# thanosDelatolas/eva-vos

Hardware: AMD Instinct MI355X
Metric: frames/sec STCN mask-propagate 480p 1-obj (higher is better)
Workload: dtype f32; 1 GPU; DAVIS-17-val-shaped 480x854 (padded 480x864) single-object STCN propagate: fresh engine, interact(mask,0), T=66 frames/video, mem_freq=5, top_k=50; one video per step per GPU; videos_per_gpu=38, streams_per_gpu=4, key_lookahead=0, clips=8 distinct synthetic clips (one per pooled engine), weights=synthetic recipe seed 0 (no checkpoints offline)

## Files before the change

### eva_vos_amd/csrc/engine.cpp

```cpp
#include "engine.h"
#include "src_hash.h"

#include <algorithm>
#include <atomic>
#include <cmath>
#include <cstdarg>
#include <cstdio>
#include <cstdlib>
#include <cstring>
#include <map>
#include <mutex>
#include <unordered_map>
#include <utility>

namespace stcn {

static thread_local char g_err[512] = "";
void set_error(const char *fmt, ...) {
    va_list ap;
    va_start(ap, fmt);
    vsnprintf(g_err, sizeof(g_err), fmt, ap);
    va_end(ap);
}
const char *get_error() { return g_err; }

Knobs Knobs::from_env() {
    Knobs k;
    k.wino_min_cin = env_int("STCN_WINO_MIN_CIN", k.wino_min_cin);
    k.wino_ppw = env_int("STCN_WINO_PPW", k.wino_ppw);
    k.wino4_chunk_mb = env_int("STCN_WINO4_CHUNK_MB", k.wino4_chunk_mb);
    k.fusion_conv12 = env_int("STCN_FUSION_CONV12", k.fusion_conv12) != 0;
    k.fusion_wino = env_int("STCN_FUSION_WINO", k.fusion_wino) != 0;
    k.pw_chain = env_int("STCN_PW_CHAIN", k.pw_chain);
    return k;
}

void Prof::reset() {
    for (int i = 0; i < STCN_K_COUNT; ++i) { flops[i] = 0; bytes[i] = 0; exec_flops[i] = 0; launches[i] = 0; }
    hbm_conv_flops = hbm_conv_bytes = hbm_conv_ms = 0; hbm_conv_launches = 0;
    wino2_flops = wino4_flops = 0;
    for (auto &e : events) { pool.push_back(e.a); pool.push_back(e.b); }
    events.clear();
}
Prof::Ev &Prof::push_pair(int cls, bool hbm) {
    Ev e; e.cls = cls; e.hbm = hbm;
    for (hipEvent_t *p : {&e.a, &e.b}) {
        if (!pool.empty()) { *p = pool.back(); pool.pop_back(); }
        else (void)hipEventCreate(p);
    }
    events.push_back(e);
    return events.back();
}
void Prof::begin(int cls, hipStream_t s) {
    launches[cls]++;
    if (!on) return;
    (void)hipEventRecord(push_pair(cls, false).a, s);
}
hipEvent_t *Prof::attach(int cls, bool hbm) {
    launches[cls]++;
    if (hbm) hbm_conv_launches++;
    if (!on) return nullptr;
    return &push_pair(cls, hbm).a;
}
void Prof::end(hipStream_t s) {
    if (!on) return;
    (void)hipEventRecord(events.back().b, s);
}
int Prof::collect(float *ms) {
    for (int i = 0; i < STCN_K_COUNT; ++i) ms[i] = 0.f;
    hbm_conv_ms = 0;
    for (auto &e : events) {
        if (hipEventSynchronize(e.b) != hipSuccess) return STCN_E_HIP;
        float t = 0.f;
        if (hipEventElapsedTime(&t, e.a, e.b) != hipSuccess) return STCN_E_HIP;
        ms[e.cls] += t;
        if (e.hbm) hbm_conv_ms += t;
    }
    return STCN_OK;
}
Prof::~Prof() {
    for (auto &e : events) { (void)hipEventDestroy(e.a); (void)hipEventDestroy(e.b); }
    for (auto &p : pool) (void)hipEventDestroy(p);
}
struct Scope {
    Prof *p; hipStream_t s;
    Scope(Prof *p_, int cls, hipStream_t s_, double fl = 0) : p(p_), s(s_) {
        if (p) { p->flops[cls] += fl; p->begin(cls, s); }
    }
    ~Scope() { if (p) p->end(s); }
};

const ConvW &Model::c(const std::string &name) const {
    auto it = conv.find(name);
    if (it == conv.end()) { static ConvW empty; set_error("missing conv '%s'", name.c_str()); return empty; }
    return it->second;
}

struct HostT { const float *p; int nd; int64_t sh[4]; };

static int upload(Model &m, const std::vector<float> &h, float **dev) {
    HIPCHK(hipMalloc((void **)dev, h.size() * sizeof(float)));
    m.allocs.push_back(*dev);
    HIPCHK(hipMemcpy(*dev, h.data(), h.size() * sizeof(float), hipMemcpyHostToDevice));
    return STCN_OK;
}

bool wants_wino(const ConvW &cw) {
    const bool fusion32 = cw.cin_p == 32 && cw.cout == 32;
    return !(!wino_enabled() || cw.kh != 3 || cw.kw != 3 || cw.cin_p % 32 || ((cw.cin_p < Knobs::from_env().wino_min_cin || cw.cout % 64) && !fusion32));
}
bool wants_wino_fusion12(const ConvW &cw) { return wino_enabled() && cw.kh == 3 && cw.kw == 3 && cw.cin_p == 12 && cw.cout == 32; }
bool wants_wino4(const ConvW &cw) {
    return !(!wino4_mode() || cw.kh != 3 || cw.kw != 3 || cw.cin_p % 32 || cw.cin_p < W4_MIN_CIN || cw.cout % 32);
}

int make_wino(Model &m, ConvW &cw, const std::vector<float> &w) {
    if (!wants_wino(cw)) return STCN_OK;
    std::vector<float> u((size_t)16 * cw.cin_p * cw.cout);
    wino_transform_weights(w.data(), cw.cout, cw.cin_p, cw.Kp, u.data());
    return upload(m, u, &cw.wino_u);
}

int make_wino_fusion12(Model &m, ConvW &cw, const std::vector<float> &w) {
    if (!wants_wino_fusion12(cw)) return STCN_OK;
    std::vector<float> w16((size_t)32 * 9 * 16, 0.f), u((size_t)16 * 16 * 32);
    for (int n = 0; n < 32; ++n)
        for (int tap = 0; tap < 9; ++tap)
            for (int c = 0; c < 12; ++c) w16[((size_t)n * 9 + tap) * 16 + c] = w[(size_t)n * cw.Kp + tap * 12 + c];
    wino_transform_weights(w16.data(), 32, 16, 9 * 16, u.data());
    return upload(m, u, &cw.wino_u);
}

int make_wino4(Model &m, ConvW &cw, const std::vector<float> &w) {
    if (!wants_wino4(cw)) return STCN_OK;
    std::vector<float> u((size_t)36 * cw.cin_p * cw.cout);
    wino4_transform_weights(w.data(), cw.cout, cw.cin_p, cw.Kp, u.data());
    return upload(m, u, &cw.wino4_u);
}

static bool wino4_layer(const std::string &name) {
    if (name == "value_encoder.layer2.0.conv1" || name == "value_encoder.layer3.0.conv1") return false;
    if (name == "key_encoder.layer2.0.conv2" || name == "key_encoder.layer3.0.conv2") return false;
    static const bool key_f4 = env_on("STCN_WINO4_KEY");
    if (key_f4 && name.compare(0, 12, "key_encoder.") == 0 && name.size() > 6 && name.compare(name.size() - 6, 6, ".conv2") == 0) return true;
    static const bool kproj_f4 = env_on("STCN_WINO4_KEYPROJ");
    if (kproj_f4 && name == "key_proj.key_proj") return true;
    return name.compare(0, 8, "decoder.") == 0 || name == "key_comp" || name.compare(0, 20, "value_encoder.fuser.") == 0 ||
           name.compare(0, 19, "value_encoder.layer") == 0;
}

static std::vector<float> repack(const HostT &wt, const std::vector<float> &scale, int lo, int hi, const ConvW &cw) {
    const int cout = (int)wt.sh[0], cin = (int)wt.sh[1], kh = (int)wt.sh[2], kw = (int)wt.sh[3];
    std::vector<float> w((size_t)cout * cw.Kp, 0.f);
    for (int n = 0; n < cout; ++n)
        for (int c = lo; c < hi; ++c)
            for (int y = 0; y < kh; ++y)
                for (int x = 0; x < kw; ++x)
                    w[(size_t)n * cw.Kp + (size_t)(y * kw + x) * cw.cin_p + (c - lo)] =
                        wt.p[(((size_t)n * cin + c) * kh + y) * kw + x] * scale[n];
    return w;
}

static int add_convs(Model &m, const std::map<std::string, HostT> &sd) {
    for (auto &kv : sd) {
        const std::string &name = kv.first;
        if (name.size() < 8 || name.compare(name.size() - 7, 7, ".weight") != 0 || kv.second.nd != 4) continue;
        const std::string pre = name.substr(0, name.size() - 7);
        const HostT &wt = kv.second;
        const int cout = (int)wt.sh[0], cin = (int)wt.sh[1], kh = (int)wt.sh[2], kw = (int)wt.sh[3];
        std::string bn;
        const size_t dot = pre.rfind('.');
        const std::string leaf = pre.substr(dot + 1), head = pre.substr(0, dot);
        if (leaf.compare(0, 4, "conv") == 0) bn = head + ".bn" + leaf.substr(4);
        else if (leaf == "0") bn = head + ".1";
        const bool has_bn = !bn.empty() && sd.count(bn + ".running_mean");
        std::vector<float> scale(cout, 1.f), bias(cout, 0.f);
        auto bit = sd.find(pre + ".bias");
        if (bit != sd.end()) for (int n = 0; n < cout; ++n) bias[n] = bit->second.p[n];
        if (has_bn) {
            const float *g = sd.at(bn + ".weight").p, *b = sd.at(bn + ".bias").p;
            const float *mu = sd.at(bn + ".running_mean").p, *var = sd.at(bn + ".running_var").p;
            for (int n = 0; n < cout; ++n) {
                const float sc = g[n] / std::sqrt(var[n] + 1e-5f);
                scale[n] = sc;
                bias[n] = (bias[n] - mu[n]) * sc + b[n];
            }
        }
        ConvW cw;
        cw.cout = cout; cw.cin = cin; cw.kh = kh; cw.kw = kw;
        cw.cin_p = (cin + 3) / 4 * 4;
        cw.K = kh * kw * cw.cin_p;
        cw.Kp = (cw.K + 31) / 32 * 32;
        const std::vector<float> w = repack(wt, scale, 0, cin, cw);
        int rc = upload(m, w, &cw.w);
        if (rc) return rc;
        rc = upload(m, bias, &cw.bias);
        if (rc) return rc;
        if ((rc = make_wino(m, cw, w)) || (rc = make_wino_fusion12(m, cw, w))) return rc;
        if (wino4_layer(pre) && (rc = make_wino4(m, cw, w))) return rc;
        cw.bias0 = bias[0];
        m.conv[pre] = cw;
        static const struct { const char *name; int c0; } splits[] = {
            {"decoder.compress.conv1", 512}, {"decoder.compress.downsample", 512},
            {"value_encoder.fuser.block1.conv1", 256}, {"value_encoder.fuser.block1.downsample", 256}};
        for (const auto &sp : splits) {
            if (pre != sp.name) continue;
            for (int part = 0; part < 2; ++part) {
                const int lo = part ? sp.c0 : 0, hi = part ? cin : sp.c0;
                ConvW pw;
                pw.cout = cout; pw.cin = hi - lo; pw.cin_p = hi - lo; pw.kh = kh; pw.kw = kw;
                pw.K = kh * kw * pw.cin_p; pw.Kp = (pw.K + 31) / 32 * 32;
                const std::vector<float> ww = repack(wt, scale, lo, hi, pw);
                std::vector<float> bb = part ? bias : std::vector<float>(cout, 0.f);
                if ((rc = upload(m, ww, &pw.w)) || (rc = upload(m, bb, &pw.bias))) return rc;
                if ((rc = make_wino(m, pw, ww))) return rc;
                if (wino4_layer(pre) && (rc = make_wino4(m, pw, ww))) return rc;
                pw.bias0 = bb[0];
                m.conv[pre + (part ? "#b" : "#a")] = pw;
            }
        }
    }
    return STCN_OK;
}

static int add_fusion(Model &m, const stcn_weight_desc *fuse, int n_fuse);
static int build_model(Model &m, const stcn_weight_desc *prop, int n_prop, const stcn_weight_desc *fuse, int n_fuse) {
    std::map<std::string, HostT> sd;
    for (int i = 0; i < n_prop; ++i) {
        if (!prop[i].name || !prop[i].data || prop[i].ndim < 0 || prop[i].ndim > 4) {
            set_error("bad weight descriptor %d", i);
            return STCN_E_INVALID;
        }
        HostT t{prop[i].data, prop[i].ndim, {1, 1, 1, 1}};
        for (int d = 0; d < prop[i].ndim; ++d) t.sh[d] = prop[i].shape[d];
        sd[prop[i].name] = t;
    }
    int rc = add_convs(m, sd);
    if (rc) return rc;
    static const char *required[] = {
        "key_encoder.conv1", "key_encoder.res2.0.downsample.0", "key_encoder.layer3.5.conv3", "key_proj.key_proj",
        "key_comp", "value_encoder.conv1", "value_encoder.layer3.1.conv2", "value_encoder.fuser.block1.downsample",
        "value_encoder.fuser.block2.conv2", "decoder.compress.downsample", "decoder.up_16_8.skip_conv",
        "decoder.up_16_8.out_conv.downsample", "decoder.up_8_4.out_conv.conv2", "decoder.pred"};
    for (const char *r : required)
        if (!m.conv.count(r)) { set_error("state_dict lacks '%s.weight'", r); return STCN_E_MISSING; }
    const char *cb = "value_encoder.fuser.attention.";
    auto need = [&](const std::string &n) -> const HostT * {
        auto it = sd.find(std::string(cb) + n);
        if (it == sd.end()) { set_error("state_dict lacks '%s%s'", cb, n.c_str()); return nullptr; }
        return &it->second;
    };
    const HostT *w1 = need("ChannelGate.mlp.1.weight"), *b1 = need("ChannelGate.mlp.1.bias");
    const HostT *w2 = need("ChannelGate.mlp.3.weight"), *b2 = need("ChannelGate.mlp.3.bias");
    const HostT *ws = need("SpatialGate.spatial.conv.weight"), *bs = need("SpatialGate.spatial.conv.bias");
    if (!w1 || !b1 || !w2 || !b2 || !ws || !bs) return STCN_E_MISSING;
    float *d;
    auto up = [&](const HostT *t, size_t n, const float **dst) -> int {
        std::vector<float> h(t->p, t->p + n);
        int r = upload(m, h, &d);
        *dst = d;
        return r;
    };
    if ((rc = up(w1, 32 * 512, &m.cbam.w1)) || (rc = up(b1, 32, &m.cbam.b1)) || (rc = up(w2, 512 * 32, &m.cbam.w2)) ||
        (rc = up(b2, 512, &m.cbam.b2)) || (rc = up(ws, 98, &m.cbam.wsp)))
        return rc;
    m.cbam.bsp = bs->p[0];
    m.has_prop = true;
    if (fuse && n_fuse > 0) return add_fusion(m, fuse, n_fuse);
    return STCN_OK;
}
static int add_fusion(Model &m, const stcn_weight_desc *fuse, int n_fuse) {
    std::map<std::string, HostT> fsd;
    for (int i = 0; i < n_fuse; ++i) {
        HostT t{fuse[i].data, fuse[i].ndim, {1, 1, 1, 1}};
        for (int dd = 0; dd < fuse[i].ndim; ++dd) t.sh[dd] = fuse[i].shape[dd];
        fsd[std::string("fuse.") + fuse[i].name] = t;
    }
    const int rc = add_convs(m, fsd);
    if (rc) return rc;
    for (const char *r : {"fuse.conv1.0", "fuse.conv2.0", "fuse.conv2.2", "fuse.conv3.0", "fuse.conv3.2", "fuse.final_conv"})
        if (!m.conv.count(r)) { set_error("fusion state_dict lacks '%s.weight'", r + 5); return STCN_E_MISSING; }
    m.has_fuse = true;
    return STCN_OK;
}

namespace {
struct DevPool {
    std::mutex mu;
    std::map<std::pair<int, size_t>, std::vector<void *>> free_;
    std::unordered_map<void *, std::pair<int, size_t>> live;
    size_t cached = 0;
    size_t cap() {
        static const size_t c = [] { const char *e = getenv("STCN_POOL_GB"); const double gb = e ? atof(e) : 64.0; return gb > 0 ? (size_t)(gb * (double)(1u << 30)) : (size_t)0; }();
        return c;
    }
    static size_t size_class(size_t bytes) {
        if (bytes <= (1u << 20)) return (bytes + 4095) / 4096 * 4096;
        size_t step = 1;
        while ((step << 4) <= bytes) step <<= 1;
        return (bytes + step - 1) / step * step;
    }
};
DevPool &pool() { static DevPool p; return p; }
}

hipError_t pool_malloc(void **p, size_t bytes) {
    DevPool &pl = pool();
    int dev = 0;
    (void)hipGetDevice(&dev);
    const size_t sc = DevPool::size_class(bytes);
    if (pl.cap() > 0) {
        bool hit = false;
        {
            std::lock_guard<std::mutex> g(pl.mu);
            auto it = pl.free_.find({dev, sc});
            if (it != pl.free_.end() && !it->second.empty()) {
                *p = it->second.back();
                it->second.pop_back();
                pl.cached -= sc;
                pl.live[*p] = {dev, sc};
                hit = true;
            }
        }
        if (hit) {
            static const bool poison = env_on("STCN_POOL_POISON", false);
            if (poison) { (void)hipMemset(*p, 0xFF, sc); (void)hipStreamSynchronize(nullptr); }
            return hipSuccess;
        }
    }
    hipError_t er = hipMalloc(p, sc);
    if (er != hipSuccess && pl.cap() > 0) {
        (void)hipGetLastError();
        pool_release();
        er = hipMalloc(p, sc);
    }
    if (er == hipSuccess && pl.cap() > 0) {
        std::lock_guard<std::mutex> g(pl.mu);
        pl.live[*p] = {dev, sc};
    }
    return er;
}

void pool_free(void *p) {
    if (!p) return;
    DevPool &pl = pool();
    {
        std::lock_guard<std::mutex> g(pl.mu);
        auto it = pl.live.find(p);
        if (it != pl.live.end()) {
            const auto key = it->second;
            pl.live.erase(it);
            if (pl.cached + key.second <= pl.cap()) {
                pl.free_[key].push_back(p);
                pl.cached += key.second;
                return;
            }
        }
    }
    (void)hipFree(p);
}

void pool_release() {
    DevPool &pl = pool();
    std::vector<void *> all;
    {
        std::lock_guard<std::mutex> g(pl.mu);
        for (auto &kv : pl.free_) { all.insert(all.end(), kv.second.begin(), kv.second.end()); kv.second.clear(); }
        pl.cached = 0;
    }
    for (void *q : all) (void)hipFree(q);
}

size_t wino_v_capacity(const Dims &d, int maxb) {
    const long mt = ((long)maxb * ((d.h4 + 1) / 2) * ((d.w4 + 1) / 2) + 63) / 64 * 64;
    size_t v = wino_enabled() ? (size_t)16 * 256 * mt : 0;
    if (v * 4 >= ((size_t)1 << 32)) v = ((size_t)1 << 30) - 64;
    return v;
}
int Work::init(int nh, int nw, int k_, int key_batch, int group) {
    d.set(nh, nw);
    k = k_;
    auto alloc = [&](void **p, size_t bytes) -> int {
        HIPCHK(pool_malloc(p, bytes));
        allocs.push_back(*p);
        return STCN_OK;
    };
    const size_t s1 = (size_t)k * d.hw2 * 64, s2 = (size_t)d.npix * 32, s3 = (size_t)k * d.hw4 * 256;
    const size_t s4 = (size_t)key_batch * d.hw2 * 64;
    const size_t s5 = (size_t)group * k * d.hw4 * 256;
    S = s1 > s2 ? s1 : s2;
    S = S > s3 ? S : s3;
    S = S > s4 ? S : s4;
    S = S > s5 ? S : s5;
    const int kg = k * group;
    int rc;
    for (float **b : {&A, &B, &C, &D})
        if ((rc = alloc((void **)b, S * sizeof(float)))) return rc;
    splitk_floats = (size_t)32 * 1024 * 1024;
    if ((rc = alloc((void **)&splitk, splitk_floats * sizeof(float)))) return rc;
    {
        wino_v_floats = wino_v_capacity(d, key_batch > k * group ? key_batch : k * group);
        if (wino_v_floats && (rc = alloc((void **)&wino_v, wino_v_floats * sizeof(float)))) return rc;
    }
    if ((rc = alloc((void **)&cbam, (size_t)k * (16 * 1024 + 512 + 3 * d.hw16) * sizeof(float)))) return rc;
    if ((rc = alloc((void **)&readout, (size_t)kg * d.hw16 * 512 * sizeof(float)))) return rc;
    if ((rc = alloc((void **)&logit4, (size_t)kg * d.hw4 * sizeof(float)))) return rc;
    if ((rc = alloc((void **)&flogit, (size_t)k * d.npix * sizeof(float)))) return rc;
    if ((rc = alloc((void **)&agg, (size_t)(k + 1) * group * d.npix * sizeof(float)))) return rc;
    if ((rc = alloc((void **)&agg_alt, (size_t)(k + 1) * group * d.npix * sizeof(float)))) return rc;
    if ((rc = alloc((void **)&pooled, (size_t)std::max(20, attention_nchp(2 * (k + 1))) * d.hw16 * sizeof(float)))) return rc;
    if ((rc = alloc((void **)&amap, (size_t)(k + 1) * 2 * d.hw16 * sizeof(float)))) return rc;
    if ((rc = alloc((void **)&attn, (size_t)(k + 1) * 2 * d.npix * sizeof(float)))) return rc;
    const MemReadScratchSizes ms = memread_scratch_floats(group * d.hw16);
    if ((rc = alloc((void **)&cand_v, std::max(ms.cand_v, attention_part_floats(k + 1, d.hw16)) * sizeof(float)))) return rc;
    if ((rc = alloc((void **)&cand_i, ms.cand_i * sizeof(int32_t)))) return rc;
    if ((rc = alloc((void **)&cand_n, ms.cand_n * sizeof(int32_t)))) return rc;
    if ((rc = alloc((void **)&qk, (size_t)group * d.hw16 * 64 * sizeof(float)))) return rc;
    if ((rc = alloc((void **)&vin, (size_t)k * d.npix * 8 * sizeof(float)))) return rc;
    if ((rc = alloc((void **)&gmax, ms.gmax * sizeof(float)))) return rc;
    if ((rc = alloc((void **)&tau, ms.tau * sizeof(float)))) return rc;
    return STCN_OK;
}
void Work::release() {
    for (void *p : allocs) pool_free(p);
    allocs.clear();
}

static thread_local int g_fail_countdown = 0;
static thread_local int g_fail_reserve = 0;
static std::atomic<int> g_side_delay_us{0};
void inject_failure_after(int n) { g_fail_countdown = n; }
int launch_status(const char *what) {
    if (g_fail_countdown > 0 && --g_fail_countdown == 0) {
        (void)hipGetLastError();
        set_error("launch of '%s' failed: injected fault (stcn_test_fail_at)", what);
        return STCN_E_HIP;
    }
    const hipError_t er = hipGetLastError();
    if (er == hipSuccess) return STCN_OK;
    set_error("launch of '%s' failed: %s", what, hipGetErrorString(er));
    return STCN_E_HIP;
}

namespace {
struct ConvPathRec {
    ConvPlan plan{};
    char lit[96] = "";
};
thread_local ConvPathRec g_path;
thread_local char g_path_str[96] = "";
thread_local bool g_trace_on = false;
thread_local std::string g_trace;
}
const char *format_conv_path(const ConvPlan &pl, char *out, size_t n) {
    switch (pl.family) {
    case CONV_FUSION: snprintf(out, n, "%s", pl.fusion_wino ? "fusion_wino" : "fusion_direct"); break;
    case CONV_WINO4: snprintf(out, n, "wino4 chunks=%d%s", pl.w4.chunks, pl.reduce ? " +tail" : ""); break;
    case CONV_WINO2: snprintf(out, n, "wino2 ppw=%d splitk=%d", pl.ppw, pl.splitk); break;
    case CONV_DIRECT: snprintf(out, n, "%s%s splitk=%d", pl.variant, pl.tail ? " +tail" : "", pl.splitk); break;
    default: snprintf(out, n, "%s", "");
    }
    return out;
}
const char *last_conv_path() { return g_path.plan.family == CONV_LITERAL ? g_path.lit : format_conv_path(g_path.plan, g_path_str, sizeof(g_path_str)); }
void set_conv_path(const char *s) { g_path.plan.family = CONV_LITERAL; snprintf(g_path.lit, sizeof(g_path.lit), "%s", s); }
void conv_trace(int on) { g_trace_on = on != 0; if (on) g_trace.clear(); }
const char *conv_trace_get() { return g_trace.c_str(); }

int plan_conv(const Model &m, const Work &w, const std::string &name, const ConvArgs &a, ConvP &p, ConvPlan &pl) {
    auto it = m.conv.find(name);
    if (it == m.conv.end()) { set_error("missing conv '%s'", name.c_str()); return STCN_E_MISSING; }
    const ConvW &cw = it->second;
    const int B = a.B, H = a.H, W = a.W, c0 = a.c0, c1 = a.c1;
    if (c0 + c1 != cw.cin_p) { set_error("conv '%s': %d+%d input channels, weights have %d", name.c_str(), c0, c1, cw.cin_p); return STCN_E_INVALID; }
    p = ConvP{};
    p.B = B; p.H = H; p.W = W;
    p.KH = cw.kh; p.KW = cw.kw; p.stride = a.stride; p.pad = cw.kh / 2;
    p.OH = (H + 2 * p.pad - cw.kh) / a.stride + 1;
    p.OW = (W + 2 * p.pad - cw.kw) / a.stride + 1;
    p.Cin = cw.cin_p;
    p.M = B * p.OH * p.OW; p.N = cw.cout; p.K = cw.K; p.Kp = cw.Kp;
    const long bs0 = a.bs0 == CONV_DENSE ? (long)H * W * c0 : a.bs0, bs1 = a.bs1 == CONV_DENSE ? (long)H * W * c1 : a.bs1;
    const long res_bs = a.res_bs == CONV_DENSE ? (long)p.OH * p.OW * p.N : a.res_bs;
    p.x0 = a.x0; p.x1 = a.x1; p.c0 = c0; p.c1 = c1; p.bs0 = bs0; p.bs1 = bs1;
    const long x0b = (bs0 ? (long)B * bs0 : (long)H * W * c0) * 4, x1b = a.x1 ? (bs1 ? (long)B * bs1 : (long)H * W * c1) * 4 : 0;
    if (x0b >= (1L << 31) || x1b >= (1L << 31) || (long)cw.cout * cw.Kp * 4 >= (1L << 31)) {
        set_error("conv '%s': operand of %ld bytes exceeds the 2 GiB the kernels can address (B=%d, %dx%d)", name.c_str(), x0b > x1b ? x0b : x1b, B, H, W);
        return STCN_E_INVALID;
    }
    p.x0_bytes = (unsigned)x0b;
    p.x1_bytes = (unsigned)x1b;
    p.w_bytes = (unsigned)((long)cw.cout * cw.Kp * 4);
    if (a.x1 && ((cw.cin_p % 32) || (c0 % 32) || cw.kh * cw.kw > 32)) { set_error("conv '%s': two-source input needs 32-aligned channel splits", name.c_str()); return STCN_E_INVALID; }
    p.w = cw.w; p.wino_u = cw.wino_u; p.wino4_u = cw.wino4_u;
    p.bias = cw.bias; p.res = a.res; p.res_bs = res_bs; p.res_bmod = a.res_bmod; p.y = a.y; p.y_bs = a.y_bs;
    p.relu_in = a.relu_in; p.relu_out = a.relu_out;
    p.fd_ohw = fastdiv_make((unsigned)(p.OH * p.OW));
    p.fd_ow = fastdiv_make((unsigned)p.OW);
    p.fd_cin = fastdiv_make((unsigned)p.Cin);
    p.fd_kw = fastdiv_make((unsigned)p.KW);
    p.pointwise = cw.kh == 1 && cw.kw == 1 && a.stride == 1 && !a.x1 && bs0 == (long)H * W * c0;
    p.affine_out = (a.y_bs == 0 || a.y_bs == (long)p.OH * p.OW * p.N) && (!a.res || (res_bs == (long)p.OH * p.OW * p.N && !a.res_bmod)) &&
                   ((long)p.M + 128) * p.N * 4 < (1L << 32);
    p.partial = w.splitk;
    p.kn = w.kn;
    pl = ConvPlan{};
    pl.fl = 2.0 * p.M * p.N * (double)(cw.kh * cw.kw * cw.cin);
    if (a.force_splitk <= 0 && (fusion_conv_plan(p, pl) || wino4_plan(p, m.wino4_min_wg, w.wino_v_floats, w.splitk_floats, pl) ||
                                wino_plan(p, w.wino_v_floats, w.splitk_floats, pl)))
        return STCN_OK;
    conv_plan(p, a.force_splitk, w.splitk_floats, pl);
    return STCN_OK;
}

int run_conv(const Model &m, Work &w, hipStream_t s, const std::string &name, const ConvArgs &a) {
    ConvP p;
    ConvPlan &pl = g_path.plan;
    const int rc = plan_conv(m, w, name, a, p, pl);
    if (rc) return rc;
    hipEvent_t *eg[W4_MAX_CHUNKS] = {}, *ei[W4_MAX_CHUNKS] = {}, *er = nullptr;
    if (w.prof) {
        const double in0 = (double)(p.bs0 ? p.B : 1) * p.H * p.W * p.c0, in1 = p.x1 ? (double)(p.bs1 ? p.B : 1) * p.H * p.W * p.c1 : 0.0;
        const double resb = p.res ? (p.res_bs ? (double)p.M * p.N : (double)p.OH * p.OW * p.N) : 0.0;
        const double bytes = 4.0 * (in0 + in1 + (double)p.N * p.K + (double)p.M * p.N + resb);
        const bool hbm_bound = pl.fl / bytes < 157.3e12 / 8.0e12;
        const int cls = w.conv_cls;
        const bool hbm_acc = hbm_bound && cls == STCN_K_CONV;
        w.prof->bytes[cls] += bytes;
        w.prof->flops[cls] += pl.fl;
        w.prof->exec_flops[cls] += pl.fl_exec;
        if (hbm_acc) { w.prof->hbm_conv_bytes += bytes; w.prof->hbm_conv_flops += pl.fl; }
        if (pl.family == CONV_WINO4) w.prof->wino4_flops += pl.fl; else if (pl.family == CONV_WINO2) w.prof->wino2_flops += pl.fl;
        for (int c = 0; c < pl.n_gemm; ++c) {
            eg[c] = w.prof->attach(cls, hbm_acc);
            if (c < pl.n_in) ei[c] = w.prof->attach(STCN_K_WINO_INPUT);
        }
        if (pl.reduce) er = w.prof->attach(STCN_K_CONV_REDUCE);
    }
    if (g_trace_on) { char b[96]; g_trace += name; g_trace += '='; g_trace += format_conv_path(pl, b, sizeof(b)); g_trace += '\n'; }
    switch (pl.family) {
    case CONV_FUSION: fusion_conv_launch(p, pl, s, eg[0]); break;
    case CONV_WINO4: wino4_launch(p, pl, w.wino_v, s, ei, eg, er); break;
    case CONV_WINO2: wino_launch(p, pl, w.wino_v, s, ei[0], eg[0], er); break;
    default: conv_launch(p, s, eg[0], er);
    }
    return launch_status(name.c_str());
}

#define RC(x) do { int rc_ = (x); if (rc_) return rc_; } while (0)

int encode_key(const Model &m, Work &w, hipStream_t s, const float *img4, const KeyOut &o, int B, long out_bs) {
    const Dims &d = w.d;
    const long obs = B > 1 ? out_bs : 0;
    const long ibs = obs ? obs : CONV_DENSE;
    RC(run_conv(m, w, s, "key_encoder.conv1", ConvArgs(img4, 4, B, d.nh, d.nw).strided(2).out(w.A).relu(0, 1)));
    { Scope sc(w.prof, STCN_K_ELEMWISE, s); maxpool3x3s2_launch(w.A, w.B, B, d.h2, d.w2, 64, s); }
    struct St { const char *name; int n, planes, stride; } stages[3] = {{"res2", 3, 64, 1}, {"layer2", 4, 128, 2}, {"layer3", 6, 256, 2}};
    int H = d.h4, W = d.w4, cin = 64;
    float *x = w.B;
    for (int si = 0; si < 3; ++si) {
        const St &st = stages[si];
        for (int i = 0; i < st.n; ++i) {
            const std::string p = std::string("key_encoder.") + st.name + "." + std::to_string(i);
            const int sd = i == 0 ? st.stride : 1;
            const int OH = H / sd, OW = W / sd;
            const float *idt = x;
            if (i == 0) { RC(run_conv(m, w, s, p + ".downsample.0", ConvArgs(x, cin, B, H, W).strided(sd).out(w.D))); idt = w.D; }
            RC(run_conv(m, w, s, p + ".conv1", ConvArgs(x, cin, B, H, W).out(w.C).relu(0, 1)));
            RC(run_conv(m, w, s, p + ".conv2", ConvArgs(w.C, st.planes, B, H, W).strided(sd).out(w.A).relu(0, 1)));
            float *dst = x;
            long dst_bs = 0;
            if (si == 2 && i == st.n - 1) { dst = o.f16; dst_bs = obs; }
            RC(run_conv(m, w, s, p + ".conv3", ConvArgs(w.A, st.planes, B, OH, OW).out(dst, dst_bs).residual(idt).relu(0, 1)));
            x = dst; H = OH; W = OW; cin = st.planes * 4;
        }
        if (si == 0) {
            if (o.f4_copy) HIPCHK(hipMemcpyAsync(o.f4_copy, x, (size_t)d.hw4 * 256 * 4, hipMemcpyDeviceToDevice, s));
            if (o.s4) RC(run_conv(m, w, s, "decoder.up_8_4.skip_conv", ConvArgs(x, 256, B, d.h4, d.w4).out(o.s4, obs)));
        } else if (si == 1) {
            if (o.f8_copy) HIPCHK(hipMemcpyAsync(o.f8_copy, x, (size_t)d.hw8 * 512 * 4, hipMemcpyDeviceToDevice, s));
            if (o.s8) RC(run_conv(m, w, s, "decoder.up_16_8.skip_conv", ConvArgs(x, 512, B, d.h8, d.w8).out(o.s8, obs)));
        }
    }
    if (o.k16) {
        RC(run_conv(m, w, s, "key_proj.key_proj", ConvArgs(o.f16, 1024, B, d.h16, d.w16, ibs).out(o.k16, obs)));
        if (o.msq) {
            Scope sc(w.prof, STCN_K_ELEMWISE, s);
            rowsumsq_launch(o.k16, d.hw16, 64, o.msq, s, B, out_bs, out_bs);
        }
    }
    if (o.f16_thin) RC(run_conv(m, w, s, "key_comp", ConvArgs(o.f16, 1024, B, d.h16, d.w16, ibs).out(o.f16_thin, obs)));
    if (o.f16_thin && o.dthin) {
        RC(run_conv(m, w, s, "decoder.compress.downsample#b", ConvArgs(o.f16_thin, 512, B, d.h16, d.w16, ibs).out(o.dthin, obs)));
        RC(run_conv(m, w, s, "decoder.compress.conv1#b", ConvArgs(o.f16_thin, 512, B, d.h16, d.w16, ibs).out(o.cthin, obs).relu(1, 0)));
    }
    return STCN_OK;
}

int value_frame_parts(const Model &m, Work &w, hipStream_t s, const float *f16, float *vd, float *vc) {
    const Dims &d = w.d;
    RC(run_conv(m, w, s, "value_encoder.fuser.block1.downsample#b", ConvArgs(f16, 1024, 1, d.h16, d.w16).out(vd)));
    RC(run_conv(m, w, s, "value_encoder.fuser.block1.conv1#b", ConvArgs(f16, 1024, 1, d.h16, d.w16).out(vc).relu(1, 0)));
    return STCN_OK;
}

static int resblock_split(const Model &m, Work &w, hipStream_t s, const std::string &p, const float *x, int c, int B,
                          int H, int W, const float *dpart, const float *cpart, long part_bs, int part_bmod, float *t1, float *t2,
                          float *out, long out_bs) {
    const ConvW &cw = m.c(p + ".conv1");
    RC(run_conv(m, w, s, p + ".downsample#a", ConvArgs(x, c, B, H, W).out(t2).residual(dpart, part_bs, part_bmod)));
    RC(run_conv(m, w, s, p + ".conv1#a", ConvArgs(x, c, B, H, W).out(t1).residual(cpart, part_bs, part_bmod).relu(1, 1)));
    RC(run_conv(m, w, s, p + ".conv2", ConvArgs(t1, cw.cout, B, H, W).out(out, out_bs).residual(t2)));
    return STCN_OK;
}

static int resblock(const Model &m, Work &w, hipStream_t s, const std::string &p, const float *x0, int c0, long bs0,
                    const float *x1, int c1, long bs1, int B, int H, int W, float *t1, float *t2, float *out,
                    long out_bs) {
    const ConvW &cw = m.c(p + ".conv1");
    const ConvArgs in = ConvArgs(x0, c0, B, H, W, bs0).concat(x1, c1, bs1);
    const float *skip; long skip_bs;
    if (m.conv.count(p + ".downsample")) {
        RC(run_conv(m, w, s, p + ".downsample", ConvArgs(in).out(t2)));
        skip = t2; skip_bs = CONV_DENSE;
    } else { skip = x0; skip_bs = bs0; }
    RC(run_conv(m, w, s, p + ".conv1", ConvArgs(in).out(t1).relu(1, 1)));
    RC(run_conv(m, w, s, p + ".conv2", ConvArgs(t1, cw.cout, B, H, W).out(out, out_bs).residual(skip, skip_bs)));
    return STCN_OK;
}

int encode_value(const Model &m, Work &w, hipStream_t s, const float *img4, const float *f16, const float *masks,
                 long mask_stride, float *out, long out_bs, const float *vd, const float *vc) {
    const Dims &d = w.d;
    const int k = w.k;
    { Scope sc(w.prof, STCN_K_ELEMWISE, s); pack_value_input_launch(img4, masks, mask_stride, k, (int)d.npix, w.vin, s); }
    RC(run_conv(m, w, s, "value_encoder.conv1", ConvArgs(w.vin, 8, k, d.nh, d.nw).strided(2).out(w.C).relu(0, 1)));
    { Scope sc(w.prof, STCN_K_ELEMWISE, s); maxpool3x3s2_launch(w.C, w.B, k, d.h2, d.w2, 64, s); }
    int H = d.h4, W = d.w4, cin = 64;
    const int planes[3] = {64, 128, 256}, strides[3] = {1, 2, 2};
    for (int li = 0; li < 3; ++li)
        for (int i = 0; i < 2; ++i) {
            const std::string p = "value_encoder.layer" + std::to_string(li + 1) + "." + std::to_string(i);
            const int sd = i == 0 ? strides[li] : 1;
            const int OH = H / sd, OW = W / sd;
            const float *idt = w.B;
            if (m.conv.count(p + ".downsample.0")) {
                RC(run_conv(m, w, s, p + ".downsample.0", ConvArgs(w.B, cin, k, H, W).strided(sd).out(w.D)));
                idt = w.D;
            }
            RC(run_conv(m, w, s, p + ".conv1", ConvArgs(w.B, cin, k, H, W).strided(sd).out(w.C).relu(0, 1)));
            RC(run_conv(m, w, s, p + ".conv2", ConvArgs(w.C, planes[li], k, OH, OW).out(w.B).residual(idt).relu(0, 1)));
            H = OH; W = OW; cin = planes[li];
        }
    const std::string f = "value_encoder.fuser.";
    if (vd && vc)
        RC(resblock_split(m, w, s, f + "block1", w.B, 256, k, d.h16, d.w16, vd, vc, 0, 0, w.C, w.D, w.A, 0));
    else
        RC(resblock(m, w, s, f + "block1", w.B, 256, (long)d.hw16 * 256, f16, 1024, 0, k, d.h16, d.w16, w.C, w.D, w.A, 0));
    { Scope sc(w.prof, STCN_K_OTHER, s); cbam_launch(w.A, w.C, k, d.h16, d.w16, m.cbam, w.cbam, s); }
    RC(resblock(m, w, s, f + "block2", w.C, 512, (long)d.hw16 * 512, nullptr, 0, 0, k, d.h16, d.w16, w.D, w.A, out, out_bs));
    return STCN_OK;
}

int decode_logit4(const Model &m, Work &w, hipStream_t s, const float *readout, const float *f16_thin, const float *s8,
                  const float *s4, const float *dthin, const float *cthin, int G, long slot_bs) {
    const Dims &d = w.d;
    const int k = w.k;
    if (G > 1 && (!dthin || !cthin)) { set_error("decode: frame batches need the cached frame parts"); return STCN_E_INVALID; }
    const int B = G > 1 ? G * k : k;
    const long fbs = G > 1 ? slot_bs : 0;
    const int bmod = G > 1 && k > 1 ? G : 0;
    if (dthin && cthin) {
        RC(resblock_split(m, w, s, "decoder.compress", readout, 512, B, d.h16, d.w16, dthin, cthin, fbs, bmod, w.C, w.D, w.A, 0));
    } else {
        RC(resblock(m, w, s, "decoder.compress", readout, 512, (long)d.hw16 * 512, f16_thin, 512, 0, k, d.h16, d.w16, w.C,
                    w.D, w.A, 0));
    }
    { Scope sc(w.prof, STCN_K_ELEMWISE, s); upsample2x_add_launch(w.A, s8, w.B, B, d.h16, d.w16, 512, s, fbs, bmod); }
    RC(resblock(m, w, s, "decoder.up_16_8.out_conv", w.B, 512, (long)d.hw8 * 512, nullptr, 0, 0, B, d.h8, d.w8, w.C, w.D,
                w.A, 0));
    { Scope sc(w.prof, STCN_K_ELEMWISE, s); upsample2x_add_launch(w.A, s4, w.B, B, d.h8, d.w8, 256, s, fbs, bmod); }
    RC(resblock(m, w, s, "decoder.up_8_4.out_conv", w.B, 256, (long)d.hw4 * 256, nullptr, 0, 0, B, d.h4, d.w4, w.C, w.D,
                w.A, 0));
    const ConvW &pw = m.c("decoder.pred");
    {
        Scope sc(w.prof, STCN_K_CONV_N1, s, 2.0 * B * d.hw4 * 9 * 256);
        conv_n1_launch(w.A, pw.w, pw.bias0, w.logit4, B, d.h4, d.w4, 256, 3, 1, s);
    }
    return STCN_OK;
}

int decode(const Model &m, Work &w, hipStream_t s, const float *readout, const float *f16_thin, const float *s8,
           const float *s4, float *agg, long agg_stride, const float *dthin, const float *cthin, int G, long slot_bs, long agg_gs) {
    const Dims &d = w.d;
    const int k = w.k;
    RC(decode_logit4(m, w, s, readout, f16_thin, s8, s4, dthin, cthin, G, slot_bs));
    {
        Scope sc(w.prof, STCN_K_ELEMWISE, s);
        if (G > 1)
            up4_sigmoid_aggregate_launch(w.logit4, k, d.h4, d.w4, agg, agg_stride, s, (long)G * d.hw4, G, (long)d.hw4, agg_gs ? agg_gs : (long)(k + 1) * agg_stride);
        else
            up4_sigmoid_aggregate_launch(w.logit4, k, d.h4, d.w4, agg, agg_stride, s);
    }
    return launch_status("decoder tail");
}

int fusion_logit(const Model &m, Work &w, hipStream_t s, const float *img4, const float *prev, const float *curr,
                 const float *attn2, float nc, float nr, float *logit) {
    if (!m.has_fuse) { set_error("model was built without a fusion network"); return STCN_E_STATE; }
    const Dims &d = w.d;
    { Scope sc(w.prof, STCN_K_ELEMWISE, s); pack_fusion_input_launch(img4, prev, curr, attn2, nc, nr, d.npix, w.A, s); }
    struct Cls { Work &w; Cls(Work &w_) : w(w_) { w.conv_cls = STCN_K_FUSION_CONV; } ~Cls() { w.conv_cls = STCN_K_CONV; } } cls_guard(w);
    RC(run_conv(m, w, s, "fuse.conv1.0", ConvArgs(w.A, 12, 1, d.nh, d.nw).out(w.B).relu(0, 1)));
    RC(run_conv(m, w, s, "fuse.conv2.0", ConvArgs(w.B, 32, 1, d.nh, d.nw).out(w.C).relu(0, 1)));
    RC(run_conv(m, w, s, "fuse.conv2.2", ConvArgs(w.C, 32, 1, d.nh, d.nw).out(w.D).residual(w.B).relu(0, 1)));
    RC(run_conv(m, w, s, "fuse.conv3.0", ConvArgs(w.D, 32, 1, d.nh, d.nw).out(w.C).relu(0, 1)));
    RC(run_conv(m, w, s, "fuse.conv3.2", ConvArgs(w.C, 32, 1, d.nh, d.nw).out(w.B).residual(w.D).relu(0, 1)));
    const ConvW &fw = m.c("fuse.final_conv");
    Scope sc(w.prof, STCN_K_CONV_N1, s, 2.0 * d.npix * 9 * 32);
    conv_n1_launch(w.B, fw.w, fw.bias0, logit, 1, d.nh, d.nw, 32, 3, 0, s);
    return STCN_OK;
}

std::vector<SweepGroup> plan_sweep(int idx, int closest, int mem_freq, int cap) {
    const int step = closest > idx ? 1 : -1, span = std::abs(closest - idx) - 1;
    std::vector<SweepGroup> groups;
    if (span > 0) groups.reserve(span / mem_freq + span / (cap > 1 ? cap : 1) + 1);
    int last = 0;
    auto inserts = [&](int dist) { return dist != span && dist - last >= mem_freq; };
    for (int dist = 1, G; dist <= span; dist += G) {
        G = 1;
        while (G < cap && !inserts(dist + G - 1) && dist + G <= span) ++G;
        const int first = idx + dist * step;
        const bool ins = inserts(dist + G - 1);
        groups.push_back(SweepGroup{first, step > 0 ? first : first - (G - 1), G, ins});
        if (ins) last = dist + G - 1;
    }
    return groups;
}

}

using namespace stcn;

extern "C" {

const char *stcn_last_error(void) { return stcn::get_error(); }
const char *stcn_version(void) { return "stcn_hip 0.4 (gfx950; exact-fp32 MFMA convs: direct implicit GEMM + Winograd; src " STCN_SRC_HASH ")"; }

int stcn_model_create(int device, const stcn_weight_desc *prop, int n_prop, const stcn_weight_desc *fuse, int n_fuse,
                      stcn_model **out) {
    return stcn_model_create_ex(device, prop, n_prop, fuse, n_fuse, nullptr, out);
}

static_assert(STCN_MAX_TOP_K == MEMREAD_MAX_TOPK, "the C ABI's limit is the read's");

int stcn_model_create_ex(int device, const stcn_weight_desc *prop, int n_prop, const stcn_weight_desc *fuse, int n_fuse,
                         const stcn_model_opts *opts, stcn_model **out) {
    if (!prop || n_prop <= 0 || !out) { set_error("stcn_model_create: null arguments"); return STCN_E_INVALID; }
    const int top_k = opts && opts->top_k > 0 ? opts->top_k : STCN_MAX_TOP_K;
    if (top_k > STCN_MAX_TOP_K) {
        set_error("stcn_model_create: top_k=%d is not supported: the memory read is built for 1 <= top_k <= %d", top_k, STCN_MAX_TOP_K);
        return STCN_E_INVALID;
    }
    if (opts && !std::isfinite(opts->km)) {
        set_error("stcn_model_create: km=%f is not supported: the kernelized memory read takes a finite km > 0 (0 or negative: not given)", (double)opts->km);
        return STCN_E_INVALID;
    }
    const float km = opts && opts->km > 0.f ? opts->km : 0.f;
    HIPCHK(hipSetDevice(device));
    stcn_model *mm = new stcn_model();
    mm->m.device = device;
    mm->m.top_k = top_k;
    mm->m.km = km;
    const int rc = build_model(mm->m, prop, n_prop, fuse, n_fuse);
    if (rc) { stcn_model_destroy(mm); return rc; }
    *out = mm;
    return STCN_OK;
}

int stcn_fusion_model_create(int device, const stcn_weight_desc *fuse, int n_fuse, stcn_model **out) {
    if (!fuse || n_fuse <= 0 || !out) { set_error("stcn_fusion_model_create: null arguments"); return STCN_E_INVALID; }
    for (int i = 0; i < n_fuse; ++i)
        if (!fuse[i].name || !fuse[i].data || fuse[i].ndim < 0 || fuse[i].ndim > 4) { set_error("bad weight descriptor %d", i); return STCN_E_INVALID; }
    HIPCHK(hipSetDevice(device));
    stcn_model *mm = new stcn_model();
    mm->m.device = device;
    const int rc = add_fusion(mm->m, fuse, n_fuse);
    if (rc) { stcn_model_destroy(mm); return rc; }
    *out = mm;
    return STCN_OK;
}

int stcn_model_get_top_k(const stcn_model *m, int32_t *top_k) {
    if (!m || !top_k) { set_error("stcn_model_get_top_k: null arguments"); return STCN_E_INVALID; }
    *top_k = m->m.top_k;
    return STCN_OK;
}

int stcn_model_get_km(const stcn_model *m, float *km) {
    if (!m || !km) { set_error("stcn_model_get_km: null arguments"); return STCN_E_INVALID; }
    *km = m->m.km;
    return STCN_OK;
}

int stcn_model_destroy(stcn_model *m) {
    if (!m) return STCN_OK;
    for (void *p : m->m.allocs) (void)hipFree(p);
    delete m;
    return STCN_OK;
}

static int eng_alloc(stcn_engine *e, void **p, size_t bytes) {
    HIPCHK(pool_malloc(p, bytes));
    e->allocs.push_back(*p);
    return STCN_OK;
}

struct SlotPtrs { float *k16, *msq, *f16_thin, *f16, *s8, *s4, *dthin, *cthin, *vd, *vc; };
struct PassCtx { hipStream_t s; Work *w; bool may_offload; int dir; };
static PassCtx main_ctx(stcn_engine *e) { return PassCtx{e->stream, &e->work, true, +1}; }
struct SweepBank {
    int lo, n_certain, dir, n_temp;
    int slots() const { return n_certain + n_temp; }
    int first() const { return dir > 0 ? lo : lo - n_temp; }
    int next_slot() const { return dir > 0 ? lo + n_certain + n_temp : lo - 1 - n_temp; }
};
struct Neighbours { int lo, hi; };
static Neighbours interacted_neighbours(const stcn_engine *e, int idx) {
    Neighbours n{-1, e->T};
    for (int t : e->interacted) { if (t < idx && t > n.lo) n.lo = t; if (t > idx && t < n.hi) n.hi = t; }
    return n;
}
static int sweep_slots(int span, int mem_freq) { return span / mem_freq + 1; }
static SlotPtrs slot_ptrs(const stcn_engine *e, int slot) {
    const Dims &d = e->d;
    float *b = e->cache + (size_t)slot * e->slot_floats;
    SlotPtrs p;
    p.k16 = b; b += (size_t)d.hw16 * 64;
    p.msq = b; b += (size_t)(d.hw16 + 3) / 4 * 4;
    p.f16_thin = b; b += (size_t)d.hw16 * 512;
    p.f16 = b; b += (size_t)d.hw16 * 1024;
    p.s8 = b; b += (size_t)d.hw8 * 512;
    p.s4 = b; b += (size_t)d.hw4 * 256;
    p.dthin = b; b += (size_t)d.hw16 * 512;
    p.cthin = b; b += (size_t)d.hw16 * 512;
    p.vd = b; b += (size_t)d.hw16 * 512;
    p.vc = b;
    return p;
}

static void bank_collect_retired(stcn_engine *e, bool wait) {
    if (e->retired.empty()) return;
    if (wait) (void)hipEventSynchronize(e->retire_ev);
    else if (hipEventQuery(e->retire_ev) != hipSuccess) return;
    for (void *p : e->retired) pool_free(p);
    e->retired.clear();
}

static int bank_reserve(stcn_engine *e, int slots) {
    if (slots <= e->bank_cap) return STCN_OK;
    const Dims &d = e->d;
    int cap = e->bank_cap ? e->bank_cap : 8;
    while (cap < slots) cap *= 2;
    float *nk = nullptr, *nq = nullptr, *nv = nullptr;
    int32_t *nc = nullptr;
    const size_t rows = (size_t)cap * d.hw16;
    const size_t cblock = e->model->km > 0.f ? (size_t)e->group * memread_centre_stride((int)rows) : 0;
    hipError_t er = pool_malloc((void **)&nk, rows * 64 * 4);
    if (er == hipSuccess) er = pool_malloc((void **)&nq, (rows + MEMREAD_MSQ_PAD) * 4);
    if (er == hipSuccess) er = pool_malloc((void **)&nv, (size_t)e->k * rows * 512 * 4);
    if (er == hipSuccess && cblock) er = pool_malloc((void **)&nc, 2 * cblock * 4);
    if (er != hipSuccess) {
        if (nk) pool_free(nk);
        if (nq) pool_free(nq);
        if (nv) pool_free(nv);
        if (nc) pool_free(nc);
        set_error("bank_reserve: %d slots (%zu MB) -> %s", cap, ((size_t)e->k * rows * 512 * 4 + rows * 65 * 4) >> 20, hipGetErrorString(er));
        return STCN_E_HIP;
    }
    auto fail = [&](hipError_t err, const char *what) {
        (void)hipStreamSynchronize(e->stream);
        pool_free(nk); pool_free(nq); pool_free(nv);
        if (nc) pool_free(nc);
        set_error("bank_reserve: %s -> %s", what, hipGetErrorString(err));
        return STCN_E_HIP;
    };
    if (e->n_certain > 0) {
        const size_t crow = (size_t)e->n_certain * d.hw16, orow = (size_t)e->bank_cap * d.hw16, lo = (size_t)e->bank_lo * d.hw16;
        if ((er = hipMemcpyAsync(nk + lo * 64, e->bank_k + lo * 64, crow * 64 * 4, hipMemcpyDeviceToDevice, e->stream)) != hipSuccess) return fail(er, "copy of the certain keys");
        if ((er = hipMemcpyAsync(nq + lo, e->bank_msq + lo, crow * 4, hipMemcpyDeviceToDevice, e->stream)) != hipSuccess) return fail(er, "copy of |mk|^2");
        for (int o = 0; o < e->k; ++o)
            if ((er = hipMemcpyAsync(nv + (o * rows + lo) * 512, e->bank_v + (o * orow + lo) * 512, crow * 512 * 4, hipMemcpyDeviceToDevice, e->stream)) != hipSuccess)
                return fail(er, "copy of the certain values");
    }
    if (e->bank_k) {
        bank_collect_retired(e, true);
        if (!e->retire_ev && (er = hipEventCreateWithFlags(&e->retire_ev, hipEventDisableTiming)) != hipSuccess) return fail(er, "event create");
        if ((er = hipEventRecord(e->retire_ev, e->stream)) != hipSuccess) return fail(er, "event record");
        e->retired = {e->bank_k, e->bank_msq, e->bank_v};
        if (e->bank_centre) e->retired.push_back(e->bank_centre);
    }
    e->bank_k = nk; e->bank_msq = nq; e->bank_v = nv; e->bank_cap = cap;
    e->bank_centre = nc; e->work.centre = nc; e->work2.centre = nc ? nc + cblock : nullptr;
    return STCN_OK;
}

static int engine_alloc_common(stcn_engine *e) {
    const Dims &d = e->d;
    if (!e->images4) {
        HIPCHK(pool_malloc((void **)&e->images4, (size_t)e->T * d.npix * 4 * 4));
        e->images_owner = std::shared_ptr<void>(e->images4, [](void *p) { pool_free(p); });
    }
    e->n_slots = e->T < 106 ? e->T : 106;
    e->slot_floats = (size_t)d.hw16 * (64 + 512 + 1024) + (size_t)(d.hw16 + 3) / 4 * 4 + (size_t)d.hw8 * 512 + (size_t)d.hw4 * 256 +
                     (size_t)4 * d.hw16 * 512;
    RC(eng_alloc(e, (void **)&e->cache, (size_t)e->n_slots * e->slot_floats * 4));
    e->slot_of.assign(e->T, -1);
    e->vparts_ready.assign(e->T, 0);
    RC(eng_alloc(e, (void **)&e->mask_pad, (size_t)(e->k + 1) * d.npix * 4));
    RC(eng_alloc(e, (void **)&e->pos, (size_t)(e->k + 1) * d.npix * 4));
    RC(eng_alloc(e, (void **)&e->neg, (size_t)(e->k + 1) * d.npix * 4));
    auto opt = [](int32_t &field, const char *env, int dflt) { if (field < 0) field = env_int(env, dflt); return (int)field; };
    const int la_env = opt(e->opts.lookahead, "STCN_LOOKAHEAD", 2);
    e->lookahead = la_env;
    if (e->T > e->n_slots) e->lookahead = 0;
    e->group = opt(e->opts.decode_batch, "STCN_DECODE_BATCH", 8);
    if (e->group > e->mem_freq) e->group = e->mem_freq;
    if (e->group < 1) e->group = 1;
    if (e->group > MAX_DECODE_GROUP) e->group = MAX_DECODE_GROUP;
    while (e->group > 1 && e->group * e->k > 16) --e->group;
    e->key_batch = opt(e->opts.key_batch, "STCN_KEY_BATCH", 0);
    if (e->key_batch <= 0) e->key_batch = e->group > 4 ? e->group : 4;
    if (e->key_batch < 1) e->key_batch = 1;
    if (e->key_batch > 8) e->key_batch = 8;
    RC(e->work.init(d.nh, d.nw, e->k, e->lookahead > 0 ? 1 : e->key_batch, e->group));
    e->work.prof = &e->prof;
    e->fuse_side = la_env > 0 && e->model->has_fuse && opt(e->opts.fuse_side, "STCN_FUSE_SIDE", 1) != 0;
    if (e->lookahead > 0 || e->fuse_side) {
        HIPCHK(hipStreamCreateWithFlags(&e->side, hipStreamNonBlocking));
        RC(e->work_side.init(d.nh, d.nw, e->k, e->lookahead > 0 ? e->key_batch : 1));
        e->work_side.prof = &e->prof;
        for (int b = 0; b < 2 && e->fuse_side; ++b) {
            HIPCHK(hipEventCreateWithFlags(&e->ev_dec[b], hipEventDisableTiming));
            HIPCHK(hipEventCreateWithFlags(&e->ev_fuse[b], hipEventDisableTiming));
        }
    }
    if (e->lookahead > 0) {
        e->key_ready.assign(e->T, nullptr);
        for (int t = 0; t < e->T; ++t) HIPCHK(hipEventCreateWithFlags(&e->key_ready[t], hipEventDisableTiming));
    }
    e->key_pending.assign(e->T, 0);
    e->bank_lo = 0;
    {
        const char *dv = getenv("STCN_DUAL_SWEEP");
        if (la_env > 0 && e->T <= e->n_slots && e->T >= 3 && (!dv || atoi(dv) != 0)) {
            HIPCHK(hipStreamCreateWithFlags(&e->stream2, hipStreamNonBlocking));
            RC(e->work2.init(d.nh, d.nw, e->k, e->lookahead > 0 ? 1 : e->key_batch, e->group));
            e->work2.prof = &e->prof;
            HIPCHK(hipEventCreateWithFlags(&e->ev_fork, hipEventDisableTiming));
            HIPCHK(hipEventCreateWithFlags(&e->ev_join, hipEventDisableTiming));
            e->bank_lo = sweep_slots(e->T - 1, e->mem_freq) + 1;
        }
    }
    return STCN_OK;
}

static int engine_init_outputs(stcn_engine *e) {
    const Dims &d = e->d;
    fill_launch(e->prob, 1e-7f, (long)e->T * d.npix, e->stream);
    fill_launch(e->prob + (size_t)e->T * d.npix, 0.f, (long)e->k * e->T * d.npix, e->stream);
    HIPCHK(hipMemsetAsync(e->masks, 0, (size_t)e->T * d.npix, e->stream));
    return STCN_OK;
}

int stcn_engine_create(const stcn_model *m, int T, int H, int W, int k, int mem_freq, void *stream,
                       const float *images_dev, float *prob_dev, uint8_t *masks_dev, stcn_engine **out) {
    return stcn_engine_create_ex(m, T, H, W, k, mem_freq, stream, images_dev, prob_dev, masks_dev, nullptr, out);
}

int stcn_engine_create_ex(const stcn_model *m, int T, int H, int W, int k, int mem_freq, void *stream,
                          const float *images_dev, float *prob_dev, uint8_t *masks_dev, const stcn_engine_opts *opts, stcn_engine **out) {
    if (!m || !images_dev || !prob_dev || !masks_dev || !out) { set_error("stcn_engine_create: null arguments"); return STCN_E_INVALID; }
    if (T < 1 || H < 16 || W < 16 || k < 1 || k > STCN_MAX_OBJECTS || mem_freq < 1) {
        set_error("stcn_engine_create: bad shape T=%d H=%d W=%d k=%d mem_freq=%d (1<=k<=%d)", T, H, W, k, mem_freq, STCN_MAX_OBJECTS);
        return STCN_E_INVALID;
    }
    if (!m->m.has_prop) { set_error("stcn_engine_create: a model of stcn_fusion_model_create serves stcn_stage_fusion only"); return STCN_E_STATE; }
    HIPCHK(hipSetDevice(m->m.device));
    stcn_engine *e = new stcn_engine();
    e->model = &m->m; e->stream = (hipStream_t)stream;
    if (opts) e->opts = *opts;
    e->T = T; e->H = H; e->W = W; e->k = k; e->mem_freq = mem_freq;
    const int nh = (H + 15) / 16 * 16, nw = (W + 15) / 16 * 16;
    e->lh = (nh - H) / 2; e->uh = nh - H - e->lh; e->lw = (nw - W) / 2; e->uw = nw - W - e->lw;
    e->d.set(nh, nw);
    if ((long)e->d.hw16 < m->m.top_k) {
        set_error("frame too small: (H/16)*(W/16) = %d must be >= top_k = %d for the top-k read", e->d.hw16, m->m.top_k);
        delete e;
        return STCN_E_INVALID;
    }
    e->prob = prob_dev; e->masks = masks_dev;
    int rc = engine_alloc_common(e);
    if (!rc) rc = bank_reserve(e, e->bank_lo + sweep_slots(T - 1, mem_freq) + 8);
    if (rc) { stcn_engine_destroy(e); return rc; }
    const Dims &d = e->d;
    for (int t = 0; t < T; ++t)
        pack_image_launch(images_dev + (size_t)t * 3 * H * W, e->images4 + (size_t)t * d.npix * 4, H, W, nh, nw, e->lw, e->lh, e->stream);
    if ((rc = engine_init_outputs(e))) { stcn_engine_destroy(e); return rc; }
    HIPCHK(hipStreamSynchronize(e->stream));
    *out = e;
    return STCN_OK;
}

int stcn_engine_reset(stcn_engine *e) {
    if (!e) { set_error("stcn_engine_reset: null engine"); return STCN_E_INVALID; }
    HIPCHK(hipSetDevice(e->model->device));
    if (e->side) HIPCHK(hipStreamSynchronize(e->side));
    if (e->stream2) HIPCHK(hipStreamSynchronize(e->stream2));
    e->failed.clear();
    e->interacted.clear();
    e->n_certain = 0;
    e->n_cached = 0;
    std::fill(e->slot_of.begin(), e->slot_of.end(), -1);
    std::fill(e->vparts_ready.begin(), e->vparts_ready.end(), 0);
    std::fill(e->key_pending.begin(), e->key_pending.end(), 0);
    e->fuse_pending[0] = e->fuse_pending[1] = 0;
    e->stats = stcn_stats{};
    return engine_init_outputs(e);
}

int stcn_engine_destroy(stcn_engine *e) {
    if (!e) return STCN_OK;
    if (e->stream) (void)hipStreamSynchronize(e->stream); else (void)hipDeviceSynchronize();
    if (e->side) { (void)hipStreamSynchronize(e->side); (void)hipStreamDestroy(e->side); }
    if (e->stream2) { (void)hipStreamSynchronize(e->stream2); (void)hipStreamDestroy(e->stream2); }
    if (e->ev_fork) (void)hipEventDestroy(e->ev_fork);
    if (e->ev_join) (void)hipEventDestroy(e->ev_join);
    e->work2.release();
    for (hipEvent_t ev : e->key_ready) if (ev) (void)hipEventDestroy(ev);
    for (int b = 0; b < 2; ++b) { if (e->ev_dec[b]) (void)hipEventDestroy(e->ev_dec[b]); if (e->ev_fuse[b]) (void)hipEventDestroy(e->ev_fuse[b]); }
    e->work_side.release();
    for (void *p : e->allocs) pool_free(p);
    if (e->bank_k) { pool_free(e->bank_k); pool_free(e->bank_msq); pool_free(e->bank_v); }
    if (e->bank_centre) pool_free(e->bank_centre);
    bank_collect_retired(e, true);
    if (e->retire_ev) (void)hipEventDestroy(e->retire_ev);
    e->work.release();
    delete e;
    return STCN_OK;
}

static int clone_state(stcn_engine *e, const stcn_engine *src) {
    const Dims &d = e->d;
    HIPCHK(hipStreamSynchronize(src->stream));
    if (src->side) HIPCHK(hipStreamSynchronize(src->side));
    if (src->stream2) HIPCHK(hipStreamSynchronize(src->stream2));
    HIPCHK(hipMemcpyAsync(e->cache, src->cache, (size_t)src->n_cached * e->slot_floats * 4, hipMemcpyDeviceToDevice, e->stream));
    e->slot_of = src->slot_of; e->n_cached = src->n_cached; e->vparts_ready = src->vparts_ready;
    e->n_certain = src->n_certain; e->interacted = src->interacted; e->failed = src->failed;
    const size_t crow = (size_t)e->n_certain * d.hw16;
    if (crow) {
        const size_t lo = (size_t)e->bank_lo * d.hw16, slo = (size_t)src->bank_lo * d.hw16;
        HIPCHK(hipMemcpyAsync(e->bank_k + lo * 64, src->bank_k + slo * 64, crow * 64 * 4, hipMemcpyDeviceToDevice, e->stream));
        HIPCHK(hipMemcpyAsync(e->bank_msq + lo, src->bank_msq + slo, crow * 4, hipMemcpyDeviceToDevice, e->stream));
        for (int o = 0; o < e->k; ++o)
            HIPCHK(hipMemcpyAsync(e->bank_v + ((size_t)o * e->bank_cap * d.hw16 + lo) * 512,
                                  src->bank_v + ((size_t)o * src->bank_cap * d.hw16 + slo) * 512, crow * 512 * 4,
                                  hipMemcpyDeviceToDevice, e->stream));
    }
    HIPCHK(hipMemcpyAsync(e->pos, src->pos, (size_t)(e->k + 1) * d.npix * 4, hipMemcpyDeviceToDevice, e->stream));
    HIPCHK(hipMemcpyAsync(e->neg, src->neg, (size_t)(e->k + 1) * d.npix * 4, hipMemcpyDeviceToDevice, e->stream));
    HIPCHK(hipStreamSynchronize(e->stream));
    return STCN_OK;
}

int stcn_engine_clone(const stcn_engine *src, float *prob_dev, uint8_t *masks_dev, void *stream, stcn_engine **out) {
    if (!src || !prob_dev || !masks_dev || !out) { set_error("stcn_engine_clone: null arguments"); return STCN_E_INVALID; }
    HIPCHK(hipSetDevice(src->model->device));
    stcn_engine *e = new stcn_engine();
    e->model = src->model; e->stream = (hipStream_t)stream;
    e->T = src->T; e->H = src->H; e->W = src->W; e->k = src->k; e->mem_freq = src->mem_freq;
    e->lw = src->lw; e->uw = src->uw; e->lh = src->lh; e->uh = src->uh; e->d = src->d;
    e->prob = prob_dev; e->masks = masks_dev;
    e->images4 = src->images4; e->images_owner = src->images_owner;
    e->opts = src->opts;
    e->work.kn = src->work.kn; e->work_side.kn = src->work_side.kn; e->work2.kn = src->work.kn;
    int rc = engine_alloc_common(e);
    if (!rc) rc = bank_reserve(e, src->bank_cap + e->bank_lo);
    if (!rc) rc = clone_state(e, src);
    if (rc) { stcn_engine_destroy(e); return rc; }
    *out = e;
    return STCN_OK;
}

static void flush_key_cache(stcn_engine *e) {
    for (int b = 0; b < 2; ++b)
        if (e->fuse_pending[b]) { (void)hipStreamWaitEvent(e->stream, e->ev_fuse[b], 0); e->fuse_pending[b] = 0; }
    std::fill(e->slot_of.begin(), e->slot_of.end(), -1);
    std::fill(e->vparts_ready.begin(), e->vparts_ready.end(), 0);
    e->n_cached = 0;
}

static int enqueue_key_batch(stcn_engine *e, int t_lo, int B, const PassCtx &cx) {
    const int slot = e->n_cached;
    e->n_cached += B;
    for (int b = 0; b < B; ++b) { e->slot_of[t_lo + b] = slot + b; e->vparts_ready[t_lo + b] = 0; }
    const SlotPtrs p = slot_ptrs(e, slot);
    KeyOut ko{p.k16, p.msq, p.f16_thin, p.f16, p.s8, p.s4, nullptr, nullptr, p.dthin, p.cthin};
    const float *img = e->images4 + (size_t)t_lo * e->d.npix * 4;
    if (e->lookahead > 0) {
        hipStream_t ks = e->side;
        if (const int us = g_side_delay_us.load(std::memory_order_relaxed)) spin_launch(us, ks);
        RC(encode_key(*e->model, e->work_side, ks, img, ko, B, (long)e->slot_floats));
        for (int b = 0; b < B; ++b) {
            HIPCHK(hipEventRecord(e->key_ready[t_lo + b], ks));
            e->key_pending[t_lo + b] = 1;
        }
    } else {
        RC(encode_key(*e->model, *cx.w, cx.s, img, ko, B, (long)e->slot_floats));
    }
    e->stats.key_miss += B;
    return STCN_OK;
}

static int enqueue_key(stcn_engine *e, int ti, const PassCtx &cx, int step = 0, int stop = 0) {
    if (e->slot_of[ti] >= 0) return STCN_OK;
    if (e->n_cached >= e->n_slots) flush_key_cache(e);
    int B = 1;
    if (step != 0)
        while (B < e->key_batch && e->n_cached + B < e->n_slots) {
            const int tn = ti + B * step;
            if (tn == stop || tn < 0 || tn >= e->T || e->slot_of[tn] >= 0) break;
            ++B;
        }
    return enqueue_key_batch(e, step < 0 ? ti - (B - 1) : ti, B, cx);
}

static int enqueue_group(stcn_engine *e, int t_lo, int G, const PassCtx &cx) {
    int missing = 0;
    for (int b = 0; b < G; ++b) missing += e->slot_of[t_lo + b] < 0;
    if (!missing) return STCN_OK;
    if (e->n_cached + missing > e->n_slots) { flush_key_cache(e); }
    for (int b = 0; b < G;) {
        if (e->slot_of[t_lo + b] >= 0) { ++b; continue; }
        int n = 1;
        while (b + n < G && n < e->key_batch && e->slot_of[t_lo + b + n] < 0) ++n;
        RC(enqueue_key_batch(e, t_lo + b, n, cx));
        b += n;
    }
    return STCN_OK;
}

static int ensure_key(stcn_engine *e, int ti, SlotPtrs *out, const PassCtx &cx) {
    RC(enqueue_key(e, ti, cx));
    if (e->key_pending[ti]) {
        HIPCHK(hipStreamWaitEvent(cx.s, e->key_ready[ti], 0));
        e->key_pending[ti] = 0;
    }
    *out = slot_ptrs(e, e->slot_of[ti]);
    return STCN_OK;
}

static void dbg_sum(stcn_engine *e, const char *tag, int ti, const float *p, size_t n) {
    static const bool on = getenv("STCN_DEBUG_CHECKSUM") != nullptr;
    if (!on) return;
    (void)hipDeviceSynchronize();
    std::vector<float> h(n);
    (void)hipMemcpy(h.data(), p, n * 4, hipMemcpyDeviceToHost);
    double s1 = 0, s2 = 0;
    unsigned long long hsh = 1469598103934665603ull, bag = 0;
    for (size_t i = 0; i < n; ++i) {
        unsigned u; memcpy(&u, &h[i], 4);
        hsh = (hsh ^ u) * 1099511628211ull;
        bag += (unsigned long long)u * 2654435761ull;
        if (std::isfinite(h[i])) { s1 += h[i]; s2 += (double)h[i] * h[i] * (1 + (i % 7)); }
    }
    fprintf(stderr, "CHK %-10s t=%d %.10e %.10e hash %016llx bag %016llx\n", tag, ti, s1, s2, hsh, bag);
    (void)e;
}

static float *bank_v_slot(stcn_engine *e, int slot) { return e->bank_v + (size_t)slot * e->d.hw16 * 512; }

static int bank_insert(stcn_engine *e, int slot, int ti, const SlotPtrs &kf, const float *masks, long mask_stride, const PassCtx &cx) {
    const Dims &d = e->d;
    {
        Scope sc(&e->prof, STCN_K_ELEMWISE, cx.s);
        copy2_launch(kf.k16, e->bank_k + (size_t)slot * d.hw16 * 64, (long)d.hw16 * 64, kf.msq, e->bank_msq + (size_t)slot * d.hw16, d.hw16, cx.s);
    }
    if (!e->vparts_ready[ti]) {
        RC(value_frame_parts(*e->model, *cx.w, cx.s, kf.f16, kf.vd, kf.vc));
        e->vparts_ready[ti] = 1;
    }
    RC(encode_value(*e->model, *cx.w, cx.s, e->images4 + (size_t)ti * d.npix * 4, kf.f16, masks, mask_stride,
                    bank_v_slot(e, slot), (long)e->bank_cap * d.hw16 * 512, kf.vd, kf.vc));
    dbg_sum(e, "value", ti, bank_v_slot(e, slot), (size_t)d.hw16 * 512);
    e->stats.value_enc++;
    return STCN_OK;
}

struct Sweep {
    const PassCtx &cx;
    int idx, closest, step;
    bool fuse;
    bool offload;
    SweepBank bank;
};

static int stage_keys_grouped(stcn_engine *e, const PassCtx &cx, const SweepGroup &g, const SweepGroup *next) {
    RC(enqueue_group(e, g.t_lo, g.G, cx));
    if (e->lookahead > 0 && next) RC(enqueue_group(e, next->t_lo, next->G, cx));
    return STCN_OK;
}
static int stage_keys_framewise(stcn_engine *e, const Sweep &sw, int ti) {
    RC(enqueue_key(e, ti, sw.cx, sw.step, sw.closest));
    for (int a = 1, tj = ti + sw.step; a <= e->lookahead && tj != sw.closest; ++a, tj += sw.step) RC(enqueue_key(e, tj, sw.cx, sw.step, sw.closest));
    return STCN_OK;
}

static int acquire_agg(stcn_engine *e, const PassCtx &cx, bool off, float **buf) {
    const int bi = off ? e->agg_buf : 0;
    if (cx.may_offload && e->fuse_pending[bi]) {
        HIPCHK(hipStreamWaitEvent(cx.s, e->ev_fuse[bi], 0));
        e->fuse_pending[bi] = 0;
    }
    *buf = bi ? cx.w->agg_alt : cx.w->agg;
    return STCN_OK;
}

static int read_decode(stcn_engine *e, const Sweep &sw, const SlotPtrs &f, int t_lo, int n, float *agg, long agg_rs) {
    const Dims &d = e->d;
    const int k = e->k, Q = n * d.hw16, N = sw.bank.slots() * d.hw16;
    const size_t row0 = (size_t)sw.bank.first() * d.hw16;
    Work &w = *sw.cx.w;
    hipStream_t const S = sw.cx.s;
    const float *qk = f.k16;
    if (n > 1) {
        Scope sc(&e->prof, STCN_K_ELEMWISE, S);
        copy_rows_launch(f.k16, (long)e->slot_floats, w.qk, (long)d.hw16 * 64, n, (long)d.hw16 * 64, S);
        qk = w.qk;
    }
    {
        const bool km = e->model->km > 0.f;
        const MemReadKm kmo{e->model->km, d.h16, d.w16, f.msq, (long)e->slot_floats, w.centre, nullptr};
        MemRead r{};
        r.mk = e->bank_k + row0 * 64; r.msq = e->bank_msq + row0; r.mv = e->bank_v + row0 * 512; r.mv_os = (long)e->bank_cap * d.hw16 * 512; r.N = N;
        r.qk = qk; r.Q = Q; r.k = k; r.top_k = e->model->top_k; r.readout = w.readout; r.ro_os = (long)Q * 512; r.km = km ? &kmo : nullptr;
        const MemReadCost cost = memread_cost(N, Q, k, r.top_k, km);
        Scope sc(&e->prof, STCN_K_MEMREAD, S, cost.flop);
        e->prof.bytes[STCN_K_MEMREAD] += cost.bytes;
        memory_read_launch(r, MemReadScratch{w.cand_v, w.cand_i, w.cand_n, w.gmax, w.tau}, S);
    }
    RC(launch_status(n > 1 ? "memory read (decode group)" : "memory read"));
    dbg_sum(e, "k16", t_lo, qk, (size_t)Q * 64);
    dbg_sum(e, "readout", t_lo, w.readout, (size_t)k * Q * 512);
    const long agg_gs = sw.fuse ? 0 : (long)d.npix;
    return decode(*e->model, w, S, w.readout, f.f16_thin, f.s8, f.s4, agg, agg_rs, f.dthin, f.cthin, n, (long)e->slot_floats, agg_gs);
}

static int fuse_frame(stcn_engine *e, const Sweep &sw, int t, const SlotPtrs &f, const float *agg, bool off, bool first_of_group) {
    const Dims &d = e->d;
    const int k = e->k;
    const long prs = (long)e->T * d.npix;
    float *dst = e->prob + (size_t)t * d.npix;
    const float nc = (float)std::abs(sw.closest - t) / (float)std::abs(sw.closest - sw.idx);
    const float nr = (float)std::abs(sw.idx - t) / (float)std::abs(sw.closest - sw.idx);
    const int cs = e->bank_lo + e->n_certain - 1;
    Work &fw = off ? e->work_side : *sw.cx.w;
    hipStream_t fs = off ? e->side : sw.cx.s;
    if (off && first_of_group) {
        HIPCHK(hipEventRecord(e->ev_dec[e->agg_buf], sw.cx.s));
        HIPCHK(hipStreamWaitEvent(e->side, e->ev_dec[e->agg_buf], 0));
        if (const int us = g_side_delay_us.load(std::memory_order_relaxed)) spin_launch(us, e->side);
    }
    {
        Scope sc(&e->prof, STCN_K_ATTENTION, fs, 2.0 * d.hw16 * d.hw16 * 64);
        attention_read_launch(e->bank_k + (size_t)cs * d.hw16 * 64, e->bank_msq + (size_t)cs * d.hw16, f.k16, nullptr,
                              nullptr, k + 1, d.h16, d.w16, e->work.pooled, fw.amap, fw.attn, AttnScratch{fw.gmax, fw.cand_v}, fs);
    }
    RC(launch_status("attention read"));
    for (int o = 1; o <= k; ++o)
        RC(fusion_logit(*e->model, fw, fs, e->images4 + (size_t)t * d.npix * 4, dst + (size_t)o * prs,
                        agg + (size_t)o * d.npix, fw.attn + (size_t)o * 2 * d.npix, nc, nr,
                        fw.flogit + (size_t)(o - 1) * d.npix));
    Scope sc(&e->prof, STCN_K_ELEMWISE, fs);
    sigmoid_aggregate_launch(fw.flogit, k, d.npix, dst, prs, fs);
    e->stats.fused++;
    return STCN_OK;
}

static int finish_frame(stcn_engine *e, Sweep &sw, int t, const SlotPtrs &f, float *agg, long agg_rs, bool inserts, bool off, bool first_of_group) {
    if (sw.fuse) dbg_sum(e, "agg", t, agg, (size_t)(e->k + 1) * e->d.npix);
    if (inserts) {
        RC(bank_insert(e, sw.bank.next_slot(), t, f, agg + agg_rs, agg_rs, sw.cx));
        ++sw.bank.n_temp;
    }
    if (sw.fuse) RC(fuse_frame(e, sw, t, f, agg, off, first_of_group));
    e->stats.frames++;
    return STCN_OK;
}

static int do_pass(stcn_engine *e, int idx, int closest, const PassCtx &cx) {
    const Dims &d = e->d;
    const bool forward = closest > idx, fuse = closest != e->T && closest != -1;
    RC(bank_reserve(e, e->bank_lo + sweep_slots(std::abs(closest - idx) - 1, e->mem_freq) + e->n_certain));
    Sweep sw{cx, idx, closest, forward ? 1 : -1, fuse, fuse && e->fuse_side && e->side && cx.may_offload, SweepBank{e->bank_lo, e->n_certain, cx.dir, 0}};
    const long agg_fs = (long)(e->k + 1) * d.npix;
    const long agg_rs = fuse ? (long)d.npix : (long)e->T * d.npix;
    const std::vector<SweepGroup> groups = plan_sweep(idx, closest, e->mem_freq, e->group);
    for (size_t i = 0; i < groups.size(); ++i) {
        const SweepGroup &g = groups[i];
        SlotPtrs kf[MAX_DECODE_GROUP];
        if (e->group > 1) RC(stage_keys_grouped(e, cx, g, i + 1 < groups.size() ? &groups[i + 1] : nullptr));
        else RC(stage_keys_framewise(e, sw, g.first));
        for (int j = 0; j < g.G; ++j) RC(ensure_key(e, g.first + j * sw.step, &kf[j], cx));
        bool batched = g.G > 1;
        for (int b = 1; b < g.G && batched; ++b) batched = e->slot_of[g.t_lo + b] == e->slot_of[g.t_lo] + b;
        const bool off = sw.offload && (batched || g.G == 1);
        float *aggbuf;
        RC(acquire_agg(e, cx, off, &aggbuf));
        auto agg_of = [&](int t) { return fuse ? aggbuf + (size_t)(batched ? t - g.t_lo : 0) * agg_fs : e->prob + (size_t)t * d.npix; };
        if (batched) RC(read_decode(e, sw, kf[forward ? 0 : g.G - 1], g.t_lo, g.G, agg_of(g.t_lo), agg_rs));
        for (int j = 0; j < g.G; ++j) {
            const int t = g.first + j * sw.step;
            if (!batched) RC(read_decode(e, sw, kf[j], t, 1, agg_of(t), agg_rs));
            RC(finish_frame(e, sw, t, kf[j], agg_of(t), agg_rs, g.inserts && j == g.G - 1, off, j == 0));
        }
        if (off) {
            HIPCHK(hipEventRecord(e->ev_fuse[e->agg_buf], e->side));
            e->fuse_pending[e->agg_buf] = 1;
            e->agg_buf ^= 1;
        }
    }
    (forward ? e->stats.bank_fwd : e->stats.bank_bwd) = sw.bank.slots();
    return STCN_OK;
}

static int interact_run(stcn_engine *e, const float *mask_dev, int mask_channels, int idx, int scribble) {
    const int kk = e->k + 1;
    const Dims &d = e->d;
    e->interacted.insert(idx);
    {
        Scope sc(&e->prof, STCN_K_ELEMWISE, e->stream);
        interact_mask_launch(mask_dev, mask_channels, e->H, e->W, d.nh, d.nw, e->lw, e->lh, e->prob + (size_t)idx * d.npix,
                             (long)e->T * d.npix, kk, e->mask_pad, e->pos, e->neg, e->stream);
    }
    attention_pool_launch(e->pos, e->neg, kk, d.h16, d.w16, e->work.pooled, e->stream);
    RC(launch_status("interaction mask"));
    SlotPtrs kf;
    const PassCtx c0 = main_ctx(e);
    RC(ensure_key(e, idx, &kf, c0));
    RC(bank_insert(e, e->bank_lo + e->n_certain, idx, kf, e->mask_pad + (scribble ? d.npix : 0), d.npix, c0));
    e->n_certain++;
    const Neighbours nb = interacted_neighbours(e, idx);
    if (e->stream2 && nb.hi - idx > 1 && idx - nb.lo > 1) {
        HIPCHK(hipEventRecord(e->ev_fork, e->stream));
        HIPCHK(hipStreamWaitEvent(e->stream2, e->ev_fork, 0));
        if (const int us = g_side_delay_us.load(std::memory_order_relaxed)) spin_launch(us, e->stream2);
        RC(do_pass(e, idx, nb.hi, c0));
        RC(do_pass(e, idx, nb.lo, PassCtx{e->stream2, &e->work2, false, -1}));
        HIPCHK(hipEventRecord(e->ev_join, e->stream2));
        HIPCHK(hipStreamWaitEvent(e->stream, e->ev_join, 0));
    } else {
        RC(do_pass(e, idx, nb.hi, c0));
        RC(do_pass(e, idx, nb.lo, c0));
    }
    for (int b = 0; b < 2; ++b)
        if (e->fuse_pending[b]) { HIPCHK(hipStreamWaitEvent(e->stream, e->ev_fuse[b], 0)); e->fuse_pending[b] = 0; }
    {
        Scope sc(&e->prof, STCN_K_ELEMWISE, e->stream);
        argmax_launch(e->prob, kk, e->T, d.npix, e->masks, e->stream);
    }
    return launch_status("argmax");
}

int stcn_interact(stcn_engine *e, const float *mask_dev, int mask_channels, int idx, int scribble) {
    if (!e || !mask_dev) { set_error("stcn_interact: null arguments"); return STCN_E_INVALID; }
    if (!e->failed.empty()) {
        set_error("stcn_interact: the engine is in a failed state after '%s': call stcn_engine_reset() (or destroy it)", e->failed.c_str());
        return STCN_E_STATE;
    }
    if (idx < 0 || idx >= e->T) { set_error("stcn_interact: idx %d outside [0,%d)", idx, e->T); return STCN_E_INVALID; }
    const int k = e->k, kk = k + 1;
    const int vplanes = scribble ? mask_channels - 1 : mask_channels;
    if ((mask_channels != 1 && mask_channels != kk) || vplanes != k) {
        set_error("stcn_interact: mask with %d channels is not valid for k=%d, scribble=%d (reference raises too)", mask_channels, k, scribble);
        return STCN_E_INVALID;
    }
    HIPCHK(hipSetDevice(e->model->device));
    bank_collect_retired(e, false);
    {
        const Neighbours nb = interacted_neighbours(e, idx);
        const int span = std::max(nb.hi - idx - 1, idx - nb.lo - 1);
        const int rc0 = g_fail_reserve ? (g_fail_reserve = 0, set_error("bank_reserve: injected fault (stcn_test_fail_at(-1))"), STCN_E_HIP)
                                       : bank_reserve(e, e->bank_lo + sweep_slots(span, e->mem_freq) + e->n_certain + 1);
        if (rc0) return rc0;
    }
    e->stats = stcn_stats{};
    e->prof.reset();
    const bool was_interacted = e->interacted.count(idx) != 0;
    const int n_certain0 = e->n_certain;
    const int rc = interact_run(e, mask_dev, mask_channels, idx, scribble);
    if (rc) {
        const std::string why = get_error();
        (void)hipStreamSynchronize(e->stream);
        if (e->side) (void)hipStreamSynchronize(e->side);
        if (e->stream2) (void)hipStreamSynchronize(e->stream2);
        (void)hipGetLastError();
        if (!was_interacted) e->interacted.erase(idx);
        e->n_certain = n_certain0;
        std::fill(e->key_pending.begin(), e->key_pending.end(), 0);
        e->fuse_pending[0] = e->fuse_pending[1] = 0;
        e->failed = why;
        set_error("%s", why.c_str());
    }
    return rc;
}

int stcn_pool_release(void) { pool_release(); return STCN_OK; }

const char *stcn_last_conv_path(void) { return stcn::last_conv_path(); }

int stcn_test_conv_trace(int on) { stcn::conv_trace(on); return STCN_OK; }
const char *stcn_test_conv_trace_get(void) { return stcn::conv_trace_get(); }

int stcn_test_side_delay_us(int us) { g_side_delay_us.store(us < 0 ? 0 : us, std::memory_order_relaxed); return STCN_OK; }

int stcn_test_fail_at(int n) {
    if (n < 0) { g_fail_reserve = 1; return STCN_OK; }
    inject_failure_after(n);
    return STCN_OK;
}

int stcn_engine_get_opts(const stcn_engine *e, stcn_engine_opts *out) {
    if (!e || !out) return STCN_E_INVALID;
    out->lookahead = e->lookahead;
    out->decode_batch = e->group;
    out->key_batch = e->key_batch;
    out->fuse_side = e->fuse_side ? 1 : 0;
    return STCN_OK;
}

int stcn_get_stats(const stcn_engine *e, stcn_stats *out) {
    if (!e || !out) return STCN_E_INVALID;
    *out = e->stats;
    return STCN_OK;
}
int stcn_get_flops(const stcn_engine *e, double *flops) {
    if (!e || !flops) return STCN_E_INVALID;
    double t = 0;
    for (int i = 0; i < STCN_K_COUNT; ++i) t += e->prof.flops[i];
    *flops = t;
    return STCN_OK;
}
int stcn_engine_set_profiling(stcn_engine *e, int on) {
    if (!e) return STCN_E_INVALID;
    e->prof.on = on != 0;
    return STCN_OK;
}
int stcn_get_kernel_ms(const stcn_engine *e, float *ms, int32_t *launches) {
    if (!e || !ms) return STCN_E_INVALID;
    stcn_engine *me = const_cast<stcn_engine *>(e);
    const int rc = me->prof.collect(ms);
    if (launches) for (int i = 0; i < STCN_K_COUNT; ++i) launches[i] = e->prof.launches[i];
    return rc;
}
int stcn_get_kernel_flops(const stcn_engine *e, double *flops) {
    if (!e || !flops) return STCN_E_INVALID;
    for (int i = 0; i < STCN_K_COUNT; ++i) flops[i] = e->prof.flops[i];
    return STCN_OK;
}
int stcn_get_kernel_exec_flops(const stcn_engine *e, double *flops) {
    if (!e || !flops) return STCN_E_INVALID;
    for (int i = 0; i < STCN_K_COUNT; ++i) flops[i] = e->prof.exec_flops[i];
    return STCN_OK;
}
int stcn_get_kernel_bytes(const stcn_engine *e, double *bytes) {
    if (!e || !bytes) return STCN_E_INVALID;
    for (int i = 0; i < STCN_K_COUNT; ++i) bytes[i] = e->prof.bytes[i];
    return STCN_OK;
}
int stcn_get_conv_regimes(stcn_engine *e, double *out) {
    if (!e || !out) return STCN_E_INVALID;
    float ms[STCN_K_COUNT];
    if (e->prof.on) { int rc = e->prof.collect(ms); if (rc) return rc; }
    out[0] = e->prof.hbm_conv_flops; out[1] = e->prof.hbm_conv_bytes; out[2] = e->prof.hbm_conv_ms; out[3] = e->prof.hbm_conv_launches;
    out[4] = e->prof.wino2_flops; out[5] = e->prof.wino4_flops;
    return STCN_OK;
}

}
```

### eva_vos_amd/csrc/engine.h

```cpp
#pragma once
#include <hip/hip_runtime.h>

#include <deque>
#include <map>
#include <memory>
#include <set>
#include <string>
#include <vector>

#include "../../include/stcn_hip.h"
#include "kernels.h"

namespace stcn {

void set_error(const char *fmt, ...);
struct Model;
struct ConvW;
hipError_t pool_malloc(void **p, size_t bytes);
void pool_free(void *p);
void pool_release();
bool wants_wino(const ConvW &cw);
bool wants_wino4(const ConvW &cw);
bool wants_wino_fusion12(const ConvW &cw);
int make_wino(Model &m, ConvW &cw, const std::vector<float> &w_host);
int make_wino4(Model &m, ConvW &cw, const std::vector<float> &w_host);
int make_wino_fusion12(Model &m, ConvW &cw, const std::vector<float> &w_host);
#define HIPCHK(x)                                                                          \
    do {                                                                                   \
        hipError_t e_ = (x);                                                               \
        if (e_ != hipSuccess) {                                                            \
            set_error("%s:%d %s -> %s", __FILE__, __LINE__, #x, hipGetErrorString(e_));    \
            return STCN_E_HIP;                                                             \
        }                                                                                  \
    } while (0)

struct ConvW {
    float *w = nullptr, *bias = nullptr;
    float *wino_u = nullptr;
    float *wino4_u = nullptr;
    float bias0 = 0.f;
    int cout = 0, cin = 0, cin_p = 0, kh = 0, kw = 0, K = 0, Kp = 0;
};

struct Model {
    int device = 0;
    std::map<std::string, ConvW> conv;
    CbamW cbam{};
    bool has_prop = false;
    bool has_fuse = false;
    int top_k = MEMREAD_MAX_TOPK;
    float km = 0.f;
    int wino4_min_wg = 100;
    std::vector<void *> allocs;
    const ConvW &c(const std::string &name) const;
};

struct Dims {
    int nh, nw, h2, w2, h4, w4, h8, w8, h16, w16;
    long npix;
    int hw2, hw4, hw8, hw16;
    void set(int nh_, int nw_) {
        nh = nh_; nw = nw_;
        h2 = nh / 2; w2 = nw / 2; h4 = nh / 4; w4 = nw / 4; h8 = nh / 8; w8 = nw / 8; h16 = nh / 16; w16 = nw / 16;
        npix = (long)nh * nw; hw2 = h2 * w2; hw4 = h4 * w4; hw8 = h8 * w8; hw16 = h16 * w16;
    }
};

struct Prof {
    bool on = false;
    double flops[STCN_K_COUNT] = {0};
    double bytes[STCN_K_COUNT] = {0};
    double exec_flops[STCN_K_COUNT] = {0};
    int launches[STCN_K_COUNT] = {0};
    struct Ev { int cls; bool hbm; hipEvent_t a, b; };
    std::deque<Ev> events;
    std::vector<hipEvent_t> pool;
    void reset();
    void begin(int cls, hipStream_t s);
    hipEvent_t *attach(int cls, bool hbm_bound_conv = false);
    double hbm_conv_flops = 0, hbm_conv_bytes = 0, hbm_conv_ms = 0; int hbm_conv_launches = 0;
    double wino2_flops = 0, wino4_flops = 0;
    void end(hipStream_t s);
    int collect(float *ms);
    ~Prof();
private:
    Ev &push_pair(int cls, bool hbm);
};

size_t wino_v_capacity(const Dims &d, int maxb);
struct Work {
    Dims d{};
    int k = 0;
    size_t S = 0;
    float *A = nullptr, *B = nullptr, *C = nullptr, *D = nullptr;
    float *splitk = nullptr; size_t splitk_floats = 0;
    float *wino_v = nullptr; size_t wino_v_floats = 0;
    float *cbam = nullptr;
    float *readout = nullptr;
    float *logit4 = nullptr;
    float *flogit = nullptr;
    float *agg = nullptr;
    float *agg_alt = nullptr;
    float *pooled = nullptr, *amap = nullptr, *attn = nullptr;
    float *cand_v = nullptr; int32_t *cand_i = nullptr, *cand_n = nullptr;
    float *gmax = nullptr, *tau = nullptr;
    int32_t *centre = nullptr;
    float *qk = nullptr;
    float *vin = nullptr;
    Prof *prof = nullptr;
    Knobs kn = Knobs::from_env();
    int conv_cls = STCN_K_CONV;
    std::vector<void *> allocs;
    int init(int nh, int nw, int k, int key_batch = 1, int group = 1);
    void release();
};

struct KeyOut { float *k16, *msq, *f16_thin, *f16, *s8, *s4, *f8_copy, *f4_copy, *dthin = nullptr, *cthin = nullptr; };
void inject_failure_after(int n);
int launch_status(const char *what);
const char *last_conv_path();
void set_conv_path(const char *s);
void conv_trace(int on);
const char *conv_trace_get();
constexpr long CONV_DENSE = -1;
struct ConvArgs {
    const float *x0 = nullptr, *x1 = nullptr;
    int c0 = 0, c1 = 0;
    long bs0 = CONV_DENSE, bs1 = 0;
    int B = 1, H = 0, W = 0, stride = 1;
    float *y = nullptr; long y_bs = 0;
    const float *res = nullptr; long res_bs = CONV_DENSE; int res_bmod = 0;
    int relu_in = 0, relu_out = 0, force_splitk = 0;
    ConvArgs(const float *x, int c, int B_, int H_, int W_, long bs = CONV_DENSE) : x0(x), c0(c), bs0(bs), B(B_), H(H_), W(W_) {}
    ConvArgs &concat(const float *x, int c, long bs) { x1 = x; c1 = c; bs1 = bs; return *this; }
    ConvArgs &strided(int s) { stride = s; return *this; }
    ConvArgs &out(float *y_, long bs = 0) { y = y_; y_bs = bs; return *this; }
    ConvArgs &residual(const float *r, long bs = CONV_DENSE, int bmod = 0) { res = r; res_bs = bs; res_bmod = bmod; return *this; }
    ConvArgs &relu(int in, int out_) { relu_in = in; relu_out = out_; return *this; }
    ConvArgs &splitk(int k) { force_splitk = k; return *this; }
};
int plan_conv(const Model &m, const Work &w, const std::string &name, const ConvArgs &a, ConvP &p, ConvPlan &pl);
const char *format_conv_path(const ConvPlan &pl, char *out, size_t n);
int run_conv(const Model &m, Work &w, hipStream_t s, const std::string &name, const ConvArgs &a);
struct SweepGroup {
    int first;
    int t_lo;
    int G;
    bool inserts;
};
std::vector<SweepGroup> plan_sweep(int idx, int closest, int mem_freq, int cap);
constexpr int MAX_DECODE_GROUP = 8;
int encode_key(const Model &m, Work &w, hipStream_t s, const float *img4, const KeyOut &o, int B = 1, long out_bs = 0);
int encode_value(const Model &m, Work &w, hipStream_t s, const float *img4, const float *f16,
                 const float *masks, long mask_stride, float *out, long out_bs, const float *vd = nullptr,
                 const float *vc = nullptr);
int value_frame_parts(const Model &m, Work &w, hipStream_t s, const float *f16, float *vd, float *vc);
int decode(const Model &m, Work &w, hipStream_t s, const float *readout, const float *f16_thin,
           const float *s8, const float *s4, float *agg, long agg_stride, const float *dthin = nullptr,
           const float *cthin = nullptr, int G = 1, long slot_bs = 0, long agg_gs = 0);
int decode_logit4(const Model &m, Work &w, hipStream_t s, const float *readout, const float *f16_thin, const float *s8, const float *s4,
                  const float *dthin = nullptr, const float *cthin = nullptr, int G = 1, long slot_bs = 0);
int fusion_logit(const Model &m, Work &w, hipStream_t s, const float *img4, const float *prev,
                 const float *curr, const float *attn2, float nc, float nr, float *logit);

long stage_grow(long cap, long need);

}

struct stcn_model { stcn::Model m; };

struct stcn_engine {
    const stcn::Model *model = nullptr;
    hipStream_t stream = nullptr;
    int T = 0, H = 0, W = 0, k = 0, mem_freq = 5;
    stcn_engine_opts opts{-1, -1, -1, -1};
    int lw = 0, uw = 0, lh = 0, uh = 0;
    stcn::Dims d{};
    float *images4 = nullptr;
    std::shared_ptr<void> images_owner;
    float *prob = nullptr;
    uint8_t *masks = nullptr;
    int n_slots = 0;
    std::vector<int> slot_of;
    std::vector<char> vparts_ready;
    int n_cached = 0;
    float *cache = nullptr; size_t slot_floats = 0;
    int bank_cap = 0, n_certain = 0;
    float *bank_k = nullptr, *bank_msq = nullptr, *bank_v = nullptr;
    int32_t *bank_centre = nullptr;
    std::vector<void *> retired;
    hipEvent_t retire_ev = nullptr;
    std::set<int> interacted;
    float *mask_pad = nullptr, *pos = nullptr, *neg = nullptr;
    stcn::Work work;
    hipStream_t side = nullptr;
    stcn::Work work_side;
    hipStream_t stream2 = nullptr;
    stcn::Work work2;
    hipEvent_t ev_fork = nullptr, ev_join = nullptr;
    int bank_lo = 0;
    std::vector<hipEvent_t> key_ready;
    std::vector<char> key_pending;
    int lookahead = 0;
    bool fuse_side = false;
    hipEvent_t ev_dec[2] = {nullptr, nullptr}, ev_fuse[2] = {nullptr, nullptr};
    char fuse_pending[2] = {0, 0};
    int agg_buf = 0;
    int key_batch = 1;
    int group = 1;
    stcn::Prof prof;
    stcn_stats stats{};
    std::string failed;
    std::vector<void *> allocs;
};
```

### eva_vos_amd/csrc/hooks.cpp

```cpp
#include <algorithm>
#include <climits>
#include <cmath>
#include <cstdlib>
#include <cstring>
#include <string>
#include <vector>

#include "engine.h"

using namespace stcn;
#define RC(x) do { int rc_ = (x); if (rc_) return rc_; } while (0)

namespace {
struct TmpWork {
    Work w;
    int rc;
    TmpWork(int nh, int nw, int k) { rc = w.init(nh, nw, k); }
    ~TmpWork() { (void)hipDeviceSynchronize(); w.release(); }
};
struct DevBuf {
    float *p = nullptr;
    int alloc(size_t floats) { HIPCHK(hipMalloc((void **)&p, floats * 4)); return STCN_OK; }
    ~DevBuf() { if (p) { (void)hipDeviceSynchronize(); (void)hipFree(p); } }
};
ConvW test_convw(int Cin, int Cout, int KH, int KW) {
    ConvW cw;
    cw.cout = Cout; cw.cin = Cin; cw.cin_p = Cin; cw.kh = KH; cw.kw = KW;
    cw.K = KH * KW * Cin; cw.Kp = (cw.K + 31) / 32 * 32;
    return cw;
}
size_t test_wino_v_floats(int B, int OH, int OW, int Cin) {
    const size_t v2 = (size_t)16 * Cin * (((size_t)B * ((OH + 1) / 2) * ((OW + 1) / 2) + 63) / 64 * 64);
    const size_t v4 = (size_t)36 * Cin * (((size_t)B * ((OH + 3) / 4) * ((OW + 3) / 4) + 127) / 128 * 128);
    return v2 > v4 ? v2 : v4;
}
struct ConvRig {
    Model m;
    Work w;
    DevBuf wv, ws;
    ~ConvRig() { (void)hipDeviceSynchronize(); for (void *p : m.allocs) (void)hipFree(p); }
    int init(ConvW cw, const std::vector<float> *hw, bool f4, int B, int OH, int OW, size_t slab_floats) {
        if (hw) {
            RC(make_wino(m, cw, *hw));
            RC(make_wino_fusion12(m, cw, *hw));
            if (f4) RC(make_wino4(m, cw, *hw));
            w.wino_v_floats = test_wino_v_floats(B, OH, OW, cw.cin_p);
            RC(wv.alloc(w.wino_v_floats));
            w.wino_v = wv.p;
        }
        m.conv["t"] = cw;
        w.splitk_floats = slab_floats;
        RC(ws.alloc(w.splitk_floats));
        w.splitk = ws.p;
        return STCN_OK;
    }
};
int plan_test_conv(int B, int H, int W, int Cin, int Cout, int K, int stride, int flags, int splitk, ConvP &p, ConvPlan &pl) {
    static float buf[4];
    Model m;
    ConvW cw = test_convw(Cin, Cout, K, K);
    cw.w = cw.bias = buf;
    const int OH = (H + 2 * (K / 2) - K) / stride + 1, OW = (W + 2 * (K / 2) - K) / stride + 1;
    Work w;
    if (K == 3 && stride == 1) {
        if (wants_wino(cw) || wants_wino_fusion12(cw)) cw.wino_u = buf;
        if (flags & 4) { if (wants_wino4(cw)) cw.wino4_u = buf; m.wino4_min_wg = 0; }
        w.wino_v_floats = test_wino_v_floats(B, OH, OW, Cin);
        w.wino_v = buf;
    }
    m.conv["t"] = cw;
    w.splitk_floats = (size_t)16 * 1024 * 1024;
    w.splitk = buf;
    return plan_conv(m, w, "t", ConvArgs(buf, Cin, B, H, W).strided(stride).out(buf).relu(flags & 1, (flags >> 1) & 1).splitk(splitk), p, pl);
}
struct ReadRig {
    DevBuf msq, cv, ci, cn, gm, tau, qsq, cen;
    MemReadKm km{};
    MemRead r{};
    MemReadScratch scr{};
    int init(const char *who, hipStream_t s, const float *mk, const float *mv, const float *qk, int N, int Q, int k, int top_k, int h16, int w16,
             float sigma, int32_t *centres, int32_t *topk_idx, float *topk_w, float *readout) {
        const bool bad = !mk || !mv || !qk || !readout || top_k < 1 || top_k > STCN_MAX_TOP_K || N < top_k || Q < 1 || k < 1;
        if (bad) { set_error("%s: bad arguments (1 <= top_k <= %d, N >= top_k; top_k=%d N=%d)", who, STCN_MAX_TOP_K, top_k, N); return STCN_E_INVALID; }
        const bool with_km = h16 != 0 || w16 != 0 || sigma != 0.f || centres;
        const bool km_ok = std::isfinite(sigma) && sigma > 0.f && h16 >= 1 && w16 >= 1 && h16 < 32768 && w16 < 32768 && (long)h16 * w16 <= Q && Q % (h16 * w16) == 0;
        if (with_km && !km_ok) { set_error("%s_km: bad arguments (km > 0 finite, Q a multiple of h16 * w16; km=%f h16=%d w16=%d Q=%d)", who, (double)sigma, h16, w16, Q); return STCN_E_INVALID; }
        const MemReadScratchSizes sz = memread_scratch_floats(Q);
        RC(msq.alloc((size_t)N + MEMREAD_MSQ_PAD)); RC(cv.alloc(sz.cand_v)); RC(ci.alloc(sz.cand_i)); RC(cn.alloc(sz.cand_n)); RC(gm.alloc(sz.gmax)); RC(tau.alloc(sz.tau));
        scr = MemReadScratch{cv.p, reinterpret_cast<int32_t *>(ci.p), reinterpret_cast<int32_t *>(cn.p), gm.p, tau.p};
        if (with_km) {
            RC(qsq.alloc(Q)); RC(cen.alloc((size_t)(Q / (h16 * w16)) * memread_centre_stride(N)));
            rowsumsq_launch(qk, Q, 64, qsq.p, s);
            km = MemReadKm{sigma, h16, w16, qsq.p, (long)h16 * w16, reinterpret_cast<int32_t *>(cen.p), centres};
        }
        HIPCHK(hipMemsetAsync(msq.p, 0, ((size_t)N + MEMREAD_MSQ_PAD) * 4, s));
        rowsumsq_launch(mk, N, 64, msq.p, s);
        r.mk = mk; r.msq = msq.p; r.mv = mv; r.mv_os = (long)N * 512; r.N = N; r.qk = qk; r.Q = Q; r.k = k; r.top_k = top_k;
        r.readout = readout; r.ro_os = (long)Q * 512; r.topk_idx = topk_idx; r.topk_w = topk_w; r.km = with_km ? &km : nullptr;
        return STCN_OK;
    }
};
void export_memread_plan(int N, int Q, int32_t *plan7) {
    const MemReadPlan pl = memread_plan(N, Q);
    const int32_t v[7] = {pl.steps, pl.ss, pl.ns, pl.nc1, pl.spc1, pl.nc2, pl.spc2};
    for (int i = 0; i < 7; ++i) plan7[i] = v[i];
}
struct SmallKernel { const char *name; int nptr, ni, nf; unsigned wide; };
const SmallKernel SMALL_KERNELS[] = {
    {"maxpool3x3s2", 2, 4, 0, 0}, {"upsample2x_add", 3, 6, 0, 1u << 4}, {"up4_sigmoid_aggregate", 2, 8, 0, 1u << 3 | 1u << 4 | 1u << 6 | 1u << 7},
    {"up4_sigmoid", 2, 3, 0, 0}, {"sigmoid_aggregate", 2, 3, 0, 1u << 1 | 1u << 2}, {"argmax", 2, 3, 0, 1u << 2}, {"rowsumsq", 2, 5, 0, 1u << 3 | 1u << 4},
    {"pack_image", 2, 6, 0, 0}, {"pack_value_input", 3, 3, 0, 1u << 0}, {"pack_fusion_input", 5, 1, 2, 1u << 0}, {"interact_mask", 5, 9, 0, 1u << 7},
    {"cbam", 7, 3, 1, 0}, {"copy_rows", 2, 4, 0, 1u << 0 | 1u << 1 | 1u << 3}, {"copy2", 4, 2, 0, 1u << 0 | 1u << 1}, {"fill", 1, 1, 1, 1u << 0},
};
}

extern "C" {

int stcn_test_conv(void *stream, const float *x, const float *wgt, const float *bias, const float *res, float *y, int B,
                   int H, int W, int Cin, int Cout, int KH, int KW, int stride, int pad, int flags, int splitk) {
    return stcn_test_conv_ex(stream, x, wgt, bias, res, y, B, H, W, Cin, Cout, KH, KW, stride, pad, flags, splitk, nullptr, 0, CONV_DENSE, CONV_DENSE,
                             CONV_DENSE, 0, CONV_DENSE);
}

int stcn_test_conv_ex(void *stream, const float *x, const float *wgt, const float *bias, const float *res, float *y, int B,
                      int H, int W, int Cin, int Cout, int KH, int KW, int stride, int pad, int flags, int splitk,
                      const float *x1, int c1, long bs0, long bs1, long res_bs, int res_bmod, long y_bs) {
    if (!x || !wgt || !y || B < 1 || H < 1 || W < 1 || Cin < 4 || Cout < 1 || stride < 1 || Cin % 4 || pad != KH / 2 || KH != KW) {
        set_error("stcn_test_conv_ex: x, w and y, B, H, W, Cout, stride >= 1, Cin%%4==0, square kernel, pad=K/2 required"); return STCN_E_INVALID;
    }
    if ((x1 != nullptr) != (c1 > 0) || c1 % 4 || bs0 < CONV_DENSE || bs1 < CONV_DENSE || res_bs < CONV_DENSE || res_bmod < 0 || y_bs < CONV_DENSE) {
        set_error("stcn_test_conv_ex: a second source has c1 > 0 channels (c1%%4==0); strides are -1 (dense), 0 (broadcast) or elements; res_bmod >= 0");
        return STCN_E_INVALID;
    }
    hipStream_t s = (hipStream_t)stream;
    ConvW cw = test_convw(Cin + c1, Cout, KH, KW);
    DevBuf wpad;
    RC(wpad.alloc((size_t)Cout * cw.Kp));
    HIPCHK(hipMemsetAsync(wpad.p, 0, (size_t)Cout * cw.Kp * 4, s));
    HIPCHK(hipMemcpy2DAsync(wpad.p, (size_t)cw.Kp * 4, wgt, (size_t)cw.K * 4, (size_t)cw.K * 4, Cout, hipMemcpyDeviceToDevice, s));
    cw.w = wpad.p; cw.bias = const_cast<float *>(bias);
    const int OH = (H + 2 * pad - KH) / stride + 1, OW = (W + 2 * pad - KW) / stride + 1;
    const bool wino = KH == 3 && stride == 1 && !x1;
    std::vector<float> hw;
    if (wino) {
        HIPCHK(hipStreamSynchronize(s));
        hw.resize((size_t)Cout * cw.Kp);
        HIPCHK(hipMemcpy(hw.data(), wpad.p, hw.size() * 4, hipMemcpyDeviceToHost));
    }
    ConvRig r;
    RC(r.init(cw, wino ? &hw : nullptr, flags & 4, B, OH, OW, (size_t)16 * 1024 * 1024));
    if (wino && (flags & 4)) r.m.wino4_min_wg = 0;
    if (Cout == 1) {
        const bool dense = !x1 && bs0 == CONV_DENSE && y_bs == CONV_DENSE && !res;
        if (stride != 1 || !dense) { set_error("Cout==1 path is stride 1, one dense source, dense output, no residual"); return STCN_E_INVALID; }
        float b0 = 0.f;
        if (bias) HIPCHK(hipMemcpy(&b0, bias, 4, hipMemcpyDeviceToHost));
        conv_n1_launch(x, wpad.p, b0, y, B, H, W, Cin, KH, flags & 1, s);
        set_conv_path("n1");
    } else {
        RC(run_conv(r.m, r.w, s, "t", ConvArgs(x, Cin, B, H, W, bs0).concat(x1, c1, x1 ? bs1 : 0).strided(stride).out(y, y_bs == CONV_DENSE ? 0 : y_bs)
                                          .residual(res, res_bs, res_bmod).relu(flags & 1, (flags >> 1) & 1).splitk(splitk)));
    }
    HIPCHK(hipStreamSynchronize(s));
    HIPCHK(hipGetLastError());
    return STCN_OK;
}

int stcn_test_conv_path(int B, int H, int W, int Cin, int Cout, int K, int stride, int flags, int splitk, char *out, int n) {
    if (Cin % 4 || !out || n < 1) { set_error("stcn_test_conv_path: Cin%%4==0 and an output buffer required"); return STCN_E_INVALID; }
    ConvP p;
    ConvPlan pl;
    RC(plan_test_conv(B, H, W, Cin, Cout, K, stride, flags, splitk, p, pl));
    format_conv_path(pl, out, (size_t)n);
    return STCN_OK;
}

int stcn_test_conv_plan(int B, int H, int W, int Cin, int Cout, int K, int stride, int flags, int splitk, int32_t *iv, int n, double *dv) {
    if (Cin % 4 || !iv || n < STCN_CONV_PLAN_INTS || !dv) { set_error("stcn_test_conv_plan: Cin%%4==0, STCN_CONV_PLAN_INTS ints and 2 doubles required"); return STCN_E_INVALID; }
    ConvP p;
    ConvPlan pl;
    RC(plan_test_conv(B, H, W, Cin, Cout, K, stride, flags, splitk, p, pl));
    const bool w2 = pl.family == CONV_WINO2, w4 = pl.family == CONV_WINO4, direct = pl.family == CONV_DIRECT;
    const WinoGeom g = w2 || w4 ? pl.geo : WinoGeom{};
    const W4Plan q = w4 ? pl.w4 : W4Plan{};
    const int32_t v[STCN_CONV_PLAN_INTS] = {
        pl.family, pl.splitk, pl.ppw, pl.tail, pl.n_in, pl.n_gemm, pl.reduce,
        g.TH, g.TW, g.Mt, g.Mt_pad, g.KB, w2 ? pl.w2.kb_per_split : 0,
        q.mb, q.tiles_m, q.tiles_n, q.grid, q.full_wg, q.pieces, q.per, q.chunks, q.tm_per_chunk,
        direct ? p.tile_big : 0, direct ? p.rem_full : 0, direct ? p.rem_split : 0, direct ? p.rem_per : 0, direct ? p.chain : 0};
    for (int i = 0; i < STCN_CONV_PLAN_INTS; ++i) iv[i] = v[i];
    dv[0] = (double)pl.v_floats; dv[1] = pl.fl_exec;
    return STCN_OK;
}

int stcn_bench_conv(void *stream, int B, int H, int W, int Cin, int Cout, int KH, int KW, int stride, int pad, int splitk,
                    int iters, float *avg_ms, double *flops_per_launch) {
    hipStream_t s = (hipStream_t)stream;
    (void)pad;
    ConvW cw = test_convw(Cin, Cout, KH, KW);
    const int OH = (H + 2 * (KH / 2) - KH) / stride + 1, OW = (W + 2 * (KW / 2) - KW) / stride + 1;
    DevBuf x, wt, b, y;
    RC(x.alloc((size_t)B * H * W * Cin)); RC(wt.alloc((size_t)Cout * cw.Kp)); RC(b.alloc(Cout));
    RC(y.alloc((size_t)B * OH * OW * Cout));
    std::vector<float> h((size_t)B * H * W * Cin);
    unsigned st = 12345u;
    auto rnd = [&]() { st = st * 1664525u + 1013904223u; return ((st >> 8) & 0xffff) / 32768.f - 1.f; };
    for (auto &v : h) v = rnd();
    HIPCHK(hipMemcpy(x.p, h.data(), h.size() * 4, hipMemcpyHostToDevice));
    h.assign((size_t)Cout * cw.Kp, 0.f);
    for (auto &v : h) v = rnd() * 0.05f;
    HIPCHK(hipMemcpy(wt.p, h.data(), h.size() * 4, hipMemcpyHostToDevice));
    HIPCHK(hipMemsetAsync(b.p, 0, Cout * 4, s));
    cw.w = wt.p; cw.bias = b.p;
    ConvRig r;
    RC(r.init(cw, KH == 3 && stride == 1 ? &h : nullptr, getenv("STCN_BENCH_CONV_F4") != nullptr, B, OH, OW, (size_t)32 * 1024 * 1024));
    hipEvent_t e0, e1;
    HIPCHK(hipEventCreate(&e0)); HIPCHK(hipEventCreate(&e1));
    DevBuf resb;
    const long obs = (long)OH * OW * Cout;
    if (getenv("STCN_BENCH_CONV_RES")) { RC(resb.alloc((size_t)B * obs)); HIPCHK(hipMemsetAsync(resb.p, 0, (size_t)B * obs * 4, s)); }
    const ConvArgs args = ConvArgs(x.p, Cin, B, H, W).strided(stride).out(y.p).residual(resb.p).relu(0, 1).splitk(splitk);
    for (int i = 0; i < 3; ++i)
        RC(run_conv(r.m, r.w, s, "t", args));
    HIPCHK(hipEventRecord(e0, s));
    for (int i = 0; i < iters; ++i)
        RC(run_conv(r.m, r.w, s, "t", args));
    HIPCHK(hipEventRecord(e1, s));
    HIPCHK(hipEventSynchronize(e1));
    float ms = 0.f;
    HIPCHK(hipEventElapsedTime(&ms, e0, e1));
    (void)hipEventDestroy(e0); (void)hipEventDestroy(e1);
    if (avg_ms) *avg_ms = ms / iters;
    if (flops_per_launch) *flops_per_launch = 2.0 * B * OH * OW * (double)Cout * KH * KW * Cin;
    return STCN_OK;
}

static int pack_one(const float *img_chw, int nh, int nw, float *img4, hipStream_t s) {
    pack_image_launch(img_chw, img4, nh, nw, nh, nw, 0, 0, s);
    return STCN_OK;
}

int stcn_test_encode_key(const stcn_model *m, void *stream, const float *img, int nh, int nw, float *k16, float *f16_thin,
                         float *f16, float *f8, float *f4) {
    if (!m || !img || nh % 16 || nw % 16) { set_error("stcn_test_encode_key: bad arguments"); return STCN_E_INVALID; }
    hipStream_t s = (hipStream_t)stream;
    TmpWork t(nh, nw, 1);
    RC(t.rc);
    const Dims &d = t.w.d;
    DevBuf img4, tf16, tk16, tmsq;
    RC(img4.alloc((size_t)d.npix * 4)); RC(tf16.alloc((size_t)d.hw16 * 1024)); RC(tk16.alloc((size_t)d.hw16 * 64));
    RC(tmsq.alloc(d.hw16));
    RC(pack_one(img, nh, nw, img4.p, s));
    KeyOut ko{k16 ? k16 : tk16.p, tmsq.p, f16_thin, f16 ? f16 : tf16.p, nullptr, nullptr, f8, f4, nullptr, nullptr};
    RC(encode_key(m->m, t.w, s, img4.p, ko));
    HIPCHK(hipStreamSynchronize(s));
    HIPCHK(hipGetLastError());
    return STCN_OK;
}

int stcn_test_encode_value(const stcn_model *m, void *stream, const float *img, const float *f16, const float *masks, int k,
                           int nh, int nw, float *out) {
    if (!m || !img || !f16 || !masks || !out || k < 1 || k > STCN_MAX_OBJECTS) { set_error("stcn_test_encode_value: bad arguments"); return STCN_E_INVALID; }
    hipStream_t s = (hipStream_t)stream;
    TmpWork t(nh, nw, k);
    RC(t.rc);
    DevBuf img4;
    RC(img4.alloc((size_t)t.w.d.npix * 4));
    RC(pack_one(img, nh, nw, img4.p, s));
    RC(encode_value(m->m, t.w, s, img4.p, f16, masks, t.w.d.npix, out, 0));
    HIPCHK(hipStreamSynchronize(s));
    HIPCHK(hipGetLastError());
    return STCN_OK;
}

int stcn_test_memory_read(void *stream, const float *mk, const float *mv, const float *qk, int N, int Q, int k,
                          int32_t *topk_idx, float *topk_w, float *readout) {
    return stcn_test_memory_read_k(stream, mk, mv, qk, N, Q, k, STCN_MAX_TOP_K, topk_idx, topk_w, readout);
}

int stcn_test_memory_read_k(void *stream, const float *mk, const float *mv, const float *qk, int N, int Q, int k, int top_k,
                            int32_t *topk_idx, float *topk_w, float *readout) {
    return stcn_test_memory_read_km(stream, mk, mv, qk, N, Q, k, top_k, 0, 0, 0.f, nullptr, topk_idx, topk_w, readout);
}

int stcn_test_memory_read_km(void *stream, const float *mk, const float *mv, const float *qk, int N, int Q, int k, int top_k, int h16, int w16,
                             float km, int32_t *centres, int32_t *topk_idx, float *topk_w, float *readout) {
    hipStream_t s = (hipStream_t)stream;
    ReadRig rig;
    RC(rig.init("stcn_test_memory_read", s, mk, mv, qk, N, Q, k, top_k, h16, w16, km, centres, topk_idx, topk_w, readout));
    memory_read_launch(rig.r, rig.scr, s);
    HIPCHK(hipStreamSynchronize(s));
    HIPCHK(hipGetLastError());
    return STCN_OK;
}

int stcn_bench_memory_read(void *stream, const float *mk, const float *mv, const float *qk, int N, int Q, int k, int iters,
                           float *readout, float *ms, int32_t *plan7) {
    return stcn_bench_memory_read_k(stream, mk, mv, qk, N, Q, k, STCN_MAX_TOP_K, iters, readout, ms, plan7);
}

int stcn_bench_memory_read_k(void *stream, const float *mk, const float *mv, const float *qk, int N, int Q, int k, int top_k, int iters,
                             float *readout, float *ms, int32_t *plan7) {
    return stcn_bench_memory_read_km(stream, mk, mv, qk, N, Q, k, top_k, 0, 0, 0.f, iters, readout, ms, plan7);
}

int stcn_bench_memory_read_km(void *stream, const float *mk, const float *mv, const float *qk, int N, int Q, int k, int top_k, int h16, int w16,
                              float km, int iters, float *readout, float *ms, int32_t *plan7) {
    hipStream_t s = (hipStream_t)stream;
    if (!ms || iters < 1) { set_error("stcn_bench_memory_read: bad arguments (ms and iters >= 1 required; top_k=%d N=%d)", top_k, N); return STCN_E_INVALID; }
    ReadRig rig;
    RC(rig.init("stcn_bench_memory_read", s, mk, mv, qk, N, Q, k, top_k, h16, w16, km, nullptr, nullptr, nullptr, readout));
    hipEvent_t e0, e1;
    HIPCHK(hipEventCreate(&e0)); HIPCHK(hipEventCreate(&e1));
    for (int it = 0; it < 2; ++it) memory_read_launch(rig.r, rig.scr, s);
    HIPCHK(hipEventRecord(e0, s));
    for (int it = 0; it < iters; ++it) memory_read_launch(rig.r, rig.scr, s);
    HIPCHK(hipEventRecord(e1, s));
    HIPCHK(hipEventSynchronize(e1));
    HIPCHK(hipEventElapsedTime(ms, e0, e1));
    *ms /= (float)iters;
    (void)hipEventDestroy(e0); (void)hipEventDestroy(e1);
    if (plan7) export_memread_plan(N, Q, plan7);
    HIPCHK(hipGetLastError());
    return STCN_OK;
}

int stcn_test_sweep_plan(int idx, int closest, int mem_freq, int cap, int32_t *out, int n, int32_t *count) {
    if (mem_freq < 1 || cap < 1 || n < 0 || (n > 0 && !out) || !count) { set_error("stcn_test_sweep_plan: bad arguments"); return STCN_E_INVALID; }
    const std::vector<SweepGroup> groups = plan_sweep(idx, closest, mem_freq, cap);
    *count = (int32_t)groups.size();
    for (int i = 0; i < n && i < (int)groups.size(); ++i) {
        const SweepGroup &g = groups[i];
        const int32_t v[4] = {g.first, g.t_lo, g.G, g.inserts ? 1 : 0};
        for (int j = 0; j < 4; ++j) out[4 * i + j] = v[j];
    }
    return STCN_OK;
}

int stcn_memread_plan(int N, int Q, int32_t *plan7) {
    if (!plan7 || N < 1 || Q < 1) { set_error("stcn_memread_plan: bad arguments"); return STCN_E_INVALID; }
    export_memread_plan(N, Q, plan7);
    return STCN_OK;
}

int stcn_memread_scratch(int Q, int64_t *sizes5) {
    if (!sizes5 || Q < 1) { set_error("stcn_memread_scratch: bad arguments"); return STCN_E_INVALID; }
    const MemReadScratchSizes sz = memread_scratch_floats(Q);
    for (size_t i = 0, v[5] = {sz.cand_v, sz.cand_i, sz.cand_n, sz.gmax, sz.tau}; i < 5; ++i) sizes5[i] = (int64_t)v[i];
    return STCN_OK;
}

int stcn_test_decode(const stcn_model *m, void *stream, const float *readout, const float *f16_thin, const float *f8,
                     const float *f4, int k, int nh, int nw, float *logit4, float *agg) {
    if (!m || !readout || !f16_thin || !f8 || !f4 || !agg) { set_error("stcn_test_decode: bad arguments"); return STCN_E_INVALID; }
    hipStream_t s = (hipStream_t)stream;
    TmpWork t(nh, nw, k);
    RC(t.rc);
    const Dims &d = t.w.d;
    DevBuf s8, s4;
    RC(s8.alloc((size_t)d.hw8 * 512)); RC(s4.alloc((size_t)d.hw4 * 256));
    RC(run_conv(m->m, t.w, s, "decoder.up_16_8.skip_conv", ConvArgs(f8, 512, 1, d.h8, d.w8, 0).out(s8.p)));
    RC(run_conv(m->m, t.w, s, "decoder.up_8_4.skip_conv", ConvArgs(f4, 256, 1, d.h4, d.w4, 0).out(s4.p)));
    RC(decode(m->m, t.w, s, readout, f16_thin, s8.p, s4.p, agg, d.npix));
    if (logit4) HIPCHK(hipMemcpyAsync(logit4, t.w.logit4, (size_t)k * d.hw4 * 4, hipMemcpyDeviceToDevice, s));
    HIPCHK(hipStreamSynchronize(s));
    HIPCHK(hipGetLastError());
    return STCN_OK;
}

int stcn_test_attention(void *stream, const float *mk, const float *qk, const float *pos, const float *neg, int kk, int nh,
                        int nw, float *attn) {
    if (!mk || !qk || !pos || !neg || !attn || kk < 1 || kk > STCN_MAX_OBJECTS + 1) { set_error("stcn_test_attention: bad arguments"); return STCN_E_INVALID; }
    hipStream_t s = (hipStream_t)stream;
    const int h = nh / 16, w = nw / 16;
    DevBuf msq, pooled, amap, gm, part;
    RC(gm.alloc((size_t)256 * h * w)); RC(part.alloc(attention_part_floats(kk, h * w)));
    RC(msq.alloc(h * w + MEMREAD_MSQ_PAD)); RC(pooled.alloc((size_t)std::max(20, attention_nchp(2 * kk)) * h * w)); RC(amap.alloc((size_t)kk * 2 * h * w));
    HIPCHK(hipMemsetAsync(msq.p, 0, (size_t)(h * w + MEMREAD_MSQ_PAD) * 4, s));
    rowsumsq_launch(mk, h * w, 64, msq.p, s);
    attention_read_launch(mk, msq.p, qk, pos, neg, kk, h, w, pooled.p, amap.p, attn, AttnScratch{gm.p, part.p}, s);
    HIPCHK(hipStreamSynchronize(s));
    HIPCHK(hipGetLastError());
    return STCN_OK;
}

int stcn_test_fusion(const stcn_model *m, void *stream, const float *img, const float *prev, const float *curr,
                     const float *attn, float nc, float nr, int nh, int nw, float *logit) {
    if (!m || !img || !prev || !curr || !attn || !logit) { set_error("stcn_test_fusion: bad arguments"); return STCN_E_INVALID; }
    hipStream_t s = (hipStream_t)stream;
    TmpWork t(nh, nw, 1);
    RC(t.rc);
    DevBuf img4;
    RC(img4.alloc((size_t)t.w.d.npix * 4));
    RC(pack_one(img, nh, nw, img4.p, s));
    RC(fusion_logit(m->m, t.w, s, img4.p, prev, curr, attn, nc, nr, logit));
    HIPCHK(hipStreamSynchronize(s));
    HIPCHK(hipGetLastError());
    return STCN_OK;
}

static int bound_radius(int H, int W) { return (int)std::ceil(0.008 * std::sqrt((double)H * H + (double)W * W)); }

static bool metric_args_ok(const char *who, bool has_k, int k, int T, int H, int W, int min_hw, std::initializer_list<const void *> ptrs) {
    if (has_k && (k < 1 || k > STCN_MAX_OBJECTS)) { set_error("%s: k = %d outside 1..%d (STCN_MAX_OBJECTS)", who, k, STCN_MAX_OBJECTS); return false; }
    if (T < 1 || H < min_hw || W < min_hw) { set_error("%s: bad shape (T >= 1, H, W >= %d required; T=%d H=%d W=%d)", who, min_hw, T, H, W); return false; }
    for (const void *p : ptrs)
        if (!p) { set_error("%s: null pointer", who); return false; }
    return true;
}

int stcn_metrics_jf_counts(void *stream, const uint8_t *gt_dev, const uint8_t *pred_dev, int T, int H, int W,
                           int32_t *counts_dev, uint8_t *scratch_dev) {
    if (!metric_args_ok("stcn_metrics_jf_counts", false, 0, T, H, W, 2, {gt_dev, pred_dev, counts_dev, scratch_dev})) return STCN_E_INVALID;
    jf_counts_launch(gt_dev, pred_dev, T, H, W, bound_radius(H, W), scratch_dev, counts_dev, (hipStream_t)stream);
    HIPCHK(hipGetLastError());
    return STCN_OK;
}

int stcn_metrics_j_counts(void *stream, const uint8_t *gt_dev, const uint8_t *pred_dev, int T, int H, int W, int32_t *counts_dev) {
    if (!metric_args_ok("stcn_metrics_j_counts", false, 0, T, H, W, 1, {gt_dev, pred_dev, counts_dev})) return STCN_E_INVALID;
    jf_counts_launch(gt_dev, pred_dev, T, H, W, -1, nullptr, counts_dev, (hipStream_t)stream);
    HIPCHK(hipGetLastError());
    return STCN_OK;
}

int stcn_metrics_objects_scratch(int k, int T, int H, int W, int64_t *bytes) {
    if (!metric_args_ok("stcn_metrics_objects_scratch", true, k, T, H, W, 2, {bytes})) return STCN_E_INVALID;
    *bytes = (int64_t)label_scratch_bytes(k, T, H, W);
    return STCN_OK;
}

int stcn_metrics_objects_jf_counts(void *stream, const uint8_t *gt_dev, const uint8_t *pred_dev, int k, int T, int H, int W, int32_t *counts_dev,
                                   void *scratch_dev) {
    if (!metric_args_ok("stcn_metrics_objects_jf_counts", true, k, T, H, W, 2, {gt_dev, pred_dev, counts_dev, scratch_dev})) return STCN_E_INVALID;
    label_counts_launch(gt_dev, pred_dev, k, T, H, W, bound_radius(H, W), scratch_dev, counts_dev, T, (hipStream_t)stream);
    HIPCHK(hipGetLastError());
    return STCN_OK;
}

int stcn_metrics_objects_j_counts(void *stream, const uint8_t *gt_dev, const uint8_t *pred_dev, int k, int T, int H, int W, int32_t *counts_dev) {
    if (!metric_args_ok("stcn_metrics_objects_j_counts", true, k, T, H, W, 2, {gt_dev, pred_dev, counts_dev})) return STCN_E_INVALID;
    label_counts_launch(gt_dev, pred_dev, k, T, H, W, -1, nullptr, counts_dev, T, (hipStream_t)stream);
    HIPCHK(hipGetLastError());
    return STCN_OK;
}

static int metrics_round(const char *who, bool labels, void *stream, const uint8_t *masks_dev, int nh, int nw, int lh, int lw, const uint8_t *gt_dev,
                         const uint8_t *annotated_dev, const uint8_t *flags_dev, int k, int T, int H, int W, int t0, int t1, int j_only, double no_object,
                         uint8_t *gen_dev, void *scratch_dev, int32_t *counts_dev, double *object_quality_dev, double *quality_dev, int32_t *select_dev) {
    const void *unused = who;
    if (!metric_args_ok(who, labels, k, T, H, W, 2, {masks_dev, gt_dev, annotated_dev, flags_dev, gen_dev, counts_dev, labels ? object_quality_dev : unused,
                                                    quality_dev, select_dev, j_only ? unused : scratch_dev}))
        return STCN_E_INVALID;
    if (lh < 0 || lw < 0 || lh + H > nh || lw + W > nw) { set_error("%s: the %d x %d crop at (%d, %d) leaves the %d x %d tensor", who, H, W, lh, lw, nh, nw); return STCN_E_INVALID; }
    if (t0 < 0 || t1 > T || t0 >= t1) { set_error("%s: frames [%d, %d) are not a non-empty range inside [0, %d)", who, t0, t1, T); return STCN_E_INVALID; }
    const size_t hw = (size_t)H * W;
    void *scratch = j_only ? nullptr : (char *)scratch_dev + (labels ? label_scratch_bytes(k, t0, H, W) : t0 * hw);
    round_score_launch(masks_dev + (size_t)t0 * nh * nw, nh, nw, lh, lw, gt_dev + t0 * hw, annotated_dev + t0, flags_dev, labels ? k : 0, t1 - t0, H, W,
                       j_only ? -1 : bound_radius(H, W), no_object, gen_dev + t0 * hw, scratch, counts_dev + (size_t)t0 * 6, T, object_quality_dev,
                       quality_dev, select_dev, (hipStream_t)stream, t0);
    HIPCHK(hipGetLastError());
    return STCN_OK;
}

int stcn_metrics_round(void *stream, const uint8_t *masks_dev, int nh, int nw, int lh, int lw, const uint8_t *gt_dev, const uint8_t *annotated_dev,
                       const uint8_t *noobj_dev, int T, int H, int W, int t0, int t1, int j_only, double no_object, uint8_t *gen_dev, uint8_t *scratch_dev,
                       int32_t *counts_dev, double *quality_dev, int32_t *select_dev) {
    return metrics_round("stcn_metrics_round", false, stream, masks_dev, nh, nw, lh, lw, gt_dev, annotated_dev, noobj_dev, 0, T, H, W, t0, t1, j_only,
                         no_object, gen_dev, scratch_dev, counts_dev, nullptr, quality_dev, select_dev);
}

int stcn_metrics_objects_round(void *stream, const uint8_t *masks_dev, int nh, int nw, int lh, int lw, const uint8_t *gt_dev,
                               const uint8_t *annotated_dev, const uint8_t *present_dev, int k, int T, int H, int W, int t0, int t1, int j_only,
                               double no_object, uint8_t *gen_dev, void *scratch_dev, int32_t *counts_dev, double *object_quality_dev,
                               double *quality_dev, int32_t *select_dev) {
    return metrics_round("stcn_metrics_objects_round", true, stream, masks_dev, nh, nw, lh, lw, gt_dev, annotated_dev, present_dev, k, T, H, W, t0, t1,
                         j_only, no_object, gen_dev, scratch_dev, counts_dev, object_quality_dev, quality_dev, select_dev);
}

int stcn_bench_mfma_rate(void *stream, int ms_target, float *tflops, float *ms_out) {
    if (!tflops || ms_target < 1 || ms_target > 2000) { set_error("stcn_bench_mfma_rate: bad arguments"); return STCN_E_INVALID; }
    hipStream_t s = (hipStream_t)stream;
    const int cus = device_cus();
    DevBuf out;
    RC(out.alloc(64));
    hipEvent_t e0, e1;
    HIPCHK(hipEventCreate(&e0)); HIPCHK(hipEventCreate(&e1));
    const int iters = ((int)(ms_target * 1000.0 / 1.15) + 3) / 4 * 4;
    (void)mfma_probe_launch(out.p, 2 * cus, (iters / 8 + 3) / 4 * 4, s);
    HIPCHK(hipEventRecord(e0, s));
    const double fl = mfma_probe_launch(out.p, 2 * cus, iters, s);
    HIPCHK(hipEventRecord(e1, s));
    HIPCHK(hipEventSynchronize(e1));
    float ms = 0.f;
    HIPCHK(hipEventElapsedTime(&ms, e0, e1));
    (void)hipEventDestroy(e0); (void)hipEventDestroy(e1);
    HIPCHK(hipGetLastError());
    *tflops = (float)(fl / (ms * 1e-3) / 1e12);
    if (ms_out) *ms_out = ms;
    return STCN_OK;
}

int stcn_test_kernel(const char *name, void *stream, void *const *ptrs, int nptr, const int64_t *iv, int ni, const double *fv, int nf) {
    const SmallKernel *k = nullptr;
    for (const SmallKernel &c : SMALL_KERNELS)
        if (name && !strcmp(name, c.name)) k = &c;
    if (!k) { set_error("stcn_test_kernel: unknown kernel '%s'", name ? name : "(null)"); return STCN_E_INVALID; }
    bool ok = nptr == k->nptr && ni == k->ni && nf == k->nf && ptrs && iv && (nf == 0 || fv);
    for (int i = 0; ok && i < nptr; ++i) ok = ptrs[i] != nullptr;
    for (int i = 0; ok && i < ni; ++i) ok = iv[i] >= 0 && iv[i] <= ((k->wide >> i) & 1 ? (1LL << 40) : (long long)INT_MAX);
    if (!ok) {
        set_error("stcn_test_kernel: '%s' takes %d non-null pointers, %d non-negative integers and %d doubles (got %d, %d, %d); sizes fit an int, strides 2^40",
                  k->name, k->nptr, k->ni, k->nf, nptr, ni, nf);
        return STCN_E_INVALID;
    }
    hipStream_t s = (hipStream_t)stream;
    const std::string n = k->name;
    auto F = [&](int i) { return static_cast<float *>(ptrs[i]); };
    auto I = [&](int i) { return (int)iv[i]; };
    auto objects = [&](int64_t v) { return v >= 1 && v <= STCN_MAX_OBJECTS; };
    auto bad = [&](const char *what) { set_error("stcn_test_kernel: '%s' needs %s", k->name, what); return STCN_E_INVALID; };
    DevBuf scratch;
    if (n == "maxpool3x3s2") {
        if (iv[3] % 4 || iv[3] < 4 || iv[1] < 2 || iv[2] < 2 || iv[0] < 1) return bad("B >= 1, H, W >= 2, C % 4 == 0");
        maxpool3x3s2_launch(F(0), F(1), I(0), I(1), I(2), I(3), s);
    } else if (n == "upsample2x_add") {
        if (iv[3] % 4 || iv[3] < 4 || iv[0] < 1 || iv[1] < 1 || iv[2] < 1) return bad("B, h, w >= 1, C % 4 == 0");
        upsample2x_add_launch(F(0), F(1), F(2), I(0), I(1), I(2), I(3), s, (long)iv[4], I(5));
    } else if (n == "up4_sigmoid_aggregate") {
        if (!objects(iv[0]) || iv[1] < 1 || iv[2] < 1 || iv[5] < 1) return bad("1 <= k <= STCN_MAX_OBJECTS, h4, w4, G >= 1");
        up4_sigmoid_aggregate_launch(F(0), I(0), I(1), I(2), F(1), (long)iv[3], s, (long)iv[4], I(5), (long)iv[6], (long)iv[7]);
    } else if (n == "up4_sigmoid") {
        if (!objects(iv[0]) || iv[1] < 1 || iv[2] < 1) return bad("1 <= k <= STCN_MAX_OBJECTS, h4, w4 >= 1");
        up4_sigmoid_launch(F(0), I(0), I(1), I(2), F(1), s);
    } else if (n == "sigmoid_aggregate") {
        if (!objects(iv[0]) || iv[1] < 1) return bad("1 <= k <= STCN_MAX_OBJECTS, npix >= 1");
        sigmoid_aggregate_launch(F(0), I(0), (long)iv[1], F(1), (long)iv[2], s);
    } else if (n == "argmax") {
        if (iv[0] < 1 || iv[0] > 256 || iv[1] < 1 || iv[2] < 1) return bad("1 <= kk <= 256 (uint8 masks), T, npix >= 1");
        argmax_launch(F(0), I(0), I(1), (long)iv[2], static_cast<uint8_t *>(ptrs[1]), s);
    } else if (n == "rowsumsq") {
        if (iv[0] < 1 || iv[1] % 4 || iv[1] < 4 || iv[2] < 1) return bad("n, B >= 1, C % 4 == 0");
        rowsumsq_launch(F(0), I(0), I(1), F(1), s, I(2), (long)iv[3], (long)iv[4]);
    } else if (n == "pack_image") {
        if (iv[0] < 1 || iv[1] < 1 || iv[4] + iv[1] > iv[3] || iv[5] + iv[0] > iv[2]) return bad("H, W >= 1, lh + H <= nh, lw + W <= nw");
        pack_image_launch(F(0), F(1), I(0), I(1), I(2), I(3), I(4), I(5), s);
    } else if (n == "pack_value_input") {
        if (!objects(iv[1]) || iv[2] < 1) return bad("1 <= k <= STCN_MAX_OBJECTS, npix >= 1");
        pack_value_input_launch(F(0), F(1), (long)iv[0], I(1), I(2), F(2), s);
    } else if (n == "pack_fusion_input") {
        if (iv[0] < 1) return bad("npix >= 1");
        pack_fusion_input_launch(F(0), F(1), F(2), F(3), (float)fv[0], (float)fv[1], (long)iv[0], F(4), s);
    } else if (n == "interact_mask") {
        if (iv[8] < 1 || (iv[0] != 1 && iv[0] != iv[8]) || iv[1] < 1 || iv[2] < 1 || iv[6] + iv[1] > iv[3] || iv[5] + iv[2] > iv[4])
            return bad("kk >= 1, mc 1 or kk, H, W >= 1, lh + H <= nh, lw + W <= nw");
        interact_mask_launch(F(0), I(0), I(1), I(2), I(3), I(4), I(5), I(6), F(1), (long)iv[7], I(8), F(2), F(3), F(4), s);
    } else if (n == "cbam") {
        if (iv[0] < 1 || iv[1] < 1 || iv[2] < 1) return bad("B, h, w >= 1");
        RC(scratch.alloc((size_t)iv[0] * (16 * 1024 + 512 + 2 * (size_t)(iv[1] * iv[2]))));
        cbam_launch(F(0), F(1), I(0), I(1), I(2), CbamW{F(2), F(3), F(4), F(5), F(6), (float)fv[0]}, scratch.p, s);
    } else if (n == "copy_rows") {
        if (iv[2] < 1 || iv[3] < 1) return bad("rows, n >= 1");
        copy_rows_launch(F(0), (long)iv[0], F(1), (long)iv[1], I(2), (long)iv[3], s);
    } else if (n == "copy2") {
        if (iv[0] % 4) return bad("na % 4 == 0");
        copy2_launch(F(0), F(1), (long)iv[0], F(2), F(3), (long)iv[1], s);
    } else {
        fill_launch(F(0), (float)fv[0], (long)iv[0], s);
    }
    HIPCHK(hipStreamSynchronize(s));
    HIPCHK(hipGetLastError());
    return STCN_OK;
}

}
```

### eva_vos_amd/csrc/kernels.h

```cpp
#pragma once
#include <hip/hip_runtime.h>
#include <stdint.h>

#include <cstdlib>

#include "../../include/stcn_hip.h"

namespace stcn {

struct FastDiv {
    unsigned magic, shift, d;
};
static inline FastDiv fastdiv_make(unsigned d) {
    FastDiv f{0, 0, d};
    if (d <= 1) return f;
    unsigned s = 0;
    while ((1ull << s) < d) ++s;
    f.magic = (unsigned)(((1ull << (31 + s)) / d) + 1);
    f.shift = s - 1;
    return f;
}
#if defined(__HIPCC__)
__device__ __forceinline__ int fastdiv(int x, const FastDiv f) {
    return f.d <= 1 ? x : (int)(__umulhi((unsigned)x, f.magic) >> f.shift);
}
__device__ __forceinline__ int xcd_contiguous_block(int bid, int nblk) {
    const int q8 = nblk >> 3, r8 = nblk & 7, xcd = bid & 7;
    return (xcd < r8 ? xcd * (q8 + 1) : r8 * (q8 + 1) + (xcd - r8) * q8) + (bid >> 3);
}
#endif

static inline int env_int(const char *name, int dflt) { const char *e = getenv(name); return e ? atoi(e) : dflt; }
static inline bool env_on(const char *name, bool dflt = true) { return env_int(name, dflt) != 0; }
int device_cus();

struct Knobs {
    int wino_min_cin = 128;
    int wino_ppw = 0;
    int wino4_chunk_mb = 160;
    int fusion_conv12 = 0;
    int fusion_wino = 1;
    int pw_chain = 2;
    static Knobs from_env();
};

struct ConvP {
    const float *x0, *x1;
    int c0, c1;
    long bs0, bs1;
    unsigned x0_bytes, x1_bytes, w_bytes;
    int B, H, W;
    int OH, OW;
    int KH, KW, stride, pad;
    int Cin;
    int M, N;
    int K, Kp;
    const float *w;
    const float *bias;
    const float *res;
    long res_bs;
    int res_bmod;
    float *y;
    long y_bs;
    int relu_in, relu_out;
    int splitk;
    float *partial;
    int rem_full, rem_split, rem_per;
    const float *wino_u;
    const float *wino4_u;
    FastDiv fd_ohw, fd_ow;
    FastDiv fd_cin, fd_kw;
    int pointwise;
    int affine_out;
    int tile_big;
    int panel;
    int chain;
    Knobs kn;
};
constexpr int W4_MAX_CHUNKS = 16;
struct WinoGeom { int TH, TW, Mt, Mt_pad, KB; };
struct W2Plan { int tiles_n, ntile, kb_per_split; };
struct W4Plan { int tiles_m, tiles_n, mb, grid, full_wg, pieces, per, chunks, tm_per_chunk, judge_wg; };
enum ConvFamily { CONV_LITERAL = 0, CONV_FUSION = 1, CONV_WINO4 = 2, CONV_WINO2 = 3, CONV_DIRECT = 4 };
struct ConvPlan {
    int family = CONV_LITERAL;
    bool fusion_wino = false;
    WinoGeom geo{};
    W4Plan w4{};
    W2Plan w2{};
    int splitk = 1;
    int ppw = 0;
    const char *variant = "";
    bool tail = false;
    size_t v_floats = 0;
    int n_in = 0, n_gemm = 1;
    bool reduce = false;
    double fl = 0;
    double fl_exec = 0;
};
void conv_plan(ConvP &p, int force_splitk, size_t workspace_floats, ConvPlan &pl);
void conv_launch(const ConvP &p, hipStream_t s, hipEvent_t *ev_gemm = nullptr, hipEvent_t *ev_red = nullptr);
void conv_reduce_launch(const ConvP &p, hipStream_t s, hipEvent_t *ev_red = nullptr);
bool wino_plan(const ConvP &p, size_t v_cap, size_t slab_floats, ConvPlan &pl);
void wino_launch(const ConvP &p, const ConvPlan &pl, float *V, hipStream_t s, hipEvent_t *ev_in = nullptr, hipEvent_t *ev_gemm = nullptr,
                 hipEvent_t *ev_red = nullptr);
void wino_transform_weights(const float *w, int N, int Cin, int Kp, float *U);
#ifndef W4_MIN_CIN
#define W4_MIN_CIN 64
#endif
bool wino4_plan(const ConvP &p, int min_wg, size_t v_cap, size_t slab_floats, ConvPlan &pl);
void wino4_launch(const ConvP &p, const ConvPlan &pl, float *V, hipStream_t s, hipEvent_t *const *ev_in = nullptr,
                  hipEvent_t *const *ev_gemm = nullptr, hipEvent_t *ev_red = nullptr);
void wino4_transform_weights(const float *w, int N, int Cin, int Kp, float *U);
bool wino_enabled();
int wino4_mode();

bool fusion_conv_plan(const ConvP &p, ConvPlan &pl);
void fusion_conv_launch(const ConvP &p, const ConvPlan &pl, hipStream_t s, hipEvent_t *ev_gemm = nullptr);

void conv_n1_launch(const float *x, const float *w, float bias, float *y, int B, int H, int W, int C,
                    int KH, int relu_in, hipStream_t s);

void maxpool3x3s2_launch(const float *x, float *y, int B, int H, int W, int C, hipStream_t s);
void pack_image_launch(const float *img_chw, float *out, int H, int W, int nh, int nw, int lw, int lh,
                       hipStream_t s);
void pack_value_input_launch(const float *img4, const float *masks, long mask_stride, int k, int npix,
                             float *out, hipStream_t s);
void upsample2x_add_launch(const float *x, const float *skip, float *u, int B, int h, int w, int C,
                           hipStream_t s, long skip_bs = 0, int skip_bmod = 0);
void up4_sigmoid_aggregate_launch(const float *logit4, int k, int h4, int w4, float *agg,
                                  long agg_stride, hipStream_t s, long obj_stride = 0, int G = 1, long logit_gs = 0, long agg_gs = 0);
void up4_sigmoid_launch(const float *logit4, int k, int h4, int w4, float *prob, hipStream_t s);
void aggregate_wbg_launch(const float *prob, int k, long npix, int keep_bg, int hard, float *out, hipStream_t s);
void sigmoid_aggregate_launch(const float *logit, int k, long npix, float *agg, long agg_stride,
                              hipStream_t s);
void argmax_launch(const float *prob, int kk, int T, long npix, uint8_t *masks, hipStream_t s);
void rowsumsq_launch(const float *x, int n, int C, float *out, hipStream_t s, int B = 1, long x_bs = 0, long out_bs = 0);
void fill_launch(float *p, float v, long n, hipStream_t s);
void spin_launch(int us, hipStream_t s);
void copy_rows_launch(const float *src, long src_stride, float *dst, long dst_stride, int rows, long n,
                      hipStream_t s);
void copy2_launch(const float *a, float *da, long na, const float *b, float *db, long nb, hipStream_t s);
void interact_mask_launch(const float *mask, int mc, int H, int W, int nh, int nw, int lw, int lh,
                          float *prob_idx, long prob_row_stride, int kk, float *padded, float *pos,
                          float *neg, hipStream_t s);

void planes_to_rows_launch(const float *planes, long ld, long planes_bs, float *rows, long rows_bs, int B, int R, int C, hipStream_t s);
void rows_to_planes_launch(const float *rows, long rows_bs, float *planes, long ld, long planes_bs, int B, int R, int C, hipStream_t s);

struct CbamW { const float *w1, *b1, *w2, *b2, *wsp; float bsp; };
void cbam_launch(const float *x, float *out, int B, int h, int w, const CbamW &cw, float *scratch,
                 hipStream_t s);

constexpr int MEMREAD_MAX_TOPK = 50;
struct MemReadPlan { int steps, ss, ns, nc1, spc1, nc2, spc2; };
MemReadPlan memread_plan(int N, int Q);
struct MemReadCost { double flop, bytes; };
MemReadCost memread_cost(int N, int Q, int k, int top_k, bool km);
struct MemReadScratch { float *cand_v; int32_t *cand_i; int32_t *cand_n; float *gmax; float *tau; };
struct MemReadScratchSizes { size_t cand_v, cand_i, cand_n, gmax, tau; };
MemReadScratchSizes memread_scratch_floats(int Q);
constexpr int MEMREAD_MSQ_PAD = 64;
void allow_big_lds(const void *kernel, size_t lds);
#if defined(__HIPCC__)
template <typename... KArgs, typename... Args>
static inline void launch(void (*kernel)(KArgs...), dim3 grid, dim3 block, size_t lds_bytes, hipStream_t s, hipEvent_t *ev, const Args &...args) {
    if (lds_bytes > 64 * 1024) allow_big_lds(reinterpret_cast<const void *>(kernel), lds_bytes);
    if (ev) hipExtLaunchKernelGGL(kernel, grid, block, lds_bytes, s, ev[0], ev[1], 0, args...);
    else hipLaunchKernelGGL(kernel, grid, block, lds_bytes, s, args...);
}
#endif
struct MemReadKm { float sigma; int h16, w16; const float *qsq; long qsq_fs; int32_t *centre; int32_t *centre_idx; };
long memread_centre_stride(int N);
struct MemRead {
    const float *mk, *msq, *mv; long mv_os; int N;
    const float *qk; int Q;
    int k, top_k;
    float *readout; long ro_os; int32_t *topk_idx; float *topk_w;
    const MemReadKm *km;
};
void memory_read_launch(const MemRead &r, const MemReadScratch &scr, hipStream_t s);
struct AttnScratch { float *gmax, *part; };
int attention_nchp(int nch);
size_t attention_part_floats(int kk, int hw);
void attention_pool_launch(const float *pos, const float *neg, int kk, int h, int w, float *pooled, hipStream_t s);
void attention_read_launch(const float *mk, const float *msq, const float *qk, const float *pos,
                           const float *neg, int kk, int h, int w, float *pooled, float *amap,
                           float *attn, AttnScratch scr, hipStream_t s);
void pack_fusion_input_launch(const float *img4, const float *prev, const float *curr,
                              const float *attn2, float nc, float nr, long npix, float *out,
                              hipStream_t s);

void jf_counts_launch(const uint8_t *gt, const uint8_t *pred, int T, int H, int W, int radius, uint8_t *bmap,
                      int *counts, hipStream_t s);

size_t label_scratch_bytes(int k, int T, int H, int W);
void label_counts_launch(const uint8_t *gt, const uint8_t *pred, int k, int Tn, int H, int W, int radius, void *bsets, int *counts, int T_all,
                         hipStream_t s);
void round_score_launch(const uint8_t *masks, int nh, int nw, int lh, int lw, const uint8_t *gt, const uint8_t *annotated, const uint8_t *flags, int k,
                        int Tn, int H, int W, int radius, double no_object, uint8_t *gen, void *scratch, int *counts, int T_all,
                        double *object_quality, double *quality, int *select, hipStream_t s, int t0);

double mfma_probe_launch(float *out, int grid, int iters, hipStream_t s);

}
```

### eva_vos_amd/csrc/winograd4.hip

```cpp
#include <hip/hip_ext.h>

#include <cstdio>
#include <cstdlib>
#include <type_traits>

#include "wino_common.h"

namespace stcn {

typedef float f32x4 __attribute__((ext_vector_type(4)));
typedef float f32x16 __attribute__((ext_vector_type(16)));

#ifdef STCN_W4_CLOCK
__device__ unsigned long long g_w4_clock[2 * 8192];
#if STCN_W4_CLOCK == 2
#define W4_MFMA(a_, b_, c_) w4_fake_mfma(a_, b_, c_)
#endif
#endif
#ifndef W4_MFMA
#define W4_MFMA(a_, b_, c_) __builtin_amdgcn_mfma_f32_32x32x2f32(a_, b_, c_, 0, 0, 0)
#endif

static constexpr int W4T = 32;
static constexpr int W4N = 32;
static constexpr int W4W = 12;

#if defined(STCN_W4_CLOCK) && STCN_W4_CLOCK == 2
__device__ __forceinline__ f32x16 w4_fake_mfma(float a, float b, f32x16 c) {
#pragma unroll
    for (int e = 0; e < 16; ++e) asm volatile("v_fma_f32 %0, %1, %2, %0" : "+v"(c[e]) : "v"(a), "v"(b));
    return c;
}
#endif

__device__ __forceinline__ void bt6(const f32x4 &d0, const f32x4 &d1, const f32x4 &d2, const f32x4 &d3, const f32x4 &d4, const f32x4 &d5,
                                    f32x4 &o0, f32x4 &o1, f32x4 &o2, f32x4 &o3, f32x4 &o4, f32x4 &o5) {
    o0 = d0 * 1.265625f - d2 * 2.8125f + d4;
    const f32x4 e1 = d4 - d2 * 2.25f, f1 = d3 * 0.75f - d1 * 1.6875f;
    o1 = e1 + f1;
    o2 = e1 - f1;
    const f32x4 e2 = d4 - d2 * 0.5625f, f2 = d3 * 1.5f - d1 * 0.84375f;
    o3 = e2 + f2;
    o4 = e2 - f2;
    o5 = d1 * 1.265625f - d3 * 2.8125f + d5;
}

__global__ __launch_bounds__(256) void wino4_input_kernel(const float *__restrict__ x, unsigned x_bytes, long x_bs, int H, int W, int C,
                                                          int relu_in, int TH, int TW, int Mt, int Mt_pad, int cb_per_chunk,
                                                          int tile_lo, int tile_hi, float *__restrict__ V) {
    const long i = xcd_contiguous_block((int)blockIdx.x, (int)gridDim.x) * 256L + threadIdx.x;
    const int c16 = (int)(i & 7);
    const long tile = tile_lo + (i >> 3);
    if (tile >= tile_hi) return;
    const int KB = C / 8, NCB = C / 32;
    const int cb0 = blockIdx.y * cb_per_chunk, cb1 = min(NCB, cb0 + cb_per_chunk);
    const bool live = tile < Mt;
    const int tpi = TH * TW;
    const int b = live ? (int)(tile / tpi) : 0;
    const int r = live ? (int)(tile - (long)b * tpi) : 0;
    const int ty = r / TW, tx = r - ty * TW;
    const int y0 = 4 * ty - 1, x0 = 4 * tx - 1;
    unsigned long long ok = 0;
#pragma unroll
    for (int yy = 0; yy < 6; ++yy)
#pragma unroll
        for (int xx = 0; xx < 6; ++xx)
            if (live && (unsigned)(y0 + yy) < (unsigned)H && (unsigned)(x0 + xx) < (unsigned)W) ok |= 1ull << (yy * 6 + xx);
    const __amdgpu_buffer_rsrc_t rx = __builtin_amdgcn_make_buffer_rsrc(const_cast<float *>(x), 0, x_bytes, 0x00020000);
    const int xoff = (int)((b * x_bs + ((long)y0 * W + x0) * C + 4 * c16) * 4);
    const long ps = ((long)KB * Mt_pad) << 3;
    const float lo = relu_in ? 0.f : -__builtin_inff();
    for (int cb = cb0; cb < cb1; ++cb) {
        f32x4 t[6][6];
#pragma unroll
        for (int xx = 0; xx < 6; ++xx) {
            f32x4 d[6];
#pragma unroll
            for (int yy = 0; yy < 6; ++yy) {
                const unsigned vo = ((ok >> (yy * 6 + xx)) & 1ull) ? (unsigned)(xoff + ((yy * W + xx) * C + 32 * cb) * 4) : 0x80000000u;
                f32x4 v = __builtin_bit_cast(f32x4, __builtin_amdgcn_raw_buffer_load_b128(rx, vo, 0, 0));
                v.x = fmaxf(v.x, lo); v.y = fmaxf(v.y, lo); v.z = fmaxf(v.z, lo); v.w = fmaxf(v.w, lo);
                d[yy] = v;
            }
            bt6(d[0], d[1], d[2], d[3], d[4], d[5], t[0][xx], t[1][xx], t[2][xx], t[3][xx], t[4][xx], t[5][xx]);
        }
        const int kb = cb * 4 + (c16 >> 1);
        float *base = V + (((long)kb * Mt_pad + tile) << 3) + 4 * (c16 & 1);
#pragma unroll
        for (int xi = 0; xi < 6; ++xi) {
            f32x4 v[6];
            bt6(t[xi][0], t[xi][1], t[xi][2], t[xi][3], t[xi][4], t[xi][5], v[0], v[1], v[2], v[3], v[4], v[5]);
            float *dst = base + (long)(xi * 6) * ps;
#pragma unroll
            for (int nu = 0; nu < 6; ++nu) *reinterpret_cast<f32x4 *>(dst + nu * ps) = v[nu];
        }
    }
}

struct Wino4G {
    const float *V, *U;
    unsigned v_bytes, u_bytes;
    int Mt, Mt_pad, KB, N;
    int TH, TW, OH, OW, B, M;
    const float *bias, *res;
    long res_bs; int res_bmod;
    float *y; long y_bs;
    int relu_out;
    FastDiv fd_tpi, fd_tw, fd_tiles_n;
    int full_wg, pieces, kb_per_piece;
    float *partial;
    int tm0;
    int xb_m, xb_n, xb_cols;
};

template <int MB>
__global__ __launch_bounds__(64 * W4W) void wino4_gemm_kernel(const Wino4G p, const int tiles_n) {
    constexpr int PPW = 3, WT = W4T * MB;
    extern __shared__ __attribute__((aligned(16))) float smem[];
    int swz, piece = -1, kb0 = 0, kb1 = p.KB;
    if (MB == 1 && p.pieces > 1 && (int)blockIdx.x >= p.full_wg) {
        const int j = xcd_contiguous_block((int)blockIdx.x - p.full_wg, (int)gridDim.x - p.full_wg);
        const int rt = j / p.pieces;
        piece = j - rt * p.pieces;
        swz = p.full_wg + rt;
        kb0 = piece * p.kb_per_piece;
        kb1 = min(p.KB, kb0 + p.kb_per_piece);
    } else {
        swz = xcd_contiguous_block((int)blockIdx.x, MB == 1 && p.pieces > 1 ? p.full_wg : (int)gridDim.x);
    }
    int tm_l = fastdiv(swz, p.fd_tiles_n), tn = swz - tm_l * tiles_n;
    if (p.xb_m > 0 && piece < 0) {
        const int per = p.xb_m * p.xb_n, blk = swz / per, in = swz - blk * per;
        const int bm_i = blk / p.xb_cols, bn_i = blk - bm_i * p.xb_cols, im = in / p.xb_n;
        tm_l = bm_i * p.xb_m + im;
        tn = bn_i * p.xb_n + (in - im * p.xb_n);
    }
    const int tm = tm_l + p.tm0;
    const int t = threadIdx.x, lane = t & 63, l31 = lane & 31, h = lane >> 5;
    const int wave = __builtin_amdgcn_readfirstlane(t >> 6);
    const int pos0 = PPW * wave;

    const __amdgpu_buffer_rsrc_t rv = __builtin_amdgcn_make_buffer_rsrc(const_cast<float *>(p.V), 0, p.v_bytes, 0x00020000);
    const __amdgpu_buffer_rsrc_t ru = __builtin_amdgcn_make_buffer_rsrc(const_cast<float *>(p.U), 0, p.u_bytes, 0x00020000);
    const unsigned vl = (unsigned)(l31 * 32 + h * 16);
    unsigned sa0[PPW], sb0[PPW];
#pragma unroll
    for (int pi = 0; pi < PPW; ++pi) {
        sa0[pi] = (unsigned)((((long)(pos0 + pi) * p.KB + kb0) * p.Mt_pad + tm * WT) * 32);
        sb0[pi] = (unsigned)((((long)(pos0 + pi) * p.KB + kb0) * p.N + tn * W4N) * 32);
    }
    const unsigned sa = (unsigned)p.Mt_pad * 32u, sb = (unsigned)p.N * 32u;

    f32x16 acc[PPW][MB];
#pragma unroll
    for (int pi = 0; pi < PPW; ++pi)
#pragma unroll
        for (int bi = 0; bi < MB; ++bi)
#pragma unroll
            for (int e = 0; e < 16; ++e) acc[pi][bi][e] = 0.f;

    const int nk = kb1 - kb0;
    auto load1 = [&](int k, int pi, f32x4 (&fa)[MB], f32x4 &fb) {
        const unsigned oa = sa0[pi] + (unsigned)k * sa, ob = sb0[pi] + (unsigned)k * sb;
#pragma unroll
        for (int bi = 0; bi < MB; ++bi) fa[bi] = __builtin_bit_cast(f32x4, __builtin_amdgcn_raw_buffer_load_b128(rv, vl, oa + bi * 1024u, 0));
        fb = __builtin_bit_cast(f32x4, __builtin_amdgcn_raw_buffer_load_b128(ru, vl, ob, 0));
    };
    auto compute1 = [&](int pi, const f32x4 (&fa)[MB], const f32x4 &fb) {
#pragma unroll
        for (int j = 0; j < 4; ++j)
#pragma unroll
            for (int bi = 0; bi < MB; ++bi) acc[pi][bi] = W4_MFMA(fa[bi][j], fb[j], acc[pi][bi]);
    };
#ifdef STCN_W4_CLOCK
    unsigned long long ck_t0 = 0, ck_r0 = 0;
    if (wave == 0) {
        __builtin_amdgcn_sched_barrier(0);
        ck_t0 = __builtin_amdgcn_s_memtime();
        ck_r0 = __builtin_amdgcn_s_memrealtime();
        __builtin_amdgcn_s_waitcnt(0xC07F);
        __builtin_amdgcn_sched_barrier(0);
    }
#endif
    if (MB == 1) {
        f32x4 fa[3][PPW][MB], fb[3][PPW];
        auto load = [&](int k, int set) {
#pragma unroll
            for (int pi = 0; pi < PPW; ++pi) load1(k, pi, fa[set][pi], fb[set][pi]);
        };
        auto compute = [&](int set) {
#pragma unroll
            for (int j = 0; j < 4; ++j)
#pragma unroll
                for (int pi = 0; pi < PPW; ++pi)
#pragma unroll
                    for (int bi = 0; bi < MB; ++bi)
                        acc[pi][bi] = W4_MFMA(fa[set][pi][bi][j], fb[set][pi][j], acc[pi][bi]);
        };
        load(0, 0);
        load(min(1, nk - 1), 1);
        int k = 0;
        for (; k + 2 < nk; k += 3) {
            load(k + 2, 2);
            __builtin_amdgcn_sched_barrier(0);
            compute(0);
            __builtin_amdgcn_sched_barrier(0);
            load(min(k + 3, nk - 1), 0);
            __builtin_amdgcn_sched_barrier(0);
            compute(1);
            __builtin_amdgcn_sched_barrier(0);
            load(min(k + 4, nk - 1), 1);
            __builtin_amdgcn_sched_barrier(0);
            compute(2);
            __builtin_amdgcn_sched_barrier(0);
        }
        if (k < nk) compute(0);
        if (k + 1 < nk) compute(1);
    } else {
        f32x4 fa[2][PPW], fb[2][PPW];
        auto loadA = [&](int k, int bi, f32x4 (&d)[PPW]) {
#pragma unroll
            for (int pi = 0; pi < PPW; ++pi)
                d[pi] = __builtin_bit_cast(f32x4, __builtin_amdgcn_raw_buffer_load_b128(rv, vl, sa0[pi] + (unsigned)k * sa + bi * 1024u, 0));
        };
        auto loadB = [&](int k, f32x4 (&d)[PPW]) {
#pragma unroll
            for (int pi = 0; pi < PPW; ++pi)
                d[pi] = __builtin_bit_cast(f32x4, __builtin_amdgcn_raw_buffer_load_b128(ru, vl, sb0[pi] + (unsigned)k * sb, 0));
        };
        auto comp = [&](int bi, const f32x4 (&a)[PPW], const f32x4 (&bb)[PPW]) {
#pragma unroll
            for (int j = 0; j < 4; ++j)
#pragma unroll
                for (int pi = 0; pi < PPW; ++pi) acc[pi][bi] = W4_MFMA(a[pi][j], bb[pi][j], acc[pi][bi]);
        };
        loadB(0, fb[0]);
        loadA(0, 0, fa[0]);
        for (int k = 0; k < nk; k += 2) {
            const int k2 = min(k + 2, nk - 2);
            loadA(k, 1, fa[1]);
            __builtin_amdgcn_sched_barrier(0);
            comp(0, fa[0], fb[0]);
            __builtin_amdgcn_sched_barrier(0);
            loadB(k + 1, fb[1]);
            loadA(k + 1, 0, fa[0]);
            __builtin_amdgcn_sched_barrier(0);
            comp(1, fa[1], fb[0]);
            __builtin_amdgcn_sched_barrier(0);
            loadA(k + 1, 1, fa[1]);
            __builtin_amdgcn_sched_barrier(0);
            comp(0, fa[0], fb[1]);
            __builtin_amdgcn_sched_barrier(0);
            loadB(k2, fb[0]);
            loadA(k2, 0, fa[0]);
            __builtin_amdgcn_sched_barrier(0);
            comp(1, fa[1], fb[1]);
            __builtin_amdgcn_sched_barrier(0);
        }
    }
#ifdef STCN_W4_CLOCK
    if (wave == 0) {
        __builtin_amdgcn_sched_barrier(0);
        const unsigned long long ck_t1 = __builtin_amdgcn_s_memtime(), ck_r1 = __builtin_amdgcn_s_memrealtime();
        __builtin_amdgcn_s_waitcnt(0xC07F);
        __builtin_amdgcn_sched_barrier(0);
        if (lane == 0 && blockIdx.x < 8192) { g_w4_clock[2 * blockIdx.x] = ck_t1 - ck_t0; g_w4_clock[2 * blockIdx.x + 1] = ck_r1 - ck_r0; }
    }
#endif
    const int chq = t & 7, tl = (t >> 3) & 31;
    const int jh = __builtin_amdgcn_readfirstlane(t >> 8);
    const int tpi = p.TH * p.TW, ohw = p.OH * p.OW;
    const int n = tn * W4N + 4 * chq;
    const bool kpiece = MB == 1 && piece >= 0;
    const float lo = p.relu_out ? 0.f : -__builtin_inff();
    const __amdgpu_buffer_rsrc_t rres = __builtin_amdgcn_make_buffer_rsrc(const_cast<float *>(p.res ? p.res : p.y), 0, -1, 0x00020000);
    const __amdgpu_buffer_rsrc_t ry = __builtin_amdgcn_make_buffer_rsrc(p.y, 0, -1, 0x00020000);
    const unsigned y_bs = (unsigned)(p.y_bs ? p.y_bs : (long)ohw * p.N);
#pragma unroll
    for (int half = 0; half < MB; ++half) {
        int toff = 32 * half + tl;
        asm volatile("" : "+v"(toff));
        const long gt = (long)tm * WT + toff;
        const bool work = jh < 2 && gt < p.Mt;
        const int gtc = (int)min(gt, (long)p.Mt - 1);
        const int b = fastdiv(gtc, p.fd_tpi);
        const int rr = gtc - b * tpi;
        const int ty = fastdiv(rr, p.fd_tw), tx = rr - ty * p.TW;
        unsigned prow[4], pcol[2];
#pragma unroll
        for (int i2 = 0; i2 < 4; ++i2) prow[i2] = (unsigned)(min(4 * ty + i2, p.OH - 1) * p.OW * p.N) * 4u;
#pragma unroll
        for (int j = 0; j < 2; ++j) pcol[j] = (unsigned)(min(4 * tx + 2 * jh + j, p.OW - 1) * p.N + n) * 4u;
        if (half) __syncthreads();
#pragma unroll
        for (int pi = 0; pi < PPW; ++pi)
#pragma unroll
            for (int r = 0; r < 16; ++r)
                smem[((pos0 + pi) * W4T + (r & 3) + 8 * (r >> 2) + 4 * h) * W4N + l31] = acc[pi][half][r];
        f32x4 yv[2][4], bv = {0.f, 0.f, 0.f, 0.f};
        if (p.bias && !kpiece) {
            int nb = n;
            asm volatile("" : "+v"(nb));
            bv = *reinterpret_cast<const f32x4 *>(p.bias + nb);
        }
        if (p.res && !kpiece && jh < 2) {
            const unsigned rb = (unsigned)(p.res_bmod ? b % p.res_bmod : b) * (unsigned)p.res_bs * 4u;
#pragma unroll
            for (int j = 0; j < 2; ++j)
#pragma unroll
                for (int i2 = 0; i2 < 4; ++i2)
                    yv[j][i2] = __builtin_bit_cast(f32x4, __builtin_amdgcn_raw_buffer_load_b128(rres, rb + prow[i2] + pcol[j], 0, 0));
        } else {
#pragma unroll
            for (int j = 0; j < 2; ++j)
#pragma unroll
                for (int i2 = 0; i2 < 4; ++i2) yv[j][i2] = f32x4{0.f, 0.f, 0.f, 0.f};
        }
        __syncthreads();
        if (!work) continue;
        auto zrow = [&](int xi, auto JH, f32x4 (&zr)[2]) {
            f32x4 m[6];
            int ro4 = (xi * 6 * W4T + tl) * (W4N / 4) + chq;
            asm volatile("" : "+v"(ro4));
#pragma unroll
            for (int nu = 0; nu < 6; ++nu) m[nu] = reinterpret_cast<const f32x4 *>(smem)[ro4 + nu * W4T * (W4N / 4)];
            if (decltype(JH)::value == 0) {
                zr[0] = m[0] + (m[1] + m[2]) + (m[3] + m[4]);
                zr[1] = (m[1] - m[2]) * 0.75f + (m[3] - m[4]) * 1.5f;
            } else {
                zr[0] = (m[1] + m[2]) * 0.5625f + (m[3] + m[4]) * 2.25f;
                zr[1] = (m[1] - m[2]) * 0.421875f + (m[3] - m[4]) * 3.375f + m[5];
            }
        };
        auto columns = [&](auto JH) {
            f32x4 za[2];
#pragma unroll
            for (int j = 0; j < 2; ++j)
#pragma unroll
                for (int i2 = 0; i2 < 4; ++i2) yv[j][i2] += bv;
            zrow(0, JH, za);
#pragma unroll
            for (int j = 0; j < 2; ++j) yv[j][0] += za[j];
            constexpr float c1[4] = {0.75f, -0.75f, 1.5f, -1.5f}, c2[4] = {0.5625f, 0.5625f, 2.25f, 2.25f},
                            c3[4] = {0.421875f, -0.421875f, 3.375f, -3.375f};
#pragma unroll
            for (int xi = 1; xi < 5; ++xi) {
                __builtin_amdgcn_sched_barrier(0);
                zrow(xi, JH, za);
#pragma unroll
                for (int j = 0; j < 2; ++j) {
                    yv[j][0] += za[j];
                    yv[j][1] += za[j] * c1[xi - 1];
                    yv[j][2] += za[j] * c2[xi - 1];
                    yv[j][3] += za[j] * c3[xi - 1];
                }
            }
            __builtin_amdgcn_sched_barrier(0);
            zrow(5, JH, za);
#pragma unroll
            for (int j = 0; j < 2; ++j) yv[j][3] += za[j];
        };
        if (jh == 0) columns(std::integral_constant<int, 0>{});
        else columns(std::integral_constant<int, 1>{});
        if (kpiece) {
            float *dst = p.partial + (((long)(swz - p.full_wg) * p.pieces + piece) * W4T + tl) * (16 * W4N) + 4 * chq;
#pragma unroll
            for (int j = 0; j < 2; ++j)
#pragma unroll
                for (int i2 = 0; i2 < 4; ++i2) *reinterpret_cast<f32x4 *>(dst + (i2 * 4 + 2 * jh + j) * W4N) = yv[j][i2];
            continue;
        }
        const unsigned yb = (unsigned)b * y_bs * 4u;
#pragma unroll
        for (int j = 0; j < 2; ++j)
#pragma unroll
            for (int i2 = 0; i2 < 4; ++i2) {
#pragma unroll
                for (int c = 0; c < 4; ++c) yv[j][i2][c] = fmaxf(yv[j][i2][c], lo);
                const bool ok = 4 * tx + 2 * jh + j < p.OW && 4 * ty + i2 < p.OH;
                __builtin_amdgcn_raw_buffer_store_b128(__builtin_bit_cast(__attribute__((__vector_size__(4 * sizeof(unsigned)))) unsigned, yv[j][i2]), ry,
                                                       ok ? yb + prow[i2] + pcol[j] : 0xFFFFFFFFu, 0, 0);
            }
    }
}

__global__ __launch_bounds__(256) void wino4_reduce_kernel(const Wino4G p, const int tiles_n) {
    const int rt = blockIdx.x >> 6, swz = p.full_wg + rt;
    const int tm = fastdiv(swz, p.fd_tiles_n), tn = swz - tm * tiles_n;
    const int n_l = threadIdx.x & 31;
    const int e = ((blockIdx.x & 63) << 3) + (threadIdx.x >> 5);
    const int tl = e >> 4, px = e & 15;
    const int n = tn * W4N + n_l;
    const long gt = (long)tm * W4T + tl;
    if (gt >= p.Mt) return;
    const int tpi = p.TH * p.TW, ohw = p.OH * p.OW;
    const int b = fastdiv((int)gt, p.fd_tpi);
    const int rr = (int)(gt - (long)b * tpi);
    const int ty = fastdiv(rr, p.fd_tw), tx = rr - ty * p.TW;
    const int oh = 4 * ty + (px >> 2), ow = 4 * tx + (px & 3);
    if (oh >= p.OH || ow >= p.OW) return;
    const float *src = p.partial + ((long)rt * p.pieces * W4T * 16 + e) * W4N + n_l;
    float pv[8];
#pragma unroll
    for (int s2 = 0; s2 < 8; ++s2) pv[s2] = src[(long)min(s2, p.pieces - 1) * (W4T * 16 * W4N)];
    const long po = ((long)oh * p.OW + ow) * p.N + n;
    const float rv = p.res ? p.res[(long)(p.res_bmod ? b % p.res_bmod : b) * p.res_bs + po] : 0.f;
    float v = 0.f;
#pragma unroll
    for (int s2 = 0; s2 < 8; ++s2) v += s2 < p.pieces ? pv[s2] : 0.f;
    v += (p.bias ? p.bias[n] : 0.f) + rv;
    p.y[(p.y_bs ? (long)b * p.y_bs : (long)b * ohw * p.N) + po] = fmaxf(v, p.relu_out ? 0.f : -__builtin_inff());
}

int wino4_mode() {
    static const int m = env_int("STCN_WINO4", 1);
    return m;
}

static KPieces wino4_small_pieces(int grid, int KB) {
    static const bool on = env_on("STCN_WINO4_SMALL");
    const int cus = device_cus();
    if (!on || grid * 2 > cus) return {1, KB};
    return k_pieces(cus / grid, KB, 8, 8);
}

static W4Plan wino4_gemm_plan(const ConvP &p, const WinoGeom &ge, size_t slab_floats) {
    static const int mb_env = env_int("STCN_WINO4_MB", 0);
    static const bool tail_on = env_on("STCN_WINO4_TAIL");
    const int cus = device_cus(), KB = ge.KB;
    W4Plan pl{};
    pl.tiles_n = p.N / W4N;
    pl.mb = mb_env == 1 || mb_env == 2 ? mb_env : ((ge.Mt_pad / (2 * W4T)) * pl.tiles_n >= 200 ? 2 : 1);
    pl.tiles_m = ge.Mt_pad / (W4T * pl.mb);
    pl.grid = pl.tiles_m * pl.tiles_n;
    pl.full_wg = pl.grid; pl.pieces = 1; pl.per = KB;
    const bool may_split = tail_on && pl.mb == 1 && p.partial;
    if (may_split) {
        const int full = pl.grid / cus * cus, rem = pl.grid - full;
        if (full >= cus && rem > 0 && rem <= cus / 2) {
            const KPieces kp = k_pieces(cus / rem, KB, 8, 8);
            if (kp.pieces > 1 && (size_t)rem * kp.pieces * W4T * 16 * W4N <= slab_floats) {
                pl.full_wg = full; pl.pieces = kp.pieces; pl.per = kp.per;
                pl.grid = full + rem * kp.pieces;
            }
        }
    }
    const int wg32 = (ge.Mt_pad / W4T) * pl.tiles_n;
    const KPieces small = wino4_small_pieces(wg32, KB);
    pl.judge_wg = wg32 * small.pieces;
    if (may_split && pl.pieces == 1 && small.pieces > 1 && (size_t)pl.grid * small.pieces * W4T * 16 * W4N <= slab_floats) {
        pl.full_wg = 0; pl.pieces = small.pieces; pl.per = small.per;
        pl.grid *= small.pieces;
    }
    pl.chunks = 1; pl.tm_per_chunk = pl.tiles_m;
    const long chunk_bytes = (long)p.kn.wino4_chunk_mb << 20;
    const long vbytes = 36L * p.Cin * ge.Mt_pad * 4;
    if (pl.mb == 2 && chunk_bytes > 0 && vbytes > chunk_bytes * 3 / 2) {
        const int rounds = (pl.grid + cus - 1) / cus;
        const int n = (int)((vbytes + chunk_bytes - 1) / chunk_bytes);
        const int rpc = (rounds + n - 1) / n;
        int tmpc = rpc * cus / pl.tiles_n;
        tmpc = tmpc < 1 ? 1 : tmpc;
        if (tmpc < pl.tiles_m && (pl.tiles_m + tmpc - 1) / tmpc <= W4_MAX_CHUNKS) { pl.tm_per_chunk = tmpc; pl.chunks = (pl.tiles_m + tmpc - 1) / tmpc; }
    }
    return pl;
}

bool wino4_plan(const ConvP &p, int min_wg, size_t v_cap, size_t slab_floats, ConvPlan &cp) {
    if (!wino4_mode() || !p.wino4_u || p.KH != 3 || p.KW != 3 || p.stride != 1 || p.x1) return false;
    if (p.Cin % 32 || p.Cin < W4_MIN_CIN || p.N % W4N || p.bs0 == 0) return false;
    const WinoGeom ge = wino_geom(p, 4, 2 * W4T);
    if (!wino_extents_ok(p, 36, ge.Mt_pad)) return false;
    const W4Plan w4 = wino4_gemm_plan(p, ge, slab_floats);
    if (wino4_mode() < 2 && w4.judge_wg < min_wg) return false;
    const size_t need = (size_t)36 * p.Cin * ge.Mt_pad;
    if (need > v_cap) return false;
    cp.family = CONV_WINO4;
    cp.geo = ge; cp.w4 = w4;
    cp.v_floats = need;
    cp.n_in = cp.n_gemm = w4.chunks; cp.reduce = w4.pieces > 1;
    cp.fl_exec = 2.0 * (double)need * p.N;
    return true;
}

void wino4_launch(const ConvP &p, const ConvPlan &cp, float *V, hipStream_t s, hipEvent_t *const *ev_in, hipEvent_t *const *ev_gemm,
                  hipEvent_t *ev_red) {
    const W4Plan &pl = cp.w4;
    const WinoGeom &ge = cp.geo;
    const int tiles_n = pl.tiles_n, mb = pl.mb, tiles_m = pl.tiles_m;
    Wino4G g{};
    wino_fill_desc(g, p, ge, 36, V, p.wino4_u, tiles_n);
    g.full_wg = pl.full_wg; g.pieces = pl.pieces; g.kb_per_piece = pl.per; g.partial = p.partial;
    g.xb_m = g.xb_n = g.xb_cols = 0;
    {
        const int rows = pl.full_wg / tiles_n;
        if (pl.chunks == 1 && pl.full_wg % 8 == 0 && rows * tiles_n == pl.full_wg && tiles_n >= 8) {
            const int per = pl.full_wg / 8;
            int best = 0, best_sum = per % tiles_n == 0 ? per / tiles_n + tiles_n : rows + tiles_n;
            for (int bn = 2; bn <= tiles_n; ++bn) {
                if (per % bn || tiles_n % bn) continue;
                const int bm = per / bn;
                if (bm < 1 || rows % bm || (rows / bm) * (tiles_n / bn) != 8) continue;
                if (bm + bn < best_sum) { best_sum = bm + bn; best = bn; }
            }
            if (best && best != tiles_n) { g.xb_n = best; g.xb_m = per / best; g.xb_cols = tiles_n / best; }
        }
    }
    const size_t lds = (size_t)36 * W4T * W4N * sizeof(float);
    for (int c = 0; c < pl.chunks; ++c) {
        const int tm_lo = c * pl.tm_per_chunk, tm_hi = tm_lo + pl.tm_per_chunk < tiles_m ? tm_lo + pl.tm_per_chunk : tiles_m;
        const int tile_lo = tm_lo * W4T * mb, tile_hi = pl.chunks == 1 ? ge.Mt_pad : tm_hi * W4T * mb;
        hipEvent_t *ei = ev_in ? ev_in[c] : nullptr, *eg = ev_gemm ? ev_gemm[c] : nullptr;
        const WinoInGrid ig = wino_input_grid(tile_hi - tile_lo, p.Cin);
        launch(wino4_input_kernel, dim3(ig.gx, ig.chunks), dim3(256), 0, s, ei, p.x0, p.x0_bytes, p.bs0, p.H, p.W, p.Cin, p.relu_in, ge.TH, ge.TW,
               ge.Mt, ge.Mt_pad, ig.per, tile_lo, tile_hi, V);
        g.tm0 = tm_lo;
        if (mb == 2) {
            const int grid = (tm_hi - tm_lo) * tiles_n;
            launch(wino4_gemm_kernel<2>, dim3(grid), dim3(64 * W4W), lds, s, eg, g, tiles_n);
        } else {
            launch(wino4_gemm_kernel<1>, dim3(pl.grid), dim3(64 * W4W), lds, s, eg, g, tiles_n);
            if (g.pieces > 1) launch(wino4_reduce_kernel, dim3((tiles_m * tiles_n - g.full_wg) * 64), dim3(256), 0, s, ev_red, g, tiles_n);
        }
    }
}

void wino4_transform_weights(const float *w, int N, int Cin, int Kp, float *U) {
    static const double G[6][3] = {{64.0 / 81, 0, 0},
                                   {-128.0 / 243, -32.0 / 81, -8.0 / 27},
                                   {-128.0 / 243, 32.0 / 81, -8.0 / 27},
                                   {32.0 / 243, 16.0 / 81, 8.0 / 27},
                                   {32.0 / 243, -16.0 / 81, 8.0 / 27},
                                   {0, 0, 1}};
    wino_transform_weights_with(G, w, N, Cin, Kp, U);
}

#ifdef STCN_W4_CLOCK
extern "C" int stcn_debug_w4_clock(unsigned long long *host_out, int n_pairs) {
    return hipMemcpyFromSymbol(host_out, HIP_SYMBOL(g_w4_clock), (size_t)2 * (n_pairs < 8192 ? n_pairs : 8192) * sizeof(unsigned long long)) == hipSuccess ? 0 : 1;
}
#endif

}
```

Before: 802.6 frames/s.

## Add fused Winograd F(4,3) input+GEMM kernel and reuse transformed input across convs

Adds a fused Winograd-4 kernel for 64->64 channel convs that transforms input tiles in LDS while running the MFMA GEMM, removing the separate input-transform launch and its V buffer round trip. The fused path is off by default (knob wino4_fused=0). Also adds a default-on reuse of the transformed V buffer: key_comp, when it shares input with the preceding conv, skips the input-transform kernel via a tag check. The epilogue is refactored into a shared helper. The tag-based reuse risks stale data if the buffer is overwritten between calls.

```diff
diff --git a/eva_vos_amd/csrc/engine.cpp b/eva_vos_amd/csrc/engine.cpp
--- a/eva_vos_amd/csrc/engine.cpp
+++ b/eva_vos_amd/csrc/engine.cpp
@@ -32,6 +32,8 @@
     k.fusion_conv12 = env_int("STCN_FUSION_CONV12", k.fusion_conv12) != 0;
     k.fusion_wino = env_int("STCN_FUSION_WINO", k.fusion_wino) != 0;
     k.pw_chain = env_int("STCN_PW_CHAIN", k.pw_chain);
+    k.wino4_fused = env_int("STCN_WINO4_FUSED", k.wino4_fused) != 0;
+    k.wino4_reuse_v = env_int("STCN_WINO4_REUSE_V", k.wino4_reuse_v) != 0;
     return k;
 }
 
@@ -456,6 +458,7 @@
     switch (pl.family) {
     case CONV_FUSION: snprintf(out, n, "%s", pl.fusion_wino ? "fusion_wino" : "fusion_direct"); break;
     case CONV_WINO4: snprintf(out, n, "wino4 chunks=%d%s", pl.w4.chunks, pl.reduce ? " +tail" : ""); break;
+    case CONV_WINO4F: snprintf(out, n, "%s", "wino4_fused"); break;
     case CONV_WINO2: snprintf(out, n, "wino2 ppw=%d splitk=%d", pl.ppw, pl.splitk); break;
     case CONV_DIRECT: snprintf(out, n, "%s%s splitk=%d", pl.variant, pl.tail ? " +tail" : "", pl.splitk); break;
     default: snprintf(out, n, "%s", "");
@@ -504,11 +507,14 @@
                    ((long)p.M + 128) * p.N * 4 < (1L << 32);
     p.partial = w.splitk;
     p.kn = w.kn;
+    p.wino4_fused = a.wino4_fused;
     pl = ConvPlan{};
     pl.fl = 2.0 * p.M * p.N * (double)(cw.kh * cw.kw * cw.cin);
     if (a.force_splitk <= 0 && (fusion_conv_plan(p, pl) || wino4_plan(p, m.wino4_min_wg, w.wino_v_floats, w.splitk_floats, pl) ||
-                                wino_plan(p, w.wino_v_floats, w.splitk_floats, pl)))
+                                wino_plan(p, w.wino_v_floats, w.splitk_floats, pl))) {
+        if (pl.family == CONV_WINO4) wino4_fused_plan(p, pl);
         return STCN_OK;
+    }
     conv_plan(p, a.force_splitk, w.splitk_floats, pl);
     return STCN_OK;
 }
@@ -519,6 +525,16 @@
     const int rc = plan_conv(m, w, name, a, p, pl);
     if (rc) return rc;
     hipEvent_t *eg[W4_MAX_CHUNKS] = {}, *ei[W4_MAX_CHUNKS] = {}, *er = nullptr;
+    bool v_held = false;
+    {
+        Work::VTag tag{};
+        if (pl.family == CONV_WINO4 && pl.w4.chunks == 1) tag = Work::VTag{p.x0, p.bs0, p.B, p.H, p.W, p.Cin, p.relu_in, pl.geo.Mt_pad};
+        const Work::VTag &h = w.v_tag;
+        v_held = p.kn.wino4_reuse_v && a.same_x && tag.x && h.x == tag.x && h.bs == tag.bs && h.B == tag.B && h.H == tag.H && h.W == tag.W && h.Cin == tag.Cin &&
+                 h.relu_in == tag.relu_in && h.Mt_pad == tag.Mt_pad;
+        w.v_tag = tag;
+    }
+    const int n_in = v_held ? 0 : pl.n_in;
     if (w.prof) {
         const double in0 = (double)(p.bs0 ? p.B : 1) * p.H * p.W * p.c0, in1 = p.x1 ? (double)(p.bs1 ? p.B : 1) * p.H * p.W * p.c1 : 0.0;
         const double resb = p.res ? (p.res_bs ? (double)p.M * p.N : (double)p.OH * p.OW * p.N) : 0.0;
@@ -530,17 +546,18 @@
         w.prof->flops[cls] += pl.fl;
         w.prof->exec_flops[cls] += pl.fl_exec;
         if (hbm_acc) { w.prof->hbm_conv_bytes += bytes; w.prof->hbm_conv_flops += pl.fl; }
-        if (pl.family == CONV_WINO4) w.prof->wino4_flops += pl.fl; else if (pl.family == CONV_WINO2) w.prof->wino2_flops += pl.fl;
+        if (pl.family == CONV_WINO4 || pl.family == CONV_WINO4F) w.prof->wino4_flops += pl.fl; else if (pl.family == CONV_WINO2) w.prof->wino2_flops += pl.fl;
         for (int c = 0; c < pl.n_gemm; ++c) {
             eg[c] = w.prof->attach(cls, hbm_acc);
-            if (c < pl.n_in) ei[c] = w.prof->attach(STCN_K_WINO_INPUT);
+            if (c < n_in) ei[c] = w.prof->attach(STCN_K_WINO_INPUT);
         }
         if (pl.reduce) er = w.prof->attach(STCN_K_CONV_REDUCE);
     }
     if (g_trace_on) { char b[96]; g_trace += name; g_trace += '='; g_trace += format_conv_path(pl, b, sizeof(b)); g_trace += '\n'; }
     switch (pl.family) {
     case CONV_FUSION: fusion_conv_launch(p, pl, s, eg[0]); break;
-    case CONV_WINO4: wino4_launch(p, pl, w.wino_v, s, ei, eg, er); break;
+    case CONV_WINO4: wino4_launch(p, pl, w.wino_v, s, ei, eg, er, v_held); break;
+    case CONV_WINO4F: wino4_fused_launch(p, pl, s, eg[0]); break;
     case CONV_WINO2: wino_launch(p, pl, w.wino_v, s, ei[0], eg[0], er); break;
     default: conv_launch(p, s, eg[0], er);
     }
@@ -567,7 +584,7 @@
             const float *idt = x;
             if (i == 0) { RC(run_conv(m, w, s, p + ".downsample.0", ConvArgs(x, cin, B, H, W).strided(sd).out(w.D))); idt = w.D; }
             RC(run_conv(m, w, s, p + ".conv1", ConvArgs(x, cin, B, H, W).out(w.C).relu(0, 1)));
-            RC(run_conv(m, w, s, p + ".conv2", ConvArgs(w.C, st.planes, B, H, W).strided(sd).out(w.A).relu(0, 1)));
+            RC(run_conv(m, w, s, p + ".conv2", ConvArgs(w.C, st.planes, B, H, W).strided(sd).out(w.A).relu(0, 1).fused_input(si == 0)));
             float *dst = x;
             long dst_bs = 0;
             if (si == 2 && i == st.n - 1) { dst = o.f16; dst_bs = obs; }
@@ -589,7 +606,11 @@
             rowsumsq_launch(o.k16, d.hw16, 64, o.msq, s, B, out_bs, out_bs);
         }
     }
-    if (o.f16_thin) RC(run_conv(m, w, s, "key_comp", ConvArgs(o.f16, 1024, B, d.h16, d.w16, ibs).out(o.f16_thin, obs)));
+    if (o.f16_thin) {
+        ConvArgs kc = ConvArgs(o.f16, 1024, B, d.h16, d.w16, ibs).out(o.f16_thin, obs);
+        if (o.k16) kc.same_input();
+        RC(run_conv(m, w, s, "key_comp", kc));
+    }
     if (o.f16_thin && o.dthin) {
         RC(run_conv(m, w, s, "decoder.compress.downsample#b", ConvArgs(o.f16_thin, 512, B, d.h16, d.w16, ibs).out(o.dthin, obs)));
         RC(run_conv(m, w, s, "decoder.compress.conv1#b", ConvArgs(o.f16_thin, 512, B, d.h16, d.w16, ibs).out(o.cthin, obs).relu(1, 0)));
diff --git a/eva_vos_amd/csrc/engine.h b/eva_vos_amd/csrc/engine.h
--- a/eva_vos_amd/csrc/engine.h
+++ b/eva_vos_amd/csrc/engine.h
@@ -95,6 +95,7 @@
     float *A = nullptr, *B = nullptr, *C = nullptr, *D = nullptr;
     float *splitk = nullptr; size_t splitk_floats = 0;
     float *wino_v = nullptr; size_t wino_v_floats = 0;
+    struct VTag { const float *x = nullptr; long bs = 0; int B = 0, H = 0, W = 0, Cin = 0, relu_in = 0, Mt_pad = 0; } v_tag;
     float *cbam = nullptr;
     float *readout = nullptr;
     float *logit4 = nullptr;
@@ -131,6 +132,8 @@
     float *y = nullptr; long y_bs = 0;
     const float *res = nullptr; long res_bs = CONV_DENSE; int res_bmod = 0;
     int relu_in = 0, relu_out = 0, force_splitk = 0;
+    int wino4_fused = 0;
+    int same_x = 0;
     ConvArgs(const float *x, int c, int B_, int H_, int W_, long bs = CONV_DENSE) : x0(x), c0(c), bs0(bs), B(B_), H(H_), W(W_) {}
     ConvArgs &concat(const float *x, int c, long bs) { x1 = x; c1 = c; bs1 = bs; return *this; }
     ConvArgs &strided(int s) { stride = s; return *this; }
@@ -138,6 +141,8 @@
     ConvArgs &residual(const float *r, long bs = CONV_DENSE, int bmod = 0) { res = r; res_bs = bs; res_bmod = bmod; return *this; }
     ConvArgs &relu(int in, int out_) { relu_in = in; relu_out = out_; return *this; }
     ConvArgs &splitk(int k) { force_splitk = k; return *this; }
+    ConvArgs &fused_input(int on = 1) { wino4_fused = on; return *this; }
+    ConvArgs &same_input() { same_x = 1; return *this; }
 };
 int plan_conv(const Model &m, const Work &w, const std::string &name, const ConvArgs &a, ConvP &p, ConvPlan &pl);
 const char *format_conv_path(const ConvPlan &pl, char *out, size_t n);
diff --git a/eva_vos_amd/csrc/hooks.cpp b/eva_vos_amd/csrc/hooks.cpp
--- a/eva_vos_amd/csrc/hooks.cpp
+++ b/eva_vos_amd/csrc/hooks.cpp
@@ -71,7 +71,8 @@
     m.conv["t"] = cw;
     w.splitk_floats = (size_t)16 * 1024 * 1024;
     w.splitk = buf;
-    return plan_conv(m, w, "t", ConvArgs(buf, Cin, B, H, W).strided(stride).out(buf).relu(flags & 1, (flags >> 1) & 1).splitk(splitk), p, pl);
+    return plan_conv(m, w, "t", ConvArgs(buf, Cin, B, H, W).strided(stride).out(buf).relu(flags & 1, (flags >> 1) & 1).splitk(splitk).fused_input((flags >> 3) & 1),
+                     p, pl);
 }
 struct ReadRig {
     DevBuf msq, cv, ci, cn, gm, tau, qsq, cen;
@@ -159,7 +160,8 @@
         set_conv_path("n1");
     } else {
         RC(run_conv(r.m, r.w, s, "t", ConvArgs(x, Cin, B, H, W, bs0).concat(x1, c1, x1 ? bs1 : 0).strided(stride).out(y, y_bs == CONV_DENSE ? 0 : y_bs)
-                                          .residual(res, res_bs, res_bmod).relu(flags & 1, (flags >> 1) & 1).splitk(splitk)));
+                                          .residual(res, res_bs, res_bmod).relu(flags & 1, (flags >> 1) & 1).splitk(splitk)
+                                          .fused_input((flags >> 3) & 1)));
     }
     HIPCHK(hipStreamSynchronize(s));
     HIPCHK(hipGetLastError());
@@ -180,7 +182,7 @@
     ConvP p;
     ConvPlan pl;
     RC(plan_test_conv(B, H, W, Cin, Cout, K, stride, flags, splitk, p, pl));
-    const bool w2 = pl.family == CONV_WINO2, w4 = pl.family == CONV_WINO4, direct = pl.family == CONV_DIRECT;
+    const bool w2 = pl.family == CONV_WINO2, w4 = pl.family == CONV_WINO4 || pl.family == CONV_WINO4F, direct = pl.family == CONV_DIRECT;
     const WinoGeom g = w2 || w4 ? pl.geo : WinoGeom{};
     const W4Plan q = w4 ? pl.w4 : W4Plan{};
     const int32_t v[STCN_CONV_PLAN_INTS] = {
@@ -219,7 +221,8 @@
     DevBuf resb;
     const long obs = (long)OH * OW * Cout;
     if (getenv("STCN_BENCH_CONV_RES")) { RC(resb.alloc((size_t)B * obs)); HIPCHK(hipMemsetAsync(resb.p, 0, (size_t)B * obs * 4, s)); }
-    const ConvArgs args = ConvArgs(x.p, Cin, B, H, W).strided(stride).out(y.p).residual(resb.p).relu(0, 1).splitk(splitk);
+    const ConvArgs args = ConvArgs(x.p, Cin, B, H, W).strided(stride).out(y.p).residual(resb.p).relu(0, 1).splitk(splitk)
+                              .fused_input(env_int("STCN_BENCH_CONV_FUSED", 0) != 0);
     for (int i = 0; i < 3; ++i)
         RC(run_conv(r.m, r.w, s, "t", args));
     HIPCHK(hipEventRecord(e0, s));
diff --git a/eva_vos_amd/csrc/kernels.h b/eva_vos_amd/csrc/kernels.h
--- a/eva_vos_amd/csrc/kernels.h
+++ b/eva_vos_amd/csrc/kernels.h
@@ -41,6 +41,8 @@
     int fusion_conv12 = 0;
     int fusion_wino = 1;
     int pw_chain = 2;
+    int wino4_fused = 0;
+    int wino4_reuse_v = 1;
     static Knobs from_env();
 };
 
@@ -75,13 +77,14 @@
     int tile_big;
     int panel;
     int chain;
+    int wino4_fused;
     Knobs kn;
 };
 constexpr int W4_MAX_CHUNKS = 16;
 struct WinoGeom { int TH, TW, Mt, Mt_pad, KB; };
 struct W2Plan { int tiles_n, ntile, kb_per_split; };
 struct W4Plan { int tiles_m, tiles_n, mb, grid, full_wg, pieces, per, chunks, tm_per_chunk, judge_wg; };
-enum ConvFamily { CONV_LITERAL = 0, CONV_FUSION = 1, CONV_WINO4 = 2, CONV_WINO2 = 3, CONV_DIRECT = 4 };
+enum ConvFamily { CONV_LITERAL = 0, CONV_FUSION = 1, CONV_WINO4 = 2, CONV_WINO2 = 3, CONV_DIRECT = 4, CONV_WINO4F = 5 };
 struct ConvPlan {
     int family = CONV_LITERAL;
     bool fusion_wino = false;
@@ -110,7 +113,9 @@
 #endif
 bool wino4_plan(const ConvP &p, int min_wg, size_t v_cap, size_t slab_floats, ConvPlan &pl);
 void wino4_launch(const ConvP &p, const ConvPlan &pl, float *V, hipStream_t s, hipEvent_t *const *ev_in = nullptr,
-                  hipEvent_t *const *ev_gemm = nullptr, hipEvent_t *ev_red = nullptr);
+                  hipEvent_t *const *ev_gemm = nullptr, hipEvent_t *ev_red = nullptr, bool skip_input = false);
+bool wino4_fused_plan(const ConvP &p, ConvPlan &pl);
+void wino4_fused_launch(const ConvP &p, const ConvPlan &pl, hipStream_t s, hipEvent_t *ev_gemm = nullptr);
 void wino4_transform_weights(const float *w, int N, int Cin, int Kp, float *U);
 bool wino_enabled();
 int wino4_mode();
diff --git a/eva_vos_amd/csrc/winograd4.hip b/eva_vos_amd/csrc/winograd4.hip
--- a/eva_vos_amd/csrc/winograd4.hip
+++ b/eva_vos_amd/csrc/winograd4.hip
@@ -8,6 +8,7 @@
 
 namespace stcn {
 
+typedef float f32x2 __attribute__((ext_vector_type(2)));
 typedef float f32x4 __attribute__((ext_vector_type(4)));
 typedef float f32x16 __attribute__((ext_vector_type(16)));
 
@@ -33,13 +34,14 @@
 }
 #endif
 
-__device__ __forceinline__ void bt6(const f32x4 &d0, const f32x4 &d1, const f32x4 &d2, const f32x4 &d3, const f32x4 &d4, const f32x4 &d5,
-                                    f32x4 &o0, f32x4 &o1, f32x4 &o2, f32x4 &o3, f32x4 &o4, f32x4 &o5) {
+template <typename T>
+__device__ __forceinline__ void bt6(const T &d0, const T &d1, const T &d2, const T &d3, const T &d4, const T &d5,
+                                    T &o0, T &o1, T &o2, T &o3, T &o4, T &o5) {
     o0 = d0 * 1.265625f - d2 * 2.8125f + d4;
-    const f32x4 e1 = d4 - d2 * 2.25f, f1 = d3 * 0.75f - d1 * 1.6875f;
+    const T e1 = d4 - d2 * 2.25f, f1 = d3 * 0.75f - d1 * 1.6875f;
     o1 = e1 + f1;
     o2 = e1 - f1;
-    const f32x4 e2 = d4 - d2 * 0.5625f, f2 = d3 * 1.5f - d1 * 0.84375f;
+    const T e2 = d4 - d2 * 0.5625f, f2 = d3 * 1.5f - d1 * 0.84375f;
     o3 = e2 + f2;
     o4 = e2 - f2;
     o5 = d1 * 1.265625f - d3 * 2.8125f + d5;
@@ -113,6 +115,141 @@
     int xb_m, xb_n, xb_cols;
 };
 
+struct W4Epi {
+    int chq, tl, jh, tpi, ohw;
+    float lo;
+    __amdgpu_buffer_rsrc_t rres, ry;
+    unsigned y_bs;
+};
+__device__ __forceinline__ W4Epi w4_epilogue_setup(const Wino4G &p) {
+    const int t = threadIdx.x;
+    W4Epi e;
+    e.chq = t & 7; e.tl = (t >> 3) & 31;
+    e.jh = __builtin_amdgcn_readfirstlane(t >> 8);
+    e.tpi = p.TH * p.TW; e.ohw = p.OH * p.OW;
+    e.lo = p.relu_out ? 0.f : -__builtin_inff();
+    e.rres = __builtin_amdgcn_make_buffer_rsrc(const_cast<float *>(p.res ? p.res : p.y), 0, -1, 0x00020000);
+    e.ry = __builtin_amdgcn_make_buffer_rsrc(p.y, 0, -1, 0x00020000);
+    e.y_bs = (unsigned)(p.y_bs ? p.y_bs : (long)e.ohw * p.N);
+    return e;
+}
+template <bool KP>
+__device__ __forceinline__ void w4_epilogue_block(const Wino4G &p, const W4Epi &e, float *smem, const f32x16 &a0, const f32x16 &a1, const f32x16 &a2,
+                                                  const int pos0, const long tile0, const int toff0, const int tn, const bool sync_first,
+                                                  const int swz, const int piece) {
+    constexpr int PPW = 3;
+    const int lane = threadIdx.x & 63, l31 = lane & 31, h = lane >> 5;
+    const int chq = e.chq, tl = e.tl, jh = e.jh, tpi = e.tpi;
+    const int n = tn * W4N + 4 * chq;
+    const bool kpiece = KP && piece >= 0;
+    const float lo = e.lo;
+    int toff = toff0 + tl;
+    asm volatile("" : "+v"(toff));
+    const long gt = tile0 + toff;
+    const bool work = jh < 2 && gt < p.Mt;
+    const int gtc = (int)min(gt, (long)p.Mt - 1);
+    const int b = fastdiv(gtc, p.fd_tpi);
+    const int rr = gtc - b * tpi;
+    const int ty = fastdiv(rr, p.fd_tw), tx = rr - ty * p.TW;
+    unsigned prow[4], pcol[2];
+#pragma unroll
+    for (int i2 = 0; i2 < 4; ++i2) prow[i2] = (unsigned)(min(4 * ty + i2, p.OH - 1) * p.OW * p.N) * 4u;
+#pragma unroll
+    for (int j = 0; j < 2; ++j) pcol[j] = (unsigned)(min(4 * tx + 2 * jh + j, p.OW - 1) * p.N + n) * 4u;
+    if (sync_first) __syncthreads();
+#pragma unroll
+    for (int pi = 0; pi < PPW; ++pi) {
+        const f32x16 &ac = pi == 0 ? a0 : pi == 1 ? a1 : a2;
+#pragma unroll
+        for (int r = 0; r < 16; ++r)
+            smem[((pos0 + pi) * W4T + (r & 3) + 8 * (r >> 2) + 4 * h) * W4N + l31] = ac[r];
+    }
+    f32x4 yv[2][4], bv = {0.f, 0.f, 0.f, 0.f};
+    if (p.bias && !kpiece) {
+        int nb = n;
+        asm volatile("" : "+v"(nb));
+        bv = *reinterpret_cast<const f32x4 *>(p.bias + nb);
+    }
+    if (p.res && !kpiece && jh < 2) {
+        const unsigned rb = (unsigned)(p.res_bmod ? b % p.res_bmod : b) * (unsigned)p.res_bs * 4u;
+#pragma unroll
+        for (int j = 0; j < 2; ++j)
+#pragma unroll
+            for (int i2 = 0; i2 < 4; ++i2)
+                yv[j][i2] = __builtin_bit_cast(f32x4, __builtin_amdgcn_raw_buffer_load_b128(e.rres, rb + prow[i2] + pcol[j], 0, 0));
+    } else {
+#pragma unroll
+        for (int j = 0; j < 2; ++j)
+#pragma unroll
+            for (int i2 = 0; i2 < 4; ++i2) yv[j][i2] = f32x4{0.f, 0.f, 0.f, 0.f};
+    }
+    __syncthreads();
+    if (!work) return;
+    auto zrow = [&](int xi, auto JH, f32x4 (&zr)[2]) {
+        f32x4 m[6];
+        int ro4 = (xi * 6 * W4T + tl) * (W4N / 4) + chq;
+        asm volatile("" : "+v"(ro4));
+#pragma unroll
+        for (int nu = 0; nu < 6; ++nu) m[nu] = reinterpret_cast<const f32x4 *>(smem)[ro4 + nu * W4T * (W4N / 4)];
+        if (decltype(JH)::value == 0) {
+            zr[0] = m[0] + (m[1] + m[2]) + (m[3] + m[4]);
+            zr[1] = (m[1] - m[2]) * 0.75f + (m[3] - m[4]) * 1.5f;
+        } else {
+            zr[0] = (m[1] + m[2]) * 0.5625f + (m[3] + m[4]) * 2.25f;
+            zr[1] = (m[1] - m[2]) * 0.421875f + (m[3] - m[4]) * 3.375f + m[5];
+        }
+    };
+    auto columns = [&](auto JH) {
+        f32x4 za[2];
+#pragma unroll
+        for (int j = 0; j < 2; ++j)
+#pragma unroll
+            for (int i2 = 0; i2 < 4; ++i2) yv[j][i2] += bv;
+        zrow(0, JH, za);
+#pragma unroll
+        for (int j = 0; j < 2; ++j) yv[j][0] += za[j];
+        constexpr float c1[4] = {0.75f, -0.75f, 1.5f, -1.5f}, c2[4] = {0.5625f, 0.5625f, 2.25f, 2.25f},
+                        c3[4] = {0.421875f, -0.421875f, 3.375f, -3.375f};
+#pragma unroll
+        for (int xi = 1; xi < 5; ++xi) {
+            __builtin_amdgcn_sched_barrier(0);
+            zrow(xi, JH, za);
+#pragma unroll
+            for (int j = 0; j < 2; ++j) {
+                yv[j][0] += za[j];
+                yv[j][1] += za[j] * c1[xi - 1];
+                yv[j][2] += za[j] * c2[xi - 1];
+                yv[j][3] += za[j] * c3[xi - 1];
+            }
+        }
+        __builtin_amdgcn_sched_barrier(0);
+        zrow(5, JH, za);
+#pragma unroll
+        for (int j = 0; j < 2; ++j) yv[j][3] += za[j];
+    };
+    if (jh == 0) columns(std::integral_constant<int, 0>{});
+    else columns(std::integral_constant<int, 1>{});
+    if (kpiece) {
+        float *dst = p.partial + (((long)(swz - p.full_wg) * p.pieces + piece) * W4T + tl) * (16 * W4N) + 4 * chq;
+#pragma unroll
+        for (int j = 0; j < 2; ++j)
+#pragma unroll
+            for (int i2 = 0; i2 < 4; ++i2) *reinterpret_cast<f32x4 *>(dst + (i2 * 4 + 2 * jh + j) * W4N) = yv[j][i2];
+        return;
+    }
+    const unsigned yb = (unsigned)b * e.y_bs * 4u;
+#pragma unroll
+    for (int j = 0; j < 2; ++j)
+#pragma unroll
+        for (int i2 = 0; i2 < 4; ++i2) {
+#pragma unroll
+            for (int c = 0; c < 4; ++c) yv[j][i2][c] = fmaxf(yv[j][i2][c], lo);
+            const bool ok = 4 * tx + 2 * jh + j < p.OW && 4 * ty + i2 < p.OH;
+            __builtin_amdgcn_raw_buffer_store_b128(__builtin_bit_cast(__attribute__((__vector_size__(4 * sizeof(unsigned)))) unsigned, yv[j][i2]), e.ry,
+                                                   ok ? yb + prow[i2] + pcol[j] : 0xFFFFFFFFu, 0, 0);
+        }
+}
+
 template <int MB>
 __global__ __launch_bounds__(64 * W4W) void wino4_gemm_kernel(const Wino4G p, const int tiles_n) {
     constexpr int PPW = 3, WT = W4T * MB;
@@ -267,121 +404,144 @@
         if (lane == 0 && blockIdx.x < 8192) { g_w4_clock[2 * blockIdx.x] = ck_t1 - ck_t0; g_w4_clock[2 * blockIdx.x + 1] = ck_r1 - ck_r0; }
     }
 #endif
-    const int chq = t & 7, tl = (t >> 3) & 31;
-    const int jh = __builtin_amdgcn_readfirstlane(t >> 8);
-    const int tpi = p.TH * p.TW, ohw = p.OH * p.OW;
-    const int n = tn * W4N + 4 * chq;
-    const bool kpiece = MB == 1 && piece >= 0;
-    const float lo = p.relu_out ? 0.f : -__builtin_inff();
-    const __amdgpu_buffer_rsrc_t rres = __builtin_amdgcn_make_buffer_rsrc(const_cast<float *>(p.res ? p.res : p.y), 0, -1, 0x00020000);
-    const __amdgpu_buffer_rsrc_t ry = __builtin_amdgcn_make_buffer_rsrc(p.y, 0, -1, 0x00020000);
-    const unsigned y_bs = (unsigned)(p.y_bs ? p.y_bs : (long)ohw * p.N);
-#pragma unroll
-    for (int half = 0; half < MB; ++half) {
-        int toff = 32 * half + tl;
-        asm volatile("" : "+v"(toff));
-        const long gt = (long)tm * WT + toff;
-        const bool work = jh < 2 && gt < p.Mt;
-        const int gtc = (int)min(gt, (long)p.Mt - 1);
-        const int b = fastdiv(gtc, p.fd_tpi);
-        const int rr = gtc - b * tpi;
-        const int ty = fastdiv(rr, p.fd_tw), tx = rr - ty * p.TW;
-        unsigned prow[4], pcol[2];
-#pragma unroll
-        for (int i2 = 0; i2 < 4; ++i2) prow[i2] = (unsigned)(min(4 * ty + i2, p.OH - 1) * p.OW * p.N) * 4u;
-#pragma unroll
-        for (int j = 0; j < 2; ++j) pcol[j] = (unsigned)(min(4 * tx + 2 * jh + j, p.OW - 1) * p.N + n) * 4u;
-        if (half) __syncthreads();
+    const W4Epi e = w4_epilogue_setup(p);
+#pragma unroll
+    for (int half = 0; half < MB; ++half)
+        w4_epilogue_block<MB == 1>(p, e, smem, acc[0][half], acc[1][half], acc[2][half], pos0, (long)tm * WT, 32 * half, tn, half != 0, swz, piece);
+}
+
+struct Wino4F {
+    Wino4G g;
+    const float *x; unsigned x_bytes; long x_bs;
+    int H, W, relu_in;
+};
+static constexpr int W4F_SLICE = 36 * W4T * 8;
+
+__global__ __launch_bounds__(64 * W4W) void wino4_fused_kernel(const Wino4F q) {
+    constexpr int PPW = 3, C = 64, KB = 8;
+    extern __shared__ __attribute__((aligned(16))) float smem[];
+    const Wino4G &p = q.g;
+    const int t = threadIdx.x, lane = t & 63, l31 = lane & 31, h = lane >> 5;
+    const int wave = __builtin_amdgcn_readfirstlane(t >> 6);
+    const int pos0 = PPW * wave;
+    const int wg = xcd_contiguous_block((int)blockIdx.x, (int)gridDim.x);
+    const int cp = t & 3, tl2 = (t >> 2) & 31;
+    const int w6 = __builtin_amdgcn_readfirstlane(t >> 7);
+    const long tile = (long)wg * W4T + tl2;
+    const bool live = tile < p.Mt;
+    const int tpi = p.TH * p.TW;
+    const int tcl = live ? (int)tile : 0;
+    const int b = fastdiv(tcl, p.fd_tpi);
+    const int r = tcl - b * tpi;
+    const int ty = fastdiv(r, p.fd_tw), tx = r - ty * p.TW;
+    const int y0 = 4 * ty - 1, x0 = 4 * tx - 1 + w6;
+    unsigned ok = 0;
+#pragma unroll
+    for (int yy = 0; yy < 6; ++yy)
+        if (live && (unsigned)(y0 + yy) < (unsigned)q.H && (unsigned)x0 < (unsigned)q.W) ok |= 1u << yy;
+    const __amdgpu_buffer_rsrc_t rx = __builtin_amdgcn_make_buffer_rsrc(const_cast<float *>(q.x), 0, q.x_bytes, 0x00020000);
+    const int xoff = (int)((b * q.x_bs + ((long)y0 * q.W + x0) * C + 2 * cp) * 4);
+    const int rowb = q.W * C * 4;
+    const float lo = q.relu_in ? 0.f : -__builtin_inff();
+    const int tw_off = (w6 * W4T + tl2) * 8 + 2 * cp;
+    const int tr_off = (w6 * 6 * W4T + tl2) * 8 + 2 * cp;
+
+    f32x2 d[6];
+    auto loadx = [&](int kb) {
+#pragma unroll
+        for (int yy = 0; yy < 6; ++yy) {
+            const unsigned vo = ((ok >> yy) & 1u) ? (unsigned)(xoff + yy * rowb + kb * 32) : 0x80000000u;
+            f32x2 v = __builtin_bit_cast(f32x2, __builtin_amdgcn_raw_buffer_load_b64(rx, vo, 0, 0));
+            d[yy] = v;
+        }
+    };
+    auto pass1 = [&](float *T) {
+#pragma unroll
+        for (int c = 0; c < 2; ++c) {
+            float o[6];
+            bt6<float>(fmaxf(d[0][c], lo), fmaxf(d[1][c], lo), fmaxf(d[2][c], lo), fmaxf(d[3][c], lo), fmaxf(d[4][c], lo), fmaxf(d[5][c], lo),
+                       o[0], o[1], o[2], o[3], o[4], o[5]);
+#pragma unroll
+            for (int yy = 0; yy < 6; ++yy) T[tw_off + c + yy * 6 * W4T * 8] = o[yy];
+        }
+    };
+    auto pass2 = [&](const float *T, float *V) {
+#pragma unroll
+        for (int c = 0; c < 2; ++c) {
+            float a[6], v[6];
+#pragma unroll
+            for (int xx = 0; xx < 6; ++xx) a[xx] = T[tr_off + c + xx * W4T * 8];
+            bt6<float>(a[0], a[1], a[2], a[3], a[4], a[5], v[0], v[1], v[2], v[3], v[4], v[5]);
+#pragma unroll
+            for (int nu = 0; nu < 6; ++nu) V[tr_off + c + nu * W4T * 8] = v[nu];
+            __builtin_amdgcn_sched_barrier(0);
+        }
+    };
+
+    const __amdgpu_buffer_rsrc_t ru = __builtin_amdgcn_make_buffer_rsrc(const_cast<float *>(p.U), 0, p.u_bytes, 0x00020000);
+    const unsigned vl = (unsigned)(l31 * 32 + h * 16);
+    unsigned sb0[PPW];
+#pragma unroll
+    for (int pi = 0; pi < PPW; ++pi) sb0[pi] = (unsigned)((pos0 + pi) * KB * C * 32);
+    constexpr unsigned sb = C * 32u;
+    f32x16 acc[PPW][2];
+#pragma unroll
+    for (int pi = 0; pi < PPW; ++pi)
+#pragma unroll
+        for (int bi = 0; bi < 2; ++bi)
+#pragma unroll
+            for (int e = 0; e < 16; ++e) acc[pi][bi][e] = 0.f;
+    f32x4 fa[PPW], fb[2][PPW];
+    auto loadB = [&](int k, int bi, f32x4 (&dd)[PPW]) {
 #pragma unroll
         for (int pi = 0; pi < PPW; ++pi)
-#pragma unroll
-            for (int r = 0; r < 16; ++r)
-                smem[((pos0 + pi) * W4T + (r & 3) + 8 * (r >> 2) + 4 * h) * W4N + l31] = acc[pi][half][r];
-        f32x4 yv[2][4], bv = {0.f, 0.f, 0.f, 0.f};
-        if (p.bias && !kpiece) {
-            int nb = n;
-            asm volatile("" : "+v"(nb));
-            bv = *reinterpret_cast<const f32x4 *>(p.bias + nb);
-        }
-        if (p.res && !kpiece && jh < 2) {
-            const unsigned rb = (unsigned)(p.res_bmod ? b % p.res_bmod : b) * (unsigned)p.res_bs * 4u;
-#pragma unroll
-            for (int j = 0; j < 2; ++j)
-#pragma unroll
-                for (int i2 = 0; i2 < 4; ++i2)
-                    yv[j][i2] = __builtin_bit_cast(f32x4, __builtin_amdgcn_raw_buffer_load_b128(rres, rb + prow[i2] + pcol[j], 0, 0));
-        } else {
-#pragma unroll
-            for (int j = 0; j < 2; ++j)
-#pragma unroll
-                for (int i2 = 0; i2 < 4; ++i2) yv[j][i2] = f32x4{0.f, 0.f, 0.f, 0.f};
-        }
+            dd[pi] = __builtin_bit_cast(f32x4, __builtin_amdgcn_raw_buffer_load_b128(ru, vl, sb0[pi] + (unsigned)k * sb + bi * 1024u, 0));
+    };
+    auto loadA = [&](const float *V) {
+#pragma unroll
+        for (int pi = 0; pi < PPW; ++pi) fa[pi] = *reinterpret_cast<const f32x4 *>(V + (pos0 + pi) * W4T * 8 + l31 * 8 + h * 4);
+    };
+    auto comp = [&](int bi, const f32x4 (&bb)[PPW]) {
+#pragma unroll
+        for (int j = 0; j < 4; ++j)
+#pragma unroll
+            for (int pi = 0; pi < PPW; ++pi) acc[pi][bi] = W4_MFMA(fa[pi][j], bb[pi][j], acc[pi][bi]);
+    };
+
+    float *const V0 = smem, *const T0 = smem + 2 * W4F_SLICE;
+    loadB(0, 0, fb[0]);
+    loadB(0, 1, fb[1]);
+    loadx(0);
+    pass1(T0);
+    loadx(1);
+    __syncthreads();
+    pass2(T0, V0);
+    pass1(T0 + W4F_SLICE);
+    loadx(2);
+    __syncthreads();
+    for (int k = 0; k < KB; ++k) {
+        const int par = k & 1;
+        float *Vc = V0 + par * W4F_SLICE, *Vn = V0 + (par ^ 1) * W4F_SLICE;
+        float *Tc = T0 + par * W4F_SLICE, *Tn = T0 + (par ^ 1) * W4F_SLICE;
+        const int kn = min(k + 1, KB - 1);
+        loadA(Vc);
+        if (k + 2 < KB) pass1(Tc);
+        __builtin_amdgcn_sched_barrier(0);
+        comp(0, fb[0]);
+        __builtin_amdgcn_sched_barrier(0);
+        loadB(kn, 0, fb[0]);
+        if (k + 1 < KB) pass2(Tn, Vn);
+        loadx(min(k + 3, KB - 1));
+        __builtin_amdgcn_sched_barrier(0);
+        comp(1, fb[1]);
+        __builtin_amdgcn_sched_barrier(0);
+        loadB(kn, 1, fb[1]);
         __syncthreads();
-        if (!work) continue;
-        auto zrow = [&](int xi, auto JH, f32x4 (&zr)[2]) {
-            f32x4 m[6];
-            int ro4 = (xi * 6 * W4T + tl) * (W4N / 4) + chq;
-            asm volatile("" : "+v"(ro4));
-#pragma unroll
-            for (int nu = 0; nu < 6; ++nu) m[nu] = reinterpret_cast<const f32x4 *>(smem)[ro4 + nu * W4T * (W4N / 4)];
-            if (decltype(JH)::value == 0) {
-                zr[0] = m[0] + (m[1] + m[2]) + (m[3] + m[4]);
-                zr[1] = (m[1] - m[2]) * 0.75f + (m[3] - m[4]) * 1.5f;
-            } else {
-                zr[0] = (m[1] + m[2]) * 0.5625f + (m[3] + m[4]) * 2.25f;
-                zr[1] = (m[1] - m[2]) * 0.421875f + (m[3] - m[4]) * 3.375f + m[5];
-            }
-        };
-        auto columns = [&](auto JH) {
-            f32x4 za[2];
-#pragma unroll
-            for (int j = 0; j < 2; ++j)
-#pragma unroll
-                for (int i2 = 0; i2 < 4; ++i2) yv[j][i2] += bv;
-            zrow(0, JH, za);
-#pragma unroll
-            for (int j = 0; j < 2; ++j) yv[j][0] += za[j];
-            constexpr float c1[4] = {0.75f, -0.75f, 1.5f, -1.5f}, c2[4] = {0.5625f, 0.5625f, 2.25f, 2.25f},
-                            c3[4] = {0.421875f, -0.421875f, 3.375f, -3.375f};
-#pragma unroll
-            for (int xi = 1; xi < 5; ++xi) {
-                __builtin_amdgcn_sched_barrier(0);
-                zrow(xi, JH, za);
-#pragma unroll
-                for (int j = 0; j < 2; ++j) {
-                    yv[j][0] += za[j];
-                    yv[j][1] += za[j] * c1[xi - 1];
-                    yv[j][2] += za[j] * c2[xi - 1];
-                    yv[j][3] += za[j] * c3[xi - 1];
-                }
-            }
-            __builtin_amdgcn_sched_barrier(0);
-            zrow(5, JH, za);
-#pragma unroll
-            for (int j = 0; j < 2; ++j) yv[j][3] += za[j];
-        };
-        if (jh == 0) columns(std::integral_constant<int, 0>{});
-        else columns(std::integral_constant<int, 1>{});
-        if (kpiece) {
-            float *dst = p.partial + (((long)(swz - p.full_wg) * p.pieces + piece) * W4T + tl) * (16 * W4N) + 4 * chq;
-#pragma unroll
-            for (int j = 0; j < 2; ++j)
-#pragma unroll
-                for (int i2 = 0; i2 < 4; ++i2) *reinterpret_cast<f32x4 *>(dst + (i2 * 4 + 2 * jh + j) * W4N) = yv[j][i2];
-            continue;
-        }
-        const unsigned yb = (unsigned)b * y_bs * 4u;
-#pragma unroll
-        for (int j = 0; j < 2; ++j)
-#pragma unroll
-            for (int i2 = 0; i2 < 4; ++i2) {
-#pragma unroll
-                for (int c = 0; c < 4; ++c) yv[j][i2][c] = fmaxf(yv[j][i2][c], lo);
-                const bool ok = 4 * tx + 2 * jh + j < p.OW && 4 * ty + i2 < p.OH;
-                __builtin_amdgcn_raw_buffer_store_b128(__builtin_bit_cast(__attribute__((__vector_size__(4 * sizeof(unsigned)))) unsigned, yv[j][i2]), ry,
-                                                       ok ? yb + prow[i2] + pcol[j] : 0xFFFFFFFFu, 0, 0);
-            }
-    }
+    }
+    const W4Epi e = w4_epilogue_setup(p);
+#pragma unroll
+    for (int nb = 0; nb < 2; ++nb)
+        w4_epilogue_block<false>(p, e, smem, acc[0][nb], acc[1][nb], acc[2][nb], pos0, (long)wg * W4T, 0, nb, nb != 0, 0, -1);
 }
 
 __global__ __launch_bounds__(256) void wino4_reduce_kernel(const Wino4G p, const int tiles_n) {
@@ -484,7 +644,7 @@
 }
 
 void wino4_launch(const ConvP &p, const ConvPlan &cp, float *V, hipStream_t s, hipEvent_t *const *ev_in, hipEvent_t *const *ev_gemm,
-                  hipEvent_t *ev_red) {
+                  hipEvent_t *ev_red, bool skip_input) {
     const W4Plan &pl = cp.w4;
     const WinoGeom &ge = cp.geo;
     const int tiles_n = pl.tiles_n, mb = pl.mb, tiles_m = pl.tiles_m;
@@ -512,6 +672,7 @@
         const int tile_lo = tm_lo * W4T * mb, tile_hi = pl.chunks == 1 ? ge.Mt_pad : tm_hi * W4T * mb;
         hipEvent_t *ei = ev_in ? ev_in[c] : nullptr, *eg = ev_gemm ? ev_gemm[c] : nullptr;
         const WinoInGrid ig = wino_input_grid(tile_hi - tile_lo, p.Cin);
+        if (!(skip_input && pl.chunks == 1))
         launch(wino4_input_kernel, dim3(ig.gx, ig.chunks), dim3(256), 0, s, ei, p.x0, p.x0_bytes, p.bs0, p.H, p.W, p.Cin, p.relu_in, ge.TH, ge.TW,
                ge.Mt, ge.Mt_pad, ig.per, tile_lo, tile_hi, V);
         g.tm0 = tm_lo;
@@ -525,6 +686,24 @@
     }
 }
 
+bool wino4_fused_plan(const ConvP &p, ConvPlan &cp) {
+    if (cp.family != CONV_WINO4 || !p.wino4_fused || !p.kn.wino4_fused) return false;
+    if (p.Cin != 64 || p.N != 64 || p.x1 || p.bs0 != (long)p.H * p.W * p.Cin || cp.w4.pieces != 1) return false;
+    cp.family = CONV_WINO4F;
+    cp.v_floats = 0;
+    cp.n_in = 0; cp.n_gemm = 1; cp.reduce = false;
+    return true;
+}
+
+void wino4_fused_launch(const ConvP &p, const ConvPlan &cp, hipStream_t s, hipEvent_t *ev_gemm) {
+    const WinoGeom &ge = cp.geo;
+    Wino4F q{};
+    wino_fill_desc(q.g, p, ge, 36, nullptr, p.wino4_u, 2);
+    q.g.full_wg = ge.Mt_pad / W4T; q.g.pieces = 1; q.g.kb_per_piece = ge.KB; q.g.partial = nullptr;
+    q.x = p.x0; q.x_bytes = p.x0_bytes; q.x_bs = p.bs0; q.H = p.H; q.W = p.W; q.relu_in = p.relu_in;
+    launch(wino4_fused_kernel, dim3(ge.Mt_pad / W4T), dim3(64 * W4W), (size_t)4 * W4F_SLICE * sizeof(float), s, ev_gemm, q);
+}
+
 void wino4_transform_weights(const float *w, int N, int Cin, int Kp, float *U) {
     static const double G[6][3] = {{64.0 / 81, 0, 0},
                                    {-128.0 / 243, -32.0 / 81, -8.0 / 27},
```

Result: no change. 808.1 frames/s (median of 3 runs) (+0.7%).
